# antoyang/FrozenBiLM

Hardware: AMD Instinct MI355X
Metric: video-text samples/sec (MLM fwd+bwd) DeBERTa-XL+adapters (higher is better)
Workload: dtype bf16; 1 GPU; DeBERTa-v2-XLarge(24L)+adapters ds8/8, B=32/GPU, T=10x1024, L=256 (S=266), MLM fwd+bwd+allreduce+clip+Adam, dropout 0.1 live, seeded random weights; global_batch=32, seq_len=266, parallelism=dp1, dead_layer23_encoder_pass=skipped (output unused, SURVEY fact 6); FLOPs still counted

## Files before the change

frozenbilm_amd/attn_bwd.py:

```python
from __future__ import annotations

import math
from dataclasses import dataclass, field
from typing import Optional

import torch

from . import lib as L

BF16, F32 = torch.bfloat16, torch.float32
ATTN_SCALE = 1.0 / math.sqrt(64 * 3)


_RANGE = {}


def _relidx_range(S, cfg):
    key = (S, cfg.position_buckets, cfg.max_rel, cfg.att_span)
    if key not in _RANGE:
        from .model.relpos import rel_index_vector

        rv = rel_index_vector(S, cfg.position_buckets, cfg.max_rel, cfg.att_span)
        _RANGE[key] = (int(rv[0]), int(rv[-1]) - int(rv[0]) + 1)
    return _RANGE[key]


_DRANGE = {}
POS_GRAD_MAX_DELTAS = 8


def _delta_ranges(S, cfg, dev, limit=POS_GRAD_MAX_DELTAS):
    key = (S, cfg.position_buckets, cfg.max_rel, cfg.att_span, str(dev))
    if key not in _DRANGE:
        import numpy as np

        from .model.relpos import rel_index_vector

        rv = np.asarray(rel_index_vector(S, cfg.position_buckets, cfg.max_rel, cfg.att_span), dtype=np.int64)
        rmin, rcnt = int(rv[0]), int(rv[-1]) - int(rv[0]) + 1
        first = np.searchsorted(rv, np.arange(rmin, rmin + rcnt), side="left")
        last = np.searchsorted(rv, np.arange(rmin, rmin + rcnt), side="right")
        dlo = (first - (S - 1)).astype(np.int16)
        dcnt = (last - first).astype(np.int16)
        _DRANGE[key] = (torch.from_numpy(dlo).to(dev), torch.from_numpy(dcnt).to(dev), int(dcnt.max()))
    cmax = _DRANGE[key][2]
    if limit is not None and cmax > limit:
        raise NotImplementedError(
            f"position-table gradients (fbl_attn_pos_grad) take at most {limit} relative positions per table "
            f"row; position_buckets={cfg.position_buckets}, max_relative_positions={cfg.max_rel} at sequence length {S} "
            f"puts {cmax} on one row")
    return _DRANGE[key]


def disent_attn_bwd(eng, run, sv, dctx, dqkv, dpqk, defer_pos=False):
    B, S, H, nh, span2 = run.B, run.S, eng.H, eng.nh, eng.span2
    Sp = (S + 63) // 64 * 64
    dev = eng.dev
    qkv = sv.qkv
    q, k, v = qkv[:, :H], qkv[:, H:2 * H], qkv[:, 2 * H:]
    pq, pk = sv.pqk[:, :H], sv.pqk[:, H:]
    relidx = eng.relidx(S)
    klen, border = run.klen, getattr(run, "border", None)
    scale = ATTN_SCALE
    pk_ = getattr(run, "pk", None)
    row0 = pk_.row0 if pk_ is not None else None
    saved_p = getattr(sv, "psave", None) is not None

    Dv = torch.empty(B, nh, S, dtype=F32, device=dev)
    PKX = torch.empty(nh, 2 * Sp, 64, dtype=BF16, device=dev)
    if saved_p:
        QT = PQT = None
        PQX = torch.empty(nh, 2 * Sp, 64, dtype=BF16, device=dev)
    else:
        QT = torch.empty(nh, 64, B, Sp, dtype=BF16, device=dev)
        PQT = torch.empty(nh, 64, span2, dtype=BF16, device=dev)
        PQX = None
    L.attn_bwd_prep(q, pq, pk, dctx, sv.ctx, QT, PQT, Dv, B, S, Sp, nh, span2, row0=row0, relidx=relidx, PQX=PQX, PKX=PKX)
    dS = torch.empty(B, nh, Sp, Sp, dtype=BF16, device=dev)
    dST = torch.empty(B, nh, Sp, Sp, dtype=BF16, device=dev)
    lin = eng.cfg.position_buckets // 2 if eng.cfg.position_buckets > 0 else eng.cfg.att_span - 1
    if saved_p:
        L.disent_attn_bwd_dspk(sv.psave, sv.msave, q, v, dctx, PQX, sv.lse, Dv, scale, dqkv[:, H:2 * H], dqkv[:, 2 * H:], dS, dST,
                               B, S, Sp, nh, p_drop=run.p_att, seed=sv.seed_att, klen=klen, border=border, row0=row0)
        sv.psave = sv.msave = None
    else:
        lin_a = min(lin, span2 // 2) if eng.cfg.position_buckets > 0 else 0
        L.disent_attn_bwd_ds(q, k, v, dctx, pk, pq, relidx, run.mask_i32, sv.lse, Dv, scale, dqkv[:, 2 * H:], dS, dST,
                             B, S, Sp, nh, span2, p_drop=run.p_att, seed=sv.seed_att, klen=klen, border=border, lin=lin_a, row0=row0)
    L.disent_attn_bwd_dq(dS, k, PKX, dqkv[:, :H], B, S, Sp, nh, klen=klen, border=border, row0=row0)
    if not saved_p:
        L.disent_attn_bwd_shear(dST, QT, PQT, relidx, dqkv[:, H:2 * H], B, S, Sp, nh, span2, klen=klen, lin=lin, border=border,
                                row0=row0)
    rmin, rcnt = _relidx_range(S, eng.cfg)
    state = dict(dS=dS, dST=dST, q=q, k=k, rmin=rmin, rcnt=rcnt, B=B, S=S, Sp=Sp, klen=klen, row0=row0)
    if defer_pos:
        return state
    dpqk.copy_(pos_table_grads(eng, state))
    return None


def pos_table_grads(eng, st):
    H, nh, span2 = eng.H, eng.nh, eng.span2
    rmin, rcnt, B, Sp = st["rmin"], st["rcnt"], st["B"], st["Sp"]
    dpos = torch.zeros(span2, 2 * H, dtype=F32, device=eng.dev)
    dlo, dcnt, cmax = _delta_ranges(st["S"], eng.cfg, eng.dev, limit=None)
    for neg, X, Y, col0 in ((0, st["dS"], st["q"], H), (1, st["dST"], st["k"], 0)):
        d = torch.empty(1, nh, rcnt, 64, dtype=F32, device=eng.dev)
        L.attn_pos_grad(neg, [X], [Y], dlo, dcnt, cmax, d, B, st["S"], Sp, nh, rcnt, klen=st["klen"], row0=st["row0"])
        dpos[rmin:rmin + rcnt, col0:col0 + H].view(rcnt, nh, 64).copy_(d[0].permute(1, 0, 2))
    return dpos


@dataclass
class PosChain:
    rmin: int
    rcnt: int
    B: int
    S: int
    Sp: int
    dS: list = field(default_factory=list)
    dST: list = field(default_factory=list)
    q: list = field(default_factory=list)
    k: list = field(default_factory=list)
    seeds: list = field(default_factory=list)
    klen: Optional[torch.Tensor] = None
    row0: Optional[torch.Tensor] = None
    n_formed: int = 0
    n_exec: int = 0
    nh: int = 0
    dev: Optional[torch.device] = None
    dbuf: Optional[tuple] = None

    def add(self, st, seed_pos):
        self.dS.append(st["dS"]); self.dST.append(st["dST"]); self.q.append(st["q"]); self.k.append(st["k"])
        self.seeds.append(seed_pos)
        self.klen, self.row0 = st["klen"], st["row0"]

    def formed_slot(self):
        assert not self.dS and self.n_exec > self.n_formed, "executions with formed table gradients come first"
        if self.dbuf is None:
            self.dbuf = tuple(torch.empty(self.n_exec, self.nh, self.rcnt, 64, dtype=F32, device=self.dev) for _ in range(2))
        return self.dbuf[0][self.n_formed], self.dbuf[1][self.n_formed]

    def add_formed(self, seed_pos):
        self.n_formed += 1
        self.seeds.append(seed_pos)


def pos_chain_buffers(eng, run):
    rmin, rcnt = _relidx_range(run.S, eng.cfg)
    return PosChain(rmin=rmin, rcnt=rcnt, B=run.B, S=run.S, Sp=(run.S + 63) // 64 * 64, nh=eng.nh, dev=eng.dev)


def pos_table_grads_batched(eng, run, pc: PosChain):
    H, nh, span2 = eng.H, eng.nh, eng.span2
    E, rmin, rcnt, B, Sp = len(pc.seeds), pc.rmin, pc.rcnt, pc.B, pc.Sp
    dev = eng.dev
    dpb = torch.empty(E, rcnt, 2 * H, dtype=BF16, device=dev)
    dlo, dcnt, cmax = _delta_ranges(pc.S, eng.cfg, dev, limit=None)
    for neg, X, Y, col0 in ((0, pc.dS, pc.q, H), (1, pc.dST, pc.k, 0)):
        nf = pc.n_formed
        if pc.dbuf is not None:
            assert pc.n_exec == E, (pc.n_exec, E)
            d = pc.dbuf[neg]
        else:
            d = torch.empty(E, nh, rcnt, 64, dtype=F32, device=dev)
        if X:
            L.attn_pos_grad(neg, X, Y, dlo, dcnt, cmax, d[nf:], B, pc.S, Sp, nh, rcnt, klen=pc.klen, row0=pc.row0)
        L.heads_to_rows_bf16(d, dpb[:, :, col0:col0 + H])
    if getattr(run, "lora_pos_wait", False):
        eng._lora_pos_bwd(run, pc, dpb)
    tmp = torch.empty(E, rcnt, H, dtype=F32, device=dev)
    L.gemm(dpb, eng.WposT_exec[:E], out_f32=tmp)
    dR = L.zeros(span2, H, dtype=F32, device=dev)
    L.dropout_sum_f32(tmp, pc.seeds if run.p_hid > 0 else [0] * E, run.p_hid, dR[rmin:rmin + rcnt], key0=rmin * H)
    return dR
```

frozenbilm_amd/build.py:

```python
from __future__ import annotations

import concurrent.futures as cf
import os
import shutil
import subprocess
import sys

HERE = os.path.dirname(os.path.abspath(__file__))
CSRC = os.path.join(HERE, "csrc")
DEBUG = os.environ.get("FBL_DEBUG_BUILD", "0") == "1"
OBJ = os.path.join(HERE, "csrc", "build_dbg" if DEBUG else "build")
LIB = os.path.join(HERE, "libfbl_dbg.so" if DEBUG else "libfbl.so")
ARCH = "gfx950"
FLAGS = ["--offload-arch=" + ARCH, "-O3", "-std=c++17", "-fPIC", "-fno-gpu-rdc", "-Wno-unused-result"]
if DEBUG:
    FLAGS.append("-DFBL_DEBUG_SWITCHES")
    FLAGS += os.environ.get("FBL_DEBUG_EXTRA_FLAGS", "").split()
    if os.environ.get("FBL_DEBUG_LIB_NAME"):
        LIB = os.path.join(HERE, os.environ["FBL_DEBUG_LIB_NAME"])
        OBJ = os.path.join(HERE, "csrc", "build_dbg_" + os.path.splitext(os.environ["FBL_DEBUG_LIB_NAME"])[0])


def _hipcc() -> str:
    for cand in (os.environ.get("HIPCC"), shutil.which("hipcc"), "/opt/rocm/bin/hipcc"):
        if cand and os.path.exists(cand):
            return cand
    raise RuntimeError("hipcc not found (need ROCm >= 7.0 with gfx950 support)")


def sources():
    return sorted(os.path.join(CSRC, f) for f in os.listdir(CSRC) if f.endswith(".hip"))


def _deps_mtime() -> float:
    hdrs = [os.path.join(CSRC, f) for f in os.listdir(CSRC) if f.endswith(".h")]
    hdrs += [os.path.join(os.path.dirname(HERE), "include", h) for h in ("fbl.h", "fbl_mha.h", "fbl_qrows.h", "fbl_live.h", "fbl_predict.h", "fbl_groups.h", "fbl_lora.h", "fbl_ema.h", "fbl_prompt.h")]
    return max(os.path.getmtime(h) for h in hdrs)


def _compile(src: str, force: bool) -> str:
    obj = os.path.join(OBJ, os.path.basename(src)[:-4] + ".o")
    if not force and os.path.exists(obj) and os.path.getmtime(obj) > max(os.path.getmtime(src), _deps_mtime()):
        return obj
    cmd = [_hipcc(), *FLAGS, "-Rpass-analysis=kernel-resource-usage", "-c", src, "-o", obj]
    r = subprocess.run(cmd, capture_output=True, text=True)
    if r.returncode != 0:
        raise RuntimeError(f"hipcc failed for {src}:\n{r.stdout}\n{r.stderr}")
    bad, name = [], "?"
    for line in r.stderr.splitlines():
        if "Function Name:" in line:
            name = line.split("Function Name:")[1].split("[")[0].strip()
        elif "ScratchSize [bytes/lane]:" in line:
            n = int(line.split("ScratchSize [bytes/lane]:")[1].split("[")[0])
            if n > 64:
                bad.append(f"{name}: {n} bytes/lane")
            elif n > 0:
                print(f"[frozenbilm_amd.build] note: {name} spills {n} bytes/lane")
    if bad and os.environ.get("FBL_ALLOW_SCRATCH", "0") != "1":
        os.remove(obj)
        raise RuntimeError(f"{os.path.basename(src)}: kernels using scratch memory (set FBL_ALLOW_SCRATCH=1 to build anyway):\n  "
                           + "\n  ".join(bad))
    return obj


def build_lib(force: bool = False, verbose: bool = True) -> str:
    os.makedirs(OBJ, exist_ok=True)
    srcs = sources()
    with cf.ThreadPoolExecutor(max_workers=min(8, len(srcs))) as ex:
        objs = list(ex.map(lambda s: _compile(s, force), srcs))
    if force or not os.path.exists(LIB) or any(os.path.getmtime(o) > os.path.getmtime(LIB) for o in objs):
        cmd = [_hipcc(), "--offload-arch=" + ARCH, "-shared", "-fPIC", "-o", LIB, *objs]
        r = subprocess.run(cmd, capture_output=True, text=True)
        if r.returncode != 0:
            raise RuntimeError(f"link failed:\n{r.stdout}\n{r.stderr}")
        if verbose:
            print(f"[frozenbilm_amd.build] linked {LIB} from {len(objs)} objects")
    elif verbose:
        print(f"[frozenbilm_amd.build] {LIB} up to date")
    return LIB


if __name__ == "__main__":
    build_lib(force="--force" in sys.argv)
```

frozenbilm_amd/csrc/rowops.hip:

```cpp
#include "fbl_common.h"
#include "../../include/fbl.h"
#include "../../include/fbl_live.h"
#include "../../include/fbl_groups.h"
#include "../../include/fbl_ema.h"

namespace {

template <int VEC>
struct VecF {};
template <>
struct VecF<4> {
  typedef f32x4 T;
};
template <>
struct VecF<2> {
  typedef f32x2 T;
};

template <int VEC>
__device__ __forceinline__ void ldf(const float* p, float* v) {
  if (VEC == 4) {
    f32x4 x = *(const f32x4*)p;
    v[0] = x[0]; v[1] = x[1]; v[2] = x[2]; v[3] = x[3];
  } else if (VEC == 2) {
    f32x2 x = *(const f32x2*)p;
    v[0] = x[0]; v[1] = x[1];
  } else {
    v[0] = p[0];
  }
}
template <int VEC>
__device__ __forceinline__ void stf(float* p, const float* v) {
  if (VEC == 4) *(f32x4*)p = (f32x4){v[0], v[1], v[2], v[3]};
  else if (VEC == 2) *(f32x2*)p = (f32x2){v[0], v[1]};
  else p[0] = v[0];
}
template <int VEC>
__device__ __forceinline__ void stb(bf16* p, const float* v) {
  if (VEC == 4) *(bf16x4*)p = (bf16x4){f2bf(v[0]), f2bf(v[1]), f2bf(v[2]), f2bf(v[3])};
  else if (VEC == 2) *(bf16x2*)p = (bf16x2){f2bf(v[0]), f2bf(v[1])};
  else p[0] = f2bf(v[0]);
}

struct LnFwdArgs {
  const float* y; long ldy; float p_drop; uint64_t seed; const uint64_t* seed_dev;
  const float* r_plain; const float* r_t; const float* r_stats; const float* r_gamma; const float* r_beta;
  const int32_t* r_rowmask;
  const float* gamma; const float* beta; float eps; const int32_t* rowmask;
  float* out_t; float* out_stats; bf16* out_bf16; float* out_f32;
  int N, H;
};

template <int EPL>
__global__ __launch_bounds__(256) void ln_fwd_kernel(LnFwdArgs a) {
  constexpr int VEC = (EPL % 4 == 0) ? 4 : ((EPL % 2 == 0) ? 2 : 1);
  constexpr int NIT = EPL / VEC;
  const int lane = threadIdx.x & 63;
  const int row = blockIdx.x * 4 + (threadIdx.x >> 6);
  if (row >= a.N) return;
  const int H = a.H;
  float v[EPL];
  const uint32_t thr = fbl_drop_thresh(a.p_drop);
  const float inv_keep = a.p_drop > 0.f ? 1.0f / (1.0f - a.p_drop) : 1.0f;
  const uint64_t seed = a.p_drop > 0.f ? fbl_seed(a.seed, a.seed_dev) : 0;
  float rmean = 0.f, rrstd = 0.f, rmask = 1.f;
  if (a.r_t) {
    rmean = a.r_stats[2 * (long)row];
    rrstd = a.r_stats[2 * (long)row + 1];
    if (a.r_rowmask) rmask = (float)a.r_rowmask[row];
  }
#pragma unroll
  for (int it = 0; it < NIT; ++it) {
    const int col = (it * 64 + lane) * VEC;
    float* vv = v + it * VEC;
    if (a.y) {
      ldf<VEC>(a.y + (long)row * a.ldy + col, vv);
      if (a.p_drop > 0.f) {
#pragma unroll
        for (int c = 0; c < VEC; ++c) vv[c] *= fbl_dropout_scale(seed, (uint64_t)row * H + col + c, thr, inv_keep);
      }
    } else {
#pragma unroll
      for (int c = 0; c < VEC; ++c) vv[c] = 0.f;
    }
    if (a.r_plain) {
      float r[VEC];
      ldf<VEC>(a.r_plain + (long)row * H + col, r);
#pragma unroll
      for (int c = 0; c < VEC; ++c) vv[c] += r[c];
    }
    if (a.r_t) {
      float r[VEC], gg[VEC], bb[VEC];
      ldf<VEC>(a.r_t + (long)row * H + col, r);
      ldf<VEC>(a.r_gamma + col, gg);
      ldf<VEC>(a.r_beta + col, bb);
#pragma unroll
      for (int c = 0; c < VEC; ++c) vv[c] += ((r[c] - rmean) * rrstd * gg[c] + bb[c]) * rmask;
    }
    if (a.out_t) stf<VEC>(a.out_t + (long)row * H + col, vv);
  }
  float s = 0.f;
#pragma unroll
  for (int e = 0; e < EPL; ++e) s += v[e];
  const float mean = wave_sum(s) / (float)H;
  float q = 0.f;
#pragma unroll
  for (int e = 0; e < EPL; ++e) {
    const float d = v[e] - mean;
    q += d * d;
  }
  const float var = wave_sum(q) / (float)H;
  const float rstd = rsqrtf(var + a.eps);
  if (lane == 0 && a.out_stats) {
    a.out_stats[2 * (long)row] = mean;
    a.out_stats[2 * (long)row + 1] = rstd;
  }
  const float om = a.rowmask ? (float)a.rowmask[row] : 1.0f;
#pragma unroll
  for (int it = 0; it < NIT; ++it) {
    const int col = (it * 64 + lane) * VEC;
    float gg[VEC], bb[VEC], o[VEC];
    ldf<VEC>(a.gamma + col, gg);
    ldf<VEC>(a.beta + col, bb);
#pragma unroll
    for (int c = 0; c < VEC; ++c) o[c] = ((v[it * VEC + c] - mean) * rstd * gg[c] + bb[c]) * om;
    if (a.out_bf16) stb<VEC>(a.out_bf16 + (long)row * H + col, o);
    if (a.out_f32) stf<VEC>(a.out_f32 + (long)row * H + col, o);
  }
}

struct LnMatArgs {
  const float* t; const float* stats; const float* gamma; const float* beta; const int32_t* rowmask;
  const float* add_bcast; int S; float* out_f32; bf16* out_bf16; int N, H;
};
template <int EPL>
__global__ __launch_bounds__(256) void ln_mat_kernel(LnMatArgs a) {
  constexpr int VEC = (EPL % 4 == 0) ? 4 : ((EPL % 2 == 0) ? 2 : 1);
  constexpr int NIT = EPL / VEC;
  const int lane = threadIdx.x & 63;
  const int row = blockIdx.x * 4 + (threadIdx.x >> 6);
  if (row >= a.N) return;
  const int H = a.H;
  const float mean = a.stats[2 * (long)row], rstd = a.stats[2 * (long)row + 1];
  const float om = a.rowmask ? (float)a.rowmask[row] : 1.0f;
#pragma unroll
  for (int it = 0; it < NIT; ++it) {
    const int col = (it * 64 + lane) * VEC;
    float x[VEC], gg[VEC], bb[VEC], o[VEC];
    ldf<VEC>(a.t + (long)row * H + col, x);
    ldf<VEC>(a.gamma + col, gg);
    ldf<VEC>(a.beta + col, bb);
#pragma unroll
    for (int c = 0; c < VEC; ++c) o[c] = ((x[c] - mean) * rstd * gg[c] + bb[c]) * om;
    if (a.add_bcast) {
      float p[VEC];
      ldf<VEC>(a.add_bcast + (long)(row % a.S) * H + col, p);
#pragma unroll
      for (int c = 0; c < VEC; ++c) o[c] += p[c];
    }
    if (a.out_f32) stf<VEC>(a.out_f32 + (long)row * H + col, o);
    if (a.out_bf16) stb<VEC>(a.out_bf16 + (long)row * H + col, o);
  }
}

constexpr int LNB_BLOCKS = 768;
struct LnBwdArgs {
  const float* dout; const int32_t* rowmask; const float* t; const float* stats; const float* gamma;
  float p_drop; uint64_t seed; const uint64_t* seed_dev; float* out_dt; bf16* out_dy_bf16; float* out_dy_f32; float* ws; int N, H;
  long ld_dyb;
};
template <int EPL>
__global__ __launch_bounds__(256) void ln_bwd_kernel(LnBwdArgs a) {
  constexpr int VEC = (EPL % 4 == 0) ? 4 : ((EPL % 2 == 0) ? 2 : 1);
  constexpr int NIT = EPL / VEC;
  __shared__ float red[4 * 64 * EPL];
  const int lane = threadIdx.x & 63, wave = threadIdx.x >> 6;
  const int H = a.H;
  float dg[EPL], db[EPL], dys[EPL], gam[EPL];
#pragma unroll
  for (int e = 0; e < EPL; ++e) dg[e] = db[e] = dys[e] = 0.f;
#pragma unroll
  for (int it = 0; it < NIT; ++it) ldf<VEC>(a.gamma + (it * 64 + lane) * VEC, gam + it * VEC);
  const uint32_t thr = fbl_drop_thresh(a.p_drop);
  const float inv_keep = a.p_drop > 0.f ? 1.0f / (1.0f - a.p_drop) : 1.0f;
  const uint64_t seed = a.p_drop > 0.f ? fbl_seed(a.seed, a.seed_dev) : 0;
  for (int row = blockIdx.x * 4 + wave; row < a.N; row += gridDim.x * 4) {
    const float mean = a.stats[2 * (long)row], rstd = a.stats[2 * (long)row + 1];
    const float om = a.rowmask ? (float)a.rowmask[row] : 1.0f;
    float g[EPL], xh[EPL];
    float s1 = 0.f, s2 = 0.f;
#pragma unroll
    for (int it = 0; it < NIT; ++it) {
      const int col = (it * 64 + lane) * VEC;
      float d[VEC], x[VEC];
      ldf<VEC>(a.dout + (long)row * H + col, d);
      ldf<VEC>(a.t + (long)row * H + col, x);
#pragma unroll
      for (int c = 0; c < VEC; ++c) {
        const int e = it * VEC + c;
        const float dd = d[c] * om;
        xh[e] = (x[c] - mean) * rstd;
        dg[e] += dd * xh[e];
        db[e] += dd;
        g[e] = dd * gam[e];
        s1 += g[e];
        s2 += g[e] * xh[e];
      }
    }
    s1 = wave_sum(s1) / (float)H;
    s2 = wave_sum(s2) / (float)H;
#pragma unroll
    for (int it = 0; it < NIT; ++it) {
      const int col = (it * 64 + lane) * VEC;
      float dt[VEC], dy[VEC];
#pragma unroll
      for (int c = 0; c < VEC; ++c) {
        const int e = it * VEC + c;
        dt[c] = rstd * (g[e] - s1 - xh[e] * s2);
        dy[c] = dt[c];
        if (a.p_drop > 0.f) dy[c] *= fbl_dropout_scale(seed, (uint64_t)row * H + col + c, thr, inv_keep);
        dys[e] += dy[c];
      }
      if (a.out_dt) stf<VEC>(a.out_dt + (long)row * H + col, dt);
      if (a.out_dy_bf16) stb<VEC>(a.out_dy_bf16 + (long)row * a.ld_dyb + col, dy);
      if (a.out_dy_f32) stf<VEC>(a.out_dy_f32 + (long)row * H + col, dy);
    }
  }
#pragma unroll
  for (int which = 0; which < 3; ++which) {
    const float* src = which == 0 ? dg : (which == 1 ? db : dys);
    if (which) __syncthreads();
#pragma unroll
    for (int it = 0; it < NIT; ++it) {
      const int col = (it * 64 + lane) * VEC;
#pragma unroll
      for (int c = 0; c < VEC; ++c) red[wave * H + col + c] = src[it * VEC + c];
    }
    __syncthreads();
    for (int i = threadIdx.x; i < H; i += 256) {
      float s_ = 0.f;
#pragma unroll
      for (int w = 0; w < 4; ++w) s_ += red[w * H + i];
      a.ws[(long)blockIdx.x * 3 * H + which * H + i] = s_;
    }
  }
}
template <int EPL>
__global__ __launch_bounds__(256, 3) void ln_bwd2_kernel(LnBwdArgs a) {
  static_assert(EPL % 2 == 0, "two waves share a row");
  constexpr int EW = EPL / 2;
  constexpr int VEC = (EW % 4 == 0) ? 4 : ((EW % 2 == 0) ? 2 : 1);
  constexpr int NIT = EW / VEC;
  __shared__ float red[2 * 64 * EPL];
  __shared__ float xch[2][2][2][2];
  const int lane = threadIdx.x & 63, wave = threadIdx.x >> 6;
  const int slot = wave >> 1, half = wave & 1;
  const int H = a.H;
  const int c0 = half * (H / 2);
  float dg[EW], db[EW], dys[EW], gam[EW];
#pragma unroll
  for (int e = 0; e < EW; ++e) dg[e] = db[e] = dys[e] = 0.f;
#pragma unroll
  for (int it = 0; it < NIT; ++it) ldf<VEC>(a.gamma + c0 + (it * 64 + lane) * VEC, gam + it * VEC);
  const uint32_t thr = fbl_drop_thresh(a.p_drop);
  const float inv_keep = a.p_drop > 0.f ? 1.0f / (1.0f - a.p_drop) : 1.0f;
  const uint64_t seed = a.p_drop > 0.f ? fbl_seed(a.seed, a.seed_dev) : 0;
  int par = 0;
  for (int base = blockIdx.x * 2; base < a.N; base += gridDim.x * 2, par ^= 1) {
    const int row = base + slot;
    const bool live = row < a.N;
    const int rr = live ? row : a.N - 1;
    const float mean = a.stats[2 * (long)rr], rstd = a.stats[2 * (long)rr + 1];
    const float om = live ? (a.rowmask ? (float)a.rowmask[rr] : 1.0f) : 0.f;
    float g[EW], xh[EW];
    float s1 = 0.f, s2 = 0.f;
#pragma unroll
    for (int it = 0; it < NIT; ++it) {
      const int col = c0 + (it * 64 + lane) * VEC;
      float d[VEC], x[VEC];
      ldf<VEC>(a.dout + (long)rr * H + col, d);
      ldf<VEC>(a.t + (long)rr * H + col, x);
#pragma unroll
      for (int c = 0; c < VEC; ++c) {
        const int e = it * VEC + c;
        const float dd = d[c] * om;
        xh[e] = (x[c] - mean) * rstd;
        dg[e] += dd * xh[e];
        db[e] += dd;
        g[e] = dd * gam[e];
        s1 += g[e];
        s2 += g[e] * xh[e];
      }
    }
    s1 = wave_sum(s1);
    s2 = wave_sum(s2);
    if (lane == 0) {
      xch[par][slot][half][0] = s1;
      xch[par][slot][half][1] = s2;
    }
    __syncthreads();
    s1 = (xch[par][slot][0][0] + xch[par][slot][1][0]) / (float)H;
    s2 = (xch[par][slot][0][1] + xch[par][slot][1][1]) / (float)H;
    if (live) {
#pragma unroll
      for (int it = 0; it < NIT; ++it) {
        const int col = c0 + (it * 64 + lane) * VEC;
        float dt[VEC], dy[VEC];
#pragma unroll
        for (int c = 0; c < VEC; ++c) {
          const int e = it * VEC + c;
          dt[c] = rstd * (g[e] - s1 - xh[e] * s2);
          dy[c] = dt[c];
          if (a.p_drop > 0.f) dy[c] *= fbl_dropout_scale(seed, (uint64_t)row * H + col + c, thr, inv_keep);
          dys[e] += dy[c];
        }
        if (a.out_dt) stf<VEC>(a.out_dt + (long)row * H + col, dt);
        if (a.out_dy_bf16) stb<VEC>(a.out_dy_bf16 + (long)row * a.ld_dyb + col, dy);
        if (a.out_dy_f32) stf<VEC>(a.out_dy_f32 + (long)row * H + col, dy);
      }
    }
  }
#pragma unroll
  for (int which = 0; which < 3; ++which) {
    const float* src = which == 0 ? dg : (which == 1 ? db : dys);
    __syncthreads();
#pragma unroll
    for (int it = 0; it < NIT; ++it) {
      const int col = c0 + (it * 64 + lane) * VEC;
#pragma unroll
      for (int c = 0; c < VEC; ++c) red[slot * H + col + c] = src[it * VEC + c];
    }
    __syncthreads();
    for (int i = threadIdx.x; i < H; i += 256) a.ws[(long)blockIdx.x * 3 * H + which * H + i] = red[i] + red[H + i];
  }
}

__device__ __forceinline__ float fold16(const float* ws, int nblk, int ncols, int col) {
  __shared__ float red[16][17];
  const int tx = threadIdx.x & 15, ty = threadIdx.x >> 4;
  float s = 0.f;
  if (col < ncols)
    for (int b = ty; b < nblk; b += 16) s += ws[(long)b * ncols + col];
  red[ty][tx] = s;
  __syncthreads();
  if (ty == 0) {
#pragma unroll
    for (int k = 1; k < 16; ++k) s += red[k][tx];
  }
  return s;
}
__global__ __launch_bounds__(256) void ln_bwd_fold_kernel(const float* ws, int nblk, int H, float* dgamma, float* dbeta,
                                                          float* dysum) {
  __shared__ f32x4 red[4][8];
  const int tx = threadIdx.x & 7, ty = threadIdx.x >> 3;
  const int lane = threadIdx.x & 63, wave = threadIdx.x >> 6;
  const int col = blockIdx.x * 32 + tx * 4;
  const int ncols = 3 * H;
  f32x4 s = {0.f, 0.f, 0.f, 0.f};
  if (col < ncols) {
    const float* p = ws + col;
    int b = ty;
    for (; b + 224 < nblk; b += 256) {
      f32x4 v[8];
#pragma unroll
      for (int u = 0; u < 8; ++u) v[u] = *(const f32x4*)(p + (long)(b + 32 * u) * ncols);
      s += ((v[0] + v[1]) + (v[2] + v[3])) + ((v[4] + v[5]) + (v[6] + v[7]));
    }
    for (; b < nblk; b += 32) s += *(const f32x4*)(p + (long)b * ncols);
  }
#pragma unroll
  for (int o = 8; o < 64; o <<= 1) {
#pragma unroll
    for (int r = 0; r < 4; ++r) s[r] += __shfl_xor(s[r], o, 64);
  }
  if (lane < 8) red[wave][lane] = s;
  __syncthreads();
  if (threadIdx.x < 8 && col < ncols) {
    s = (red[0][tx] + red[1][tx]) + (red[2][tx] + red[3][tx]);
    float* dst = col < H ? dgamma : (col < 2 * H ? dbeta : dysum);
    if (dst) {
      float* q = dst + (col % H);
#pragma unroll
      for (int r = 0; r < 4; ++r) q[r] += s[r];
    }
  }
}

__global__ void embed_gather_kernel(const int64_t* ids, const float* E, const float* vproj, int B, int T, int L, int H,
                                    float* out) {
  const int S = T + L;
  const int row = blockIdx.x;
  const int b = row / S, s = row % S;
  const float* src = (s < T) ? vproj + ((long)b * T + s) * H : E + ids[(long)b * L + (s - T)] * (long)H;
  float* dst = out + (long)row * H;
  for (int c = threadIdx.x * 4; c < H; c += blockDim.x * 4) *(f32x4*)(dst + c) = *(const f32x4*)(src + c);
}

__global__ void video_stage_kernel(const _Float16* feats, const int64_t* row_off, const int32_t* n_rows, int T, int F,
                                   float* out, int64_t* video_len, int64_t* video_mask) {
  const int b = blockIdx.x / T, j = blockIdx.x % T;
  const int n = n_rows[b];
  const int len = n < T ? n : T;
  if (threadIdx.x == 0) {
    if (j == 0 && video_len) video_len[b] = len;
    if (video_mask) video_mask[(long)b * T + j] = j < len ? 1 : 0;
  }
  float* dst = out + ((long)b * T + j) * F;
  if (j >= len) {
    for (int c = threadIdx.x * 4; c < F; c += blockDim.x * 4) *(f32x4*)(dst + c) = (f32x4){0.f, 0.f, 0.f, 0.f};
    return;
  }
  const long r = n > T ? ((long)j * n) / T : j;
  const _Float16* src = feats + (row_off[b] + r) * (long)F;
  typedef __attribute__((ext_vector_type(8))) _Float16 f16x8;
  for (int c = threadIdx.x * 8; c < F; c += blockDim.x * 8) {
    const f16x8 h = *(const f16x8*)(src + c);
    *(f32x4*)(dst + c) = (f32x4){(float)h[0], (float)h[1], (float)h[2], (float)h[3]};
    *(f32x4*)(dst + c + 4) = (f32x4){(float)h[4], (float)h[5], (float)h[6], (float)h[7]};
  }
}

__global__ void mask_tokens_kernel(int64_t* ids, int64_t* labels, long n, const int64_t* special, int n_special, float p,
                                   int64_t mask_id, int64_t vocab, uint64_t seed) {
  const long i = (long)blockIdx.x * blockDim.x + threadIdx.x;
  if (i >= n) return;
  const int64_t id = ids[i];
  bool sp = false;
  for (int k = 0; k < n_special; ++k) sp |= (special[k] == id);
  const float inv = 1.0f / 4294967296.0f;
  const bool pick = !sp && (float)fbl_hash(seed, 4ull * i) * inv < p;
  labels[i] = pick ? id : -100;
  if (!pick) return;
  if ((float)fbl_hash(seed, 4ull * i + 1) * inv < 0.8f) ids[i] = mask_id;
  else if ((float)fbl_hash(seed, 4ull * i + 2) * inv < 0.5f) ids[i] = (int64_t)(fbl_hash(seed, 4ull * i + 3) % (uint64_t)vocab);
}

__global__ void im2col3_kernel(const bf16* x, bf16* out, int B, int S, int H) {
  const int row = blockIdx.x;
  const int s = row % S;
  const int chunks = 3 * H / 8;
  for (int i = threadIdx.x; i < chunks; i += blockDim.x) {
    const int k = (i * 8) / H, c = (i * 8) % H;
    const int ss = s + k - 1;
    bf16x8 v = {0, 0, 0, 0, 0, 0, 0, 0};
    if (ss >= 0 && ss < S) v = *(const bf16x8*)(x + ((long)row + k - 1) * H + c);
    *(bf16x8*)(out + (long)row * 3 * H + i * 8) = v;
  }
}
__global__ void col2im3_kernel(const float* dcol, float* dx, int B, int S, int H, int accumulate) {
  const int row = blockIdx.x;
  const int s = row % S;
  for (int c = threadIdx.x * 4; c < H; c += blockDim.x * 4) {
    f32x4 acc = accumulate ? *(const f32x4*)(dx + (long)row * H + c) : (f32x4){0.f, 0.f, 0.f, 0.f};
#pragma unroll
    for (int k = 0; k < 3; ++k) {
      const int ss = s - k + 1;
      if (ss >= 0 && ss < S) acc += *(const f32x4*)(dcol + ((long)row - k + 1) * 3 * H + k * H + c);
    }
    *(f32x4*)(dx + (long)row * H + c) = acc;
  }
}

__global__ void dropout_gelu_fwd_kernel(const float* c, float p, uint64_t seed0, const uint64_t* seed_dev, float* out, long n) {
  const uint64_t seed = p > 0.f ? fbl_seed(seed0, seed_dev) : 0;
  const uint32_t thr = fbl_drop_thresh(p);
  const float ik = p > 0.f ? 1.f / (1.f - p) : 1.f;
  for (long i = (long)blockIdx.x * blockDim.x + threadIdx.x; i < n; i += (long)gridDim.x * blockDim.x) {
    float v = c[i];
    if (p > 0.f) v *= fbl_dropout_scale(seed, (uint64_t)i, thr, ik);
    out[i] = gelu_erf(v);
  }
}
// ... 472 lines not shown
__global__ __launch_bounds__(256) void swap_f32_kernel(float* a, float* b, long n4) {
  u32x4* a4 = (u32x4*)a;
  u32x4* b4 = (u32x4*)b;
  for (long i = (long)blockIdx.x * blockDim.x + threadIdx.x; i < n4; i += (long)gridDim.x * blockDim.x) {
    const u32x4 x = a4[i], y = b4[i];
    a4[i] = y;
    b4[i] = x;
  }
}
__global__ void cast_bf16_kernel(const float* in, bf16* out, long n) {
  for (long i = (long)blockIdx.x * blockDim.x + threadIdx.x; i < n; i += (long)gridDim.x * blockDim.x) out[i] = f2bf(in[i]);
}
__global__ void dropout_f32_kernel(const float* in, float p, uint64_t seed0, const uint64_t* seed_dev, float* of, bf16* ob, long n) {
  const uint64_t seed = p > 0.f ? fbl_seed(seed0, seed_dev) : 0;
  const uint32_t thr = fbl_drop_thresh(p);
  const float ik = p > 0.f ? 1.f / (1.f - p) : 1.f;
  for (long i = (long)blockIdx.x * blockDim.x + threadIdx.x; i < n; i += (long)gridDim.x * blockDim.x) {
    float v = in[i];
    if (p > 0.f) v *= fbl_dropout_scale(seed, (uint64_t)i, thr, ik);
    if (of) of[i] = v;
    if (ob) ob[i] = f2bf(v);
  }
}
__global__ void dropout_bf16_kernel(bf16* x, float p, uint64_t seed0, const uint64_t* seed_dev, long n) {
  const uint64_t seed = fbl_seed(seed0, seed_dev);
  const uint32_t thr = fbl_drop_thresh(p);
  const float ik = 1.f / (1.f - p);
  for (long i = (long)blockIdx.x * blockDim.x + threadIdx.x; i < n; i += (long)gridDim.x * blockDim.x)
    x[i] = f2bf(bf2f(x[i]) * fbl_dropout_scale(seed, (uint64_t)i, thr, ik));
}

struct DropSumArgs {
  uint64_t seeds[FBL_DROPSUM_MAX_SLICES];
  const float* x;
  const uint64_t* seed_dev;
  float* out;
  long n, key0;
  int ns;
  float p;
};
__global__ void dropout_sum_kernel(DropSumArgs a) {
  const uint32_t thr = fbl_drop_thresh(a.p);
  const float ik = a.p > 0.f ? 1.f / (1.f - a.p) : 1.f;
  const uint64_t word = (a.p > 0.f && a.seed_dev) ? *a.seed_dev : 0;
  for (long i = (long)blockIdx.x * blockDim.x + threadIdx.x; i < a.n; i += (long)gridDim.x * blockDim.x) {
    float acc = 0.f;
    for (int s = 0; s < a.ns; ++s) {
      float v = a.x[(long)s * a.n + i];
      if (a.p > 0.f) v *= fbl_dropout_scale(a.seeds[s] + word, (uint64_t)(a.key0 + i), thr, ik);
      acc += v;
    }
    a.out[i] = acc;
  }
}

__global__ void heads_to_rows_bf16_kernel(const float* src, bf16* dst, int E, int nh, int rows, long ld_dst) {
  const long total = (long)E * nh * rows * 8;
  for (long t = (long)blockIdx.x * blockDim.x + threadIdx.x; t < total; t += (long)gridDim.x * blockDim.x) {
    const int c8 = (int)(t & 7);
    const long q = t >> 3;
    const int r = (int)(q % rows);
    const long eh = q / rows;
    const int h = (int)(eh % nh);
    const long e = eh / nh;
    const f32x4 a = *(const f32x4*)(src + q * 64 + c8 * 8), b = *(const f32x4*)(src + q * 64 + c8 * 8 + 4);
    *(bf16x8*)(dst + (e * rows + r) * ld_dst + h * 64 + c8 * 8) =
        (bf16x8){f2bf(a[0]), f2bf(a[1]), f2bf(a[2]), f2bf(a[3]), f2bf(b[0]), f2bf(b[1]), f2bf(b[2]), f2bf(b[3])};
  }
}

inline int grid1d(long n, int block = 256, int cap = 256 * 16) {
  long b = (n + block - 1) / block;
  return (int)(b < 1 ? 1 : (b > cap ? cap : b));
}

}

#define FBL_EPL_DISPATCH(H, KERNEL, GRID, ARGS, STREAM)                                              \
  switch ((H) / 64) {                                                                                \
    case 1: hipLaunchKernelGGL(KERNEL<1>, GRID, dim3(256), 0, STREAM, ARGS); break;                  \
    case 2: hipLaunchKernelGGL(KERNEL<2>, GRID, dim3(256), 0, STREAM, ARGS); break;                  \
    case 4: hipLaunchKernelGGL(KERNEL<4>, GRID, dim3(256), 0, STREAM, ARGS); break;                  \
    case 8: hipLaunchKernelGGL(KERNEL<8>, GRID, dim3(256), 0, STREAM, ARGS); break;                  \
    case 12: hipLaunchKernelGGL(KERNEL<12>, GRID, dim3(256), 0, STREAM, ARGS); break;                \
    case 16: hipLaunchKernelGGL(KERNEL<16>, GRID, dim3(256), 0, STREAM, ARGS); break;                \
    case 24: hipLaunchKernelGGL(KERNEL<24>, GRID, dim3(256), 0, STREAM, ARGS); break;                \
    case 32: hipLaunchKernelGGL(KERNEL<32>, GRID, dim3(256), 0, STREAM, ARGS); break;                \
    default: return FBL_ERR_SHAPE;                                                                   \
  }

extern "C" int fbl_abi_version(void) { return 9; }

extern "C" int fbl_embed_gather(const int64_t* ids, const float* E, const float* vproj, int B, int T, int L, int H,
                                float* out_t, void* stream) {
  if (H % 4) return FBL_ERR_SHAPE;
  if (T > 0 && !vproj) return FBL_ERR_ARG;
  if (B * (T + L) <= 0) return 0;
  hipLaunchKernelGGL(embed_gather_kernel, dim3(B * (T + L)), dim3(128), 0, (hipStream_t)stream, ids, E, vproj, B, T, L,
                     H, out_t);
  FBL_CHECK_LAUNCH();
  return 0;
}

extern "C" int fbl_video_stage_f16(const void* feats_f16, const int64_t* row_off, const int32_t* n_rows, int B, int T, int F,
                                   float* out_f32, int64_t* video_len, int64_t* video_mask, void* stream) {
  if (F % 8 || ((uintptr_t)feats_f16 & 15) || ((uintptr_t)out_f32 & 15)) return FBL_ERR_ALIGN;
  if (B <= 0 || T <= 0) return 0;
  hipLaunchKernelGGL(video_stage_kernel, dim3(B * T), dim3(128), 0, (hipStream_t)stream, (const _Float16*)feats_f16, row_off,
                     n_rows, T, F, out_f32, video_len, video_mask);
  FBL_CHECK_LAUNCH();
  return 0;
}

extern "C" int fbl_mask_tokens(int64_t* ids, int64_t* labels, int64_t n, const int64_t* special_ids, int n_special,
                               float mlm_probability, int64_t mask_token_id, int64_t vocab_size, uint64_t seed,
                               void* stream) {
  if (n <= 0) return 0;
  if (vocab_size <= 0 || mlm_probability < 0.f || mlm_probability > 1.f || n_special < 0) return FBL_ERR_ARG;
  hipLaunchKernelGGL(mask_tokens_kernel, dim3((unsigned)((n + 255) / 256)), dim3(256), 0, (hipStream_t)stream, ids, labels,
                     (long)n, special_ids, n_special, mlm_probability, mask_token_id, vocab_size, seed);
  FBL_CHECK_LAUNCH();
  return 0;
}

extern "C" int fbl_ln_fwd(const float* y, int64_t ldy, float p_drop, uint64_t seed, const uint64_t* seed_dev, const float* r_plain,
                          const float* r_t, const float* r_stats, const float* r_gamma, const float* r_beta,
                          const int32_t* r_rowmask, const float* gamma, const float* beta, float eps,
                          const int32_t* rowmask, float* out_t, float* out_stats, void* out_bf16, float* out_f32, int N,
                          int H, void* stream) {
  if (H % 64 || H > 2048) return FBL_ERR_SHAPE;
  if (r_t && (!r_stats || !r_gamma || !r_beta)) return FBL_ERR_ARG;
  if (N <= 0) return 0;
  LnFwdArgs a{y, ldy, p_drop, seed, seed_dev, r_plain, r_t, r_stats, r_gamma, r_beta, r_rowmask, gamma, beta, eps, rowmask,
              out_t, out_stats, (bf16*)out_bf16, out_f32, N, H};
  dim3 grid((N + 3) / 4);
  FBL_EPL_DISPATCH(H, ln_fwd_kernel, grid, a, (hipStream_t)stream);
  FBL_CHECK_LAUNCH();
  return 0;
}

extern "C" int fbl_ln_materialize(const float* t, const float* stats, const float* gamma, const float* beta,
                                  const int32_t* rowmask, const float* add_bcast, int S, float* out_f32, void* out_bf16,
                                  int N, int H, void* stream) {
  if (H % 64 || H > 2048) return FBL_ERR_SHAPE;
  if (N <= 0) return 0;
  LnMatArgs a{t, stats, gamma, beta, rowmask, add_bcast, S > 0 ? S : 1, out_f32, (bf16*)out_bf16, N, H};
  dim3 grid((N + 3) / 4);
  FBL_EPL_DISPATCH(H, ln_mat_kernel, grid, a, (hipStream_t)stream);
  FBL_CHECK_LAUNCH();
  return 0;
}

extern "C" int64_t fbl_ln_bwd_ws_floats(int H) { return (int64_t)LNB_BLOCKS * 3 * H; }
extern "C" int fbl_ln_bwd(const float* dout, const int32_t* rowmask, const float* t, const float* stats,
                          const float* gamma, float p_drop, uint64_t seed, const uint64_t* seed_dev, float* out_dt, void* out_dy_bf16,
                          float* out_dy_f32, float* dgamma, float* dbeta, float* dysum, float* ws, int N, int H,
                          int64_t ld_dy_bf16, void* stream) {
  if (H % 64 || H > 2048) return FBL_ERR_SHAPE;
  if (N <= 0) return 0;
  if (ld_dy_bf16 == 0) ld_dy_bf16 = H;
  if (ld_dy_bf16 < H || (ld_dy_bf16 % 8)) return FBL_ERR_ALIGN;
  LnBwdArgs a{dout, rowmask, t, stats, gamma, p_drop, seed, seed_dev, out_dt, (bf16*)out_dy_bf16, out_dy_f32, ws, N, H, ld_dy_bf16};
  int nblk;
  if ((H / 64) % 2 == 0) {
    nblk = (N + 1) / 2;
    if (nblk > LNB_BLOCKS) nblk = LNB_BLOCKS;
    dim3 grid(nblk);
    switch (H / 64) {
      case 2: hipLaunchKernelGGL(ln_bwd2_kernel<2>, grid, dim3(256), 0, (hipStream_t)stream, a); break;
      case 4: hipLaunchKernelGGL(ln_bwd2_kernel<4>, grid, dim3(256), 0, (hipStream_t)stream, a); break;
      case 8: hipLaunchKernelGGL(ln_bwd2_kernel<8>, grid, dim3(256), 0, (hipStream_t)stream, a); break;
      case 12: hipLaunchKernelGGL(ln_bwd2_kernel<12>, grid, dim3(256), 0, (hipStream_t)stream, a); break;
      case 16: hipLaunchKernelGGL(ln_bwd2_kernel<16>, grid, dim3(256), 0, (hipStream_t)stream, a); break;
      case 24: hipLaunchKernelGGL(ln_bwd2_kernel<24>, grid, dim3(256), 0, (hipStream_t)stream, a); break;
      case 32: hipLaunchKernelGGL(ln_bwd2_kernel<32>, grid, dim3(256), 0, (hipStream_t)stream, a); break;
      default: return FBL_ERR_SHAPE;
    }
  } else {
    nblk = (N + 3) / 4;
    if (nblk > LNB_BLOCKS) nblk = LNB_BLOCKS;
    dim3 grid(nblk);
    FBL_EPL_DISPATCH(H, ln_bwd_kernel, grid, a, (hipStream_t)stream);
  }
  FBL_CHECK_LAUNCH();
  if (dgamma || dbeta || dysum) {
    hipLaunchKernelGGL(ln_bwd_fold_kernel, dim3((3 * H + 31) / 32), dim3(256), 0, (hipStream_t)stream, ws, nblk, H,
                       dgamma, dbeta, dysum);
    FBL_CHECK_LAUNCH();
  }
  return 0;
}

extern "C" int fbl_im2col3(const void* x_bf16, void* out_bf16, int B, int S, int H, void* stream) {
  if (H % 8) return FBL_ERR_SHAPE;
  if (B * S <= 0) return 0;
  hipLaunchKernelGGL(im2col3_kernel, dim3(B * S), dim3(256), 0, (hipStream_t)stream, (const bf16*)x_bf16,
                     (bf16*)out_bf16, B, S, H);
  FBL_CHECK_LAUNCH();
  return 0;
}
extern "C" int fbl_col2im3(const float* dcol, float* dx, int B, int S, int H, int accumulate, void* stream) {
  if (H % 4) return FBL_ERR_SHAPE;
  if (B * S <= 0) return 0;
  hipLaunchKernelGGL(col2im3_kernel, dim3(B * S), dim3(256), 0, (hipStream_t)stream, dcol, dx, B, S, H, accumulate);
  FBL_CHECK_LAUNCH();
  return 0;
}

extern "C" int fbl_dropout_gelu_fwd(const float* c, float p_drop, uint64_t seed, const uint64_t* seed_dev, float* out_f32,
                                    int64_t n, void* stream) {
  if (n <= 0) return 0;
  hipLaunchKernelGGL(dropout_gelu_fwd_kernel, dim3(grid1d(n)), dim3(256), 0, (hipStream_t)stream, c, p_drop, seed, seed_dev,
                     out_f32, (long)n);
  FBL_CHECK_LAUNCH();
  return 0;
}
extern "C" int fbl_dropout_gelu_bwd(const float* dy, const float* c, float p_drop, uint64_t seed, const uint64_t* seed_dev,
                                    void* out_bf16, float* out_f32, int64_t n, void* stream) {
  if (n <= 0) return 0;
  hipLaunchKernelGGL(dropout_gelu_bwd_kernel, dim3(grid1d(n)), dim3(256), 0, (hipStream_t)stream, dy, c, p_drop, seed, seed_dev,
                     (bf16*)out_bf16, out_f32, (long)n);
  FBL_CHECK_LAUNCH();
  return 0;
}

extern "C" int fbl_transpose_to_bf16(const void* in, int in_is_bf16, int64_t ld_in, int rows, int cols, void* out_bf16,
                                     int64_t rows_pad, void* stream) {
  if (rows_pad < rows) return FBL_ERR_ARG;
  if (rows_pad <= 0 || cols <= 0) return 0;
  dim3 grid((unsigned)((rows_pad + 63) / 64), (cols + 63) / 64);
  if (in_is_bf16)
    hipLaunchKernelGGL(transpose_kernel<true>, grid, dim3(256), 0, (hipStream_t)stream, in, (long)ld_in, rows, cols,
                       (bf16*)out_bf16, (long)rows_pad);
  else
    hipLaunchKernelGGL(transpose_kernel<false>, grid, dim3(256), 0, (hipStream_t)stream, in, (long)ld_in, rows, cols,
                       (bf16*)out_bf16, (long)rows_pad);
  FBL_CHECK_LAUNCH();
  return 0;
}

extern "C" int fbl_transpose_batched_bf16(const void* src_bf16, const int64_t* src_off, void* dst_bf16,
                                          const int64_t* dst_off, int count, int rows, int cols, void* stream) {
  if (count <= 0 || rows <= 0 || cols <= 0) return 0;
  hipLaunchKernelGGL(transpose_batched_kernel, dim3((rows + 63) / 64, (cols + 63) / 64, count), dim3(256), 0,
                     (hipStream_t)stream, (const bf16*)src_bf16, src_off, (bf16*)dst_bf16, dst_off, rows, cols);
  FBL_CHECK_LAUNCH();
  return 0;
}

extern "C" int64_t fbl_colsum_ws_floats(int cols) { return (int64_t)CS_BLOCKS * cols; }
extern "C" int fbl_colsum(const void* in, int in_is_bf16, int64_t ld_in, int rows, int cols, float* out, float* ws,
                          void* stream) {
  if (rows <= 0 || cols <= 0) return 0;
  int nblk = rows < CS_BLOCKS ? rows : CS_BLOCKS;
  dim3 grid(nblk, (cols + 255) / 256);
  if (in_is_bf16)
    hipLaunchKernelGGL(colsum_kernel<true>, grid, dim3(256), 0, (hipStream_t)stream, in, (long)ld_in, rows, cols, ws);
  else
    hipLaunchKernelGGL(colsum_kernel<false>, grid, dim3(256), 0, (hipStream_t)stream, in, (long)ld_in, rows, cols, ws);
  FBL_CHECK_LAUNCH();
  hipLaunchKernelGGL(colsum_fold_kernel, dim3((cols + 15) / 16), dim3(256), 0, (hipStream_t)stream, ws, nblk, cols,
                     out);
  FBL_CHECK_LAUNCH();
  return 0;
}

extern "C" int fbl_head_transpose(const void* v_bf16, int64_t ldv, void* vt_bf16, int B, int S, int Sp, int nh,
                                  int64_t out_sh, int64_t out_sb, int64_t out_sd, void* stream) {
  if (Sp < S || Sp % 64) return FBL_ERR_SHAPE;
  if (ldv % 8 || out_sh % 8 || out_sb % 8 || out_sd % 8 || ((uintptr_t)v_bf16 & 15) || ((uintptr_t)vt_bf16 & 15)) return FBL_ERR_ALIGN;
  if (B * S <= 0) return 0;
  hipLaunchKernelGGL(head_transpose_kernel, dim3(Sp / 64, nh, B), dim3(256), 0, (hipStream_t)stream,
                     (const bf16*)v_bf16, (long)ldv, (bf16*)vt_bf16, B, S, Sp, nh, (long)out_sh, (long)out_sb,
                     (long)out_sd);
  FBL_CHECK_LAUNCH();
  return 0;
}

extern "C" int fbl_ce_fwd(const float* logits, int64_t ldv, const int64_t* labels, int N, int V, float* row_lse,
                          float* loss_sum_cnt, void* stream) {
  if (N <= 0) return 0;
  hipLaunchKernelGGL(ce_fwd_kernel, dim3(N), dim3(256), 0, (hipStream_t)stream, logits, (long)ldv, labels, N, V,
                     row_lse, loss_sum_cnt);
  FBL_CHECK_LAUNCH();
  hipLaunchKernelGGL(ce_fold_kernel, dim3(1), dim3(256), 0, (hipStream_t)stream, logits, (long)ldv, labels, N, row_lse,
                     loss_sum_cnt);
  FBL_CHECK_LAUNCH();
  return 0;
}
extern "C" int fbl_ce_bwd_rows(const float* logits, int64_t ldv, const int64_t* labels, const int32_t* rows, int R,
                               int V, int Vp, const float* row_lse, const float* loss_sum_cnt, float gscale,
                               const float* gscale_dev, void* dlogits_bf16, void* stream) {
  if (R <= 0) return 0;
  if (Vp < V) return FBL_ERR_ARG;
  hipLaunchKernelGGL(ce_bwd_rows_kernel, dim3(R), dim3(256), 0, (hipStream_t)stream, logits, (long)ldv, labels, rows, V,
                     Vp, row_lse, loss_sum_cnt, gscale, gscale_dev, (bf16*)dlogits_bf16);
  FBL_CHECK_LAUNCH();
  return 0;
}

extern "C" int fbl_gather_rows_bf16(const void* in, int64_t ld, const int32_t* rows, int R, int cols, void* out,
                                    void* stream) {
  if (R <= 0) return 0;
  if (cols % 8 || ld % 8) return FBL_ERR_ALIGN;
  hipLaunchKernelGGL(gather_rows_bf16_kernel, dim3(R), dim3(128), 0, (hipStream_t)stream, (const bf16*)in, (long)ld,
                     rows, cols, (bf16*)out);
  FBL_CHECK_LAUNCH();
  return 0;
}
extern "C" int fbl_scatter_rows_f32(const float* in, const int32_t* rows, int R, int cols, float* out, int64_t ld,
                                    void* stream) {
  if (R <= 0) return 0;
  hipLaunchKernelGGL(scatter_rows_f32_kernel, dim3(R), dim3(256), 0, (hipStream_t)stream, in, rows, cols, out,
                     (long)ld);
  FBL_CHECK_LAUNCH();
  return 0;
}

extern "C" int64_t fbl_sumsq_ws_floats(void) { return SUMSQ_BLOCKS; }
extern "C" int fbl_sumsq(const float* x, int64_t n, float* out_sumsq, float* ws, void* stream) {
  if (n <= 0) return 0;
  if (!ws || !out_sumsq) return FBL_ERR_ARG;
  const int nblk = grid1d(n, 256, SUMSQ_BLOCKS);
  hipLaunchKernelGGL(sumsq_kernel, dim3(nblk), dim3(256), 0, (hipStream_t)stream, x, (long)n, ws);
  FBL_CHECK_LAUNCH();
  hipLaunchKernelGGL(sumsq_fold_kernel, dim3(1), dim3(256), 0, (hipStream_t)stream, (const float*)ws, nblk, out_sumsq);
  FBL_CHECK_LAUNCH();
  return 0;
}
extern "C" int fbl_adam_flat(float* p, const float* g, float* m, float* v, int64_t n, float lr, float beta1,
                             float beta2, float eps, float weight_decay, int step, const float* sumsq, float max_norm,
                             float grad_scale, void* stream) {
  if (n <= 0) return 0;
  const float bc1 = 1.0f - powf(beta1, (float)step);
  const float bc2 = 1.0f - powf(beta2, (float)step);
  hipLaunchKernelGGL(adam_flat_kernel, dim3(grid1d(n)), dim3(256), 0, (hipStream_t)stream, p, g, m, v, (long)n, lr,
                     beta1, beta2, eps, weight_decay, bc1, bc2, sumsq, max_norm, grad_scale);
  FBL_CHECK_LAUNCH();
  return 0;
}

static inline bool live_aligned(const void* a) { return ((uintptr_t)a & 15) == 0; }
extern "C" int fbl_sumsq_live(const float* x, int64_t n, const int64_t* ranges, float* out_sumsq, float* ws, void* stream) {
// ... 140 lines not shown
```

frozenbilm_amd/engine.py:

```python
from __future__ import annotations

from dataclasses import dataclass, field
from typing import Dict, List, Optional

import numpy as np
import torch

from . import lib as L
from .predict import check_topk, of_call as predictions_of_call
from .live_set import REL_LN, LiveSetMixin, flat_layout, stage_plan
from .attn_bwd import ATTN_SCALE, _relidx_range, disent_attn_bwd, pos_chain_buffers, pos_table_grads_batched
from .model.deberta import PROMPT_NAME
from .model.relpos import rel_index_vector

BF16, F32 = torch.bfloat16, torch.float32


def _ru(x: int, m: int) -> int:
    return (x + m - 1) // m * m


def check_logit_rows(logit_rows: torch.Tensor, n_grid: int) -> None:
    r = logit_rows.reshape(-1)
    if r.numel() == 0:
        return
    s = torch.sort(r.long()).values
    dup = (s[1:] == s[:-1]).any() if s.numel() > 1 else torch.zeros((), dtype=torch.bool, device=s.device)
    lo, hi, dup = torch.stack([s[0], s[-1], dup.long()]).tolist()
    if lo < 0 or hi >= n_grid:
        raise ValueError(f"logit_rows must index the [B, S] token grid: 0 <= row < {n_grid} (got {lo} .. {hi})")
    if dup:
        raise ValueError("logit_rows holds an index more than once: with gradients every requested row must be distinct")


@dataclass
class NormRef:
    t: torch.Tensor
    stats: torch.Tensor
    gamma: torch.Tensor
    beta: torch.Tensor
    rowmask: Optional[torch.Tensor] = None

    def as_args(self):
        return (self.t, self.stats, self.gamma, self.beta, self.rowmask)


@dataclass
class Stream:
    bf16: torch.Tensor
    norm: Optional[NormRef] = None
    plain: Optional[torch.Tensor] = None
    full: Optional[torch.Tensor] = None


@dataclass
class Packing:
    row0: torch.Tensor
    sel: torch.Tensor
    inv: torch.Tensor
    pos: torch.Tensor
    n: int


@dataclass
class MergedPack:
    A: int
    WT: torch.Tensor
    WM: torch.Tensor
    bM: torch.Tensor
    b16: torch.Tensor
    WF: Optional[torch.Tensor]
    groups: list


@dataclass
class AdapterSite:
    name: str
    A: int
    Ap: int
    down: torch.Tensor
    up: torch.Tensor
    bd: torch.Tensor
    bu: torch.Tensor
    merged: bool
    grouped: bool
    WM: Optional[torch.Tensor] = None
    bM: Optional[torch.Tensor] = None
    WF: Optional[torch.Tensor] = None
    upT: Optional[torch.Tensor] = None
    downT: Optional[torch.Tensor] = None


@dataclass
class LoraSite:
    name: str
    li: int
    t: int
    idx: int


class Engine(LiveSetMixin):
    def __init__(self, model):
        self.m = model
        cfg = model.config
        self.cfg = cfg
        self.H, self.I, self.V = cfg.hidden_size, cfg.intermediate_size, cfg.vocab_size
        self.nh = cfg.num_attention_heads
        self.nL = cfg.num_hidden_layers
        self.span2 = 2 * cfg.att_span
        self.lin_span = min(cfg.position_buckets // 2, cfg.att_span) if cfg.position_buckets > 0 else 0
        self.F = model.features_dim
        self.Fp = _ru(self.F, 64) if self.F else 0
        self.A1 = self.H // model.ds_factor_attn if model.ds_factor_attn else 0
        self.A2 = self.H // model.ds_factor_ff if model.ds_factor_ff else 0
        self.Vp = _ru(self.V, 64)
        dev = model.device
        if dev.type != "cuda":
            raise RuntimeError("frozenbilm_amd runs on MI355X only: move the model to a cuda (HIP) device; "
                               "there is no CPU fallback")
        L.load()
        self.dev = dev
        o = dict(getattr(model, "engine_options", None) or {})
        unknown = set(o) - {"eager_logits", "dw_group", "attn_save_p"}
        if unknown:
            raise ValueError(f"unknown engine_options: {sorted(unknown)}")
        self.eager_logits = bool(o.get("eager_logits", False))
        self.attn_save_p = bool(o.get("attn_save_p", True))
        self.dw_group = max(1, min(L.ADW_MAX_ADAPTERS, int(o.get("dw_group", 16))))
        self.n_prompt = int(getattr(model, "n_prompt", 0))
        self._build_flat()
        self._pack_frozen()
        self._build_trainable_operands()
        self._build_lora()
        self._compose_ev = None
        self._relidx: Dict[int, torch.Tensor] = {}
        self._pos_cache: Dict[int, torch.Tensor] = {}
        self._no_pos_cache = False
        self.reducer = None
        self._dyz_pool: Dict[tuple, list] = {}
        self._dyz_shape = None
        self.params_version = 0
        self._ops_version = None
        self.skip_dead_layer = True
        self._ln_ws = L.ln_bwd_ws(self.H, dev)
        self._cs_ws = L.colsum_ws(max(self.H, self.I), dev)
        self.sk_ws = torch.empty(48 << 20, dtype=F32, device=dev)
        self.side = torch.cuda.Stream(device=dev)
        self.side_ws = torch.empty(8 << 20, dtype=F32, device=dev)
        self.side_cs_ws = L.colsum_ws(max(self.H, self.I), dev)
        if L._AUX.get(dev.index if dev.index is not None else torch.cuda.current_device()) is None:
            L.set_aux_stream(torch.cuda.Stream(device=dev), dev)
        L.exclude_from_aux(self.side)

    def _build_flat(self):
        from .model.deberta import flat_order

        m = self.m
        named = dict(m.named_parameters())
        train_names = m.trainable_names()
        order = flat_order(self.cfg, train_names)
        offs, total = flat_layout(order, {n: named[n].numel() for n in order})
        self.flat = torch.zeros(total, dtype=F32, device=self.dev)
        from .parallel import SCALAR_SLOT

        self.flat_grad_full = torch.zeros(SCALAR_SLOT + total, dtype=F32, device=self.dev)
        self.flat_grad = self.flat_grad_full[SCALAR_SLOT:]
        self.flat_bf16 = torch.zeros(total, dtype=BF16, device=self.dev)
        self.offsets, self.order = offs, order
        self._adT_offs = {}
        self.G: Dict[str, torch.Tensor] = {}
        self.Pb: Dict[str, torch.Tensor] = {}
        for n in order:
            p = named[n]
            o, k = offs[n], p.numel()
            view = self.flat[o:o + k].view(p.shape)
            view.copy_(p.data)
            p.data = view
            self.G[n] = self.flat_grad[o:o + k].view(p.shape)
            self.Pb[n] = self.flat_bf16[o:o + k].view(p.shape)
        self.P = {n: p.data for n, p in named.items()}
        self.named = named
        self.bucket_ends: Dict[str, int] = {}
        for n in order:
            key = self._bucket_key(n)
            self.bucket_ends[key] = offs[n] + _ru(named[n].numel(), 8)
        self._plans: Dict[tuple, object] = {}
        self._init_live()

    def plan(self, grad_in=()):
        key = (self.live_version, bool(grad_in))
        pl = self._plans.get(key)
        if pl is None:
            pl = self._plans[key] = stage_plan(self.nL, bool(self.cfg.conv_kernel_size), self.live_order, grad_in)
        return pl

    def _bucket_key(self, name: str) -> str:
        if name.startswith("lm_predictions."):
            return "head"
        if name.startswith("deberta.encoder.layer."):
            return "layer" + name.split(".")[3]
        if name.startswith("deberta.encoder.conv."):
            return "conv"
        if name.startswith("deberta.encoder.LayerNorm"):
            return "relln"
        return "emb"

    def attach_grads(self):
        fresh = all(self.named[n].grad is None for n in self.live_order)
        if fresh:
            L.zero_(self.flat_grad)
        for n in self.live_order:
            p = self.named[n]
            if p.grad is None:
                if not fresh:
                    self.G[n].zero_()
                p.grad = self.G[n]
            elif p.grad.data_ptr() != self.G[n].data_ptr():
                self.G[n].copy_(p.grad)
                p.grad = self.G[n]

    def _pack_frozen(self):
        P, H, I = self.P, self.H, self.I
        nL, dev = self.nL, self.dev
        bf = lambda t: t.to(BF16).contiguous()
        self.WoT_rev = torch.empty(nL, H, H, dtype=BF16, device=dev)
        self.WdT_rev = torch.empty(nL, I, H, dtype=BF16, device=dev)
        self.Lw = []
        for i in range(self.nL):
            p = f"deberta.encoder.layer.{i}"
            s = p + ".attention.self."
            j = nL - 1 - i
            Wqkv = torch.cat([P[s + "query_proj.weight"], P[s + "key_proj.weight"], P[s + "value_proj.weight"]], 0)
            self.WoT_rev[j].copy_(P[p + ".attention.output.dense.weight"].t())
            self.WdT_rev[j].copy_(P[p + ".output.dense.weight"].t())
            d = dict(
                Wqkv=bf(Wqkv), WqkvT=bf(Wqkv.t()),
                bqkv=torch.cat([P[s + "query_proj.bias"], P[s + "key_proj.bias"], P[s + "value_proj.bias"]]).float().contiguous(),
                Wo=bf(P[p + ".attention.output.dense.weight"]), WoT=self.WoT_rev[j],
                bo=P[p + ".attention.output.dense.bias"].float().contiguous(),
                Wi=bf(P[p + ".intermediate.dense.weight"]), WiT=bf(P[p + ".intermediate.dense.weight"].t()),
                bi=P[p + ".intermediate.dense.bias"].float().contiguous(),
                Wd=bf(P[p + ".output.dense.weight"]), WdT=self.WdT_rev[j],
                bd=P[p + ".output.dense.bias"].float().contiguous(),
            )
            self.Lw.append(d)
        order = [nL - 1, nL - 1] + list(range(nL - 2, -1, -1)) + [nL - 1]
        self.WposT_exec = torch.empty(len(order), H, 2 * H, dtype=BF16, device=dev)
        for e, li in enumerate(order):
            self.WposT_exec[e].copy_(self.Lw[li]["WqkvT"][:, : 2 * H])
        if self.cfg.conv_kernel_size:
            w = P["deberta.encoder.conv.conv.weight"]
            W2 = w.permute(0, 2, 1).reshape(H, 3 * H)
            self.Wc, self.WcT = bf(W2), bf(W2.t())
            self.bc = P["deberta.encoder.conv.conv.bias"].float().contiguous()
        hd = "lm_predictions.lm_head."
        self.Wh, self.WhT = bf(P[hd + "dense.weight"]), bf(P[hd + "dense.weight"].t())
        self.bh = P[hd + "dense.bias"].float().contiguous()
        E = P["deberta.embeddings.word_embeddings.weight"]
        self.E32 = E.float().contiguous()
        self.Eb = bf(E)
        self.ETb = torch.zeros(H, self.Vp, dtype=BF16, device=self.dev)
        self.ETb[:, : self.V] = E.t().to(BF16)
        self.head_bias = P[hd + "bias"].float().contiguous()
        self.rel_emb = P["deberta.encoder.rel_embeddings.weight"].float().contiguous()
        self.pos_emb = P["deberta.embeddings.position_embeddings.weight"].float().contiguous()
        if self.m.n_ans:
            T = P["answer_embeddings.weight"]
            self.n_ans = T.shape[0]
            self.Ansb = bf(T)
            self.ans_bias = P["answer_bias"].float().contiguous()

    def _build_trainable_operands(self):
        H, nL, dev = self.H, self.nL, self.dev
        self.sites = [[None, None] for _ in range(nL)]
        self.packs: List[MergedPack] = []
        for k, (blk, A, K, WT, wkey, bkey) in enumerate(((".attention.output.adapter", self.A1, H, self.WoT_rev, "Wo", "bo"),
                                                         (".output.adapter", self.A2, self.I, self.WdT_rev, "Wd", "bd"))):
            if not A:
                continue
            Ap = _ru(A, 64)
            merged = A % 64 == 0 and H % 64 == 0
            names = [f"deberta.encoder.layer.{i}{blk}" for i in range(nL)]
            pack = None
            if merged:
                WF = torch.zeros(nL, H, _ru(H + A, 128), dtype=BF16, device=dev) if k == 0 else None
                ow = [self.offsets[n + ".down.weight"] for n in names]
                ob = [self.offsets[n + ".down.bias"] for n in names]
                if nL >= 3 and len({ow[i - 1] - ow[i] for i in range(2, nL)}) == 1 and \
                        len({ob[i - 1] - ob[i] for i in range(2, nL)}) == 1 and ow[nL - 2] - ow[nL - 1] == ob[nL - 2] - ob[nL - 1] > 0:
                    groups = [(nL - 1, 1, ow[0], ob[0], A * H), (0, nL - 1, ow[nL - 1], ob[nL - 1], ow[nL - 2] - ow[nL - 1])]
                else:
                    groups = [(nL - 1 - i, 1, ow[i], ob[i], A * H) for i in range(nL)]
                pack = MergedPack(A=A, WT=WT, WM=torch.zeros(nL, H + A, K, dtype=BF16, device=dev),
# ... 121 lines not shown
            for t, site in enumerate(sites):
                if self._lora_live(site):
                    segs.setdefault(site.name, []).append(self._lora_products(site, dpb[e][:, t * H:(t + 1) * H], x))
        groups, nseg = [], 0
        for nm, sg in list(segs.items()) + [(None, None)]:
            if groups and (nm is None or len(groups) == L.ADW_MAX_ADAPTERS or nseg + len(sg) > L.ADW_MAX_SEGMENTS):
                L.adapter_bwd_dw(groups, A=self.lora_r)
                groups, nseg = [], 0
            if nm is not None:
                groups.append((sg, *self._dw_outputs(nm, self.Gl)))
                nseg += len(sg)

    def relidx(self, S: int) -> torch.Tensor:
        if S not in self._relidx:
            v = rel_index_vector(S, self.cfg.position_buckets, self.cfg.max_rel, self.cfg.att_span)
            self._relidx[S] = torch.from_numpy(np.ascontiguousarray(v)).to(self.dev)
        return self._relidx[S]

    def _refresh_if_stale(self, need_grad: bool):
        frozen = getattr(self.m, "_weights_frozen", 0) > 0
        ver = (self.params_version, tuple(self.named[n]._version for n in self.order)) if (frozen and not need_grad) else None
        if ver is None or ver != self._ops_version:
            self.refresh_trainable_operands()
            self._ops_version = ver

    def seed_word_value(self) -> int:
        return (self.m.dropout_seed_base() * 0x9E3779B1) & 0x7FFFFFFFFFFFFFFF

    def prepare_inference(self):
        self._refresh_if_stale(False)
        if self._compose_ev is not None:
            torch.cuda.current_stream().wait_event(self._compose_ev[1])
            self._compose_ev = None

    def invalidate_operands(self):
        self._ops_version = None
        self.params_version += 1

    def refresh_trainable_operands(self):
        self._pos_cache.clear()
        L.cast_bf16(self.flat, self.flat_bf16)
        for a in self.all_sites:
            if a.Ap != a.A:
                a.up[:, :a.A] = self.Pb[a.name + ".up.weight"]
            a.upT = a.downT = None
        if self.packs:
            self.side.wait_stream(torch.cuda.current_stream())
            with torch.cuda.stream(self.side):
                self._compose_ev = self._compose_adapter_down()
        if self.F and self.Fp != self.F:
            self.Wv[:, : self.F] = self.Pb["deberta.embeddings.linear_video.weight"]
        if self.lora_r:
            self._lora_ops = None
            self._compose_lora()

    def _compose_adapter_down(self):
        H = self.H

        def run_group(pk: MergedPack, grp):
            A, (j0, nb, o_w, o_b, st) = pk.A, grp
            wd3 = torch.as_strided(self.flat_bf16, (nb, A, H), (st, H, 1), o_w)
            L.gemm(wd3, pk.WT[j0:j0 + nb], out_bf16=pk.WM[j0:j0 + nb, H:H + A, :])
            if pk.WF is not None:
                L.gemm(pk.WT[j0:j0 + nb], wd3, out_bf16=pk.WF[j0:j0 + nb, :, H:H + A])
            bd3 = torch.as_strided(self.flat, (nb, A, 1), (st, 1, 1), o_b)
            bo3 = torch.as_strided(pk.bM, (nb, A, 1), (pk.bM.stride(0), 1, 1), pk.bM[j0, H:].storage_offset())
            L.gemm(wd3, pk.b16[j0:j0 + nb], aux=bd3, aux_kind=L.AUX_ADD_F32, out_f32=bo3)

        for pk in self.packs:
            run_group(pk, pk.groups[0])
        ev0 = torch.cuda.Event()
        ev0.record()
        for pk in self.packs:
            for grp in pk.groups[1:]:
                run_group(pk, grp)
        ev1 = torch.cuda.Event()
        ev1.record()
        return ev0, ev1

    def _adapter_bwd_operands(self, site: AdapterSite):
        if site.upT is None:
            H = self.H
            groups = {}
            for a in self.all_sites:
                groups.setdefault((a.A, a.Ap), []).append(a)
            for (A, Ap), sites in groups.items():
                upT_all = torch.empty(len(sites), A, H, dtype=BF16, device=self.dev)
                for i, a in enumerate(sites):
                    a.upT = upT_all[i]
                cache = self._adT_offs.get((A, Ap))
                if cache is None:
                    i64 = lambda v: torch.tensor(v, dtype=torch.int64, device=self.dev)
                    cache = dict(up_src=i64([self.offsets[a.name + ".up.weight"] for a in sites]),
                                 dn_src=i64([self.offsets[a.name + ".down.weight"] for a in sites]),
                                 dst=i64([i * A * H for i in range(len(sites))]))
                    self._adT_offs[(A, Ap)] = cache
                L.transpose_batched_bf16(self.flat_bf16, cache["up_src"], upT_all, cache["dst"], H, A)
                if Ap == A:
                    dnT_all = torch.empty(len(sites), H, A, dtype=BF16, device=self.dev)
                    L.transpose_batched_bf16(self.flat_bf16, cache["dn_src"], dnT_all, cache["dst"], A, H)
                    for i, a in enumerate(sites):
                        a.downT = dnT_all[i]
                else:
                    for a in sites:
                        a.downT = torch.zeros(H, Ap, dtype=BF16, device=self.dev)
                        a.downT[:, :A].copy_(a.down.t())
        return site.upT, site.downT

    def run(self, input_ids, attention_mask, video, video_mask, labels, mlm, want_hidden, logit_rows=None, want_attn=False,
            inputs_embeds=None):
        m = self.m
        train = m.training
        k_pred = check_topk(getattr(m, "predict_topk", 0))
        text = input_ids if inputs_embeds is None else inputs_embeds
        if text.device != self.dev:
            raise RuntimeError(f"inputs must be on {self.dev}")
        B, Lt = text.shape[:2]
        if attention_mask is None:
            attention_mask = (torch.ones_like(input_ids) if inputs_embeds is None
                              else torch.ones(B, Lt, dtype=torch.long, device=self.dev))
        use_video = bool(self.F) and video is not None
        grad_on = torch.is_grad_enabled()
        grad_in = []
        if grad_on and use_video and video.requires_grad:
            grad_in.append(("video", video))
        if grad_on and inputs_embeds is not None and inputs_embeds.requires_grad:
            grad_in.append(("embeds", inputs_embeds))
        need_grad = grad_on and (self.update_live() or bool(grad_in))
        T = video.shape[1] if use_video else 0
        Pn = self.n_prompt
        S = T + Pn + Lt
        if S > self.cfg.max_position_embeddings:
            raise RuntimeError(
                f"sequence of {S} positions (video {T} + " + (f"prompt {Pn} + " if Pn else "") + f"text {Lt}) exceeds "
                f"max_position_embeddings={self.cfg.max_position_embeddings} (the reference fails the same way, "
                "model/deberta.py:1020-1021,1392)")
        front = []
        if use_video:
            if video_mask is None:
                video_mask = torch.ones(video.shape[:2], device=self.dev, dtype=attention_mask.dtype)
            front.append(video_mask.to(attention_mask.dtype))
        if Pn:
            front.append(torch.ones(B, Pn, device=self.dev, dtype=attention_mask.dtype))
        mask = torch.cat([*front, attention_mask], 1) if front else attention_mask
        mask = mask.to(torch.int32).contiguous()
        full_labels = None
        if labels is not None:
            if T + Pn:
                full_labels = torch.cat([torch.full((B, T + Pn), -100, dtype=torch.long, device=self.dev), labels], 1)
            else:
                full_labels = labels
            full_labels = full_labels.contiguous().view(-1)
            rows_labelled = torch.nonzero(full_labels != -100).view(-1)
        if logit_rows is not None:
            if full_labels is not None:
                raise RuntimeError("logit_rows cannot be combined with labels (the loss of a labelled call lives on its own rows)")
            if need_grad:
                check_logit_rows(logit_rows, B * S)
        pk = None
        if (getattr(m, "packed_rows", False) and not want_attn and (full_labels is not None or logit_rows is not None)
                and not torch.cuda.is_current_stream_capturing()):
            pk = self._make_packing(mask, full_labels, logit_rows, B, S, T)
        if train:
            m.step_seed += 1
        run = Run(B=B, S=S, T=T, P=Pn, Lt=Lt, train=train, save=need_grad, seed_base=self.seed_word_value() if train else 0,
                  p_hid=self.cfg.hidden_dropout_prob if train else 0.0,
                  p_att=self.cfg.attention_probs_dropout_prob if train else 0.0,
                  p_ad=m.adapter_dropout if train else 0.0, mask=mask.view(-1), pk=pk, N=pk.n if pk is not None else B * S,
                  want_attn=bool(want_attn), labels=full_labels, rows=rows_labelled if full_labels is not None else None)
        if want_attn and train and run.p_att > 0:
            raise NotImplementedError("output_attentions=True is served in eval mode (the probabilities of a training forward "
                                      "carry the attention dropout mask, which the fused kernel regenerates instead of storing)")
        if (getattr(m, "decoder_rows", False) and not self.lora_r and not want_attn and not want_hidden and not self.eager_logits
                and (full_labels is not None or logit_rows is not None) and not torch.cuda.is_current_stream_capturing()):
            run.dec_grid = (rows_labelled if full_labels is not None else logit_rows.to(self.dev).long().view(-1))
        if pk is not None and full_labels is not None:
            run.label_rows = rows_labelled
            run.rows = pk.inv[rows_labelled]
        self._refresh_if_stale(need_grad)
        use_ans = bool(m.n_ans) and not mlm
        if logit_rows is not None:
            run.logit_rows = logit_rows.to(self.dev).to(torch.int32).contiguous().view(-1)
            if pk is not None:
                run.logit_rows = pk.inv[run.logit_rows.long()].to(torch.int32)
        run.embeds = inputs_embeds
        run.video_dtype = video.dtype if use_video else None
        run.grad_in = tuple(k for k, _ in grad_in)
        if need_grad:
            run.plan, run.live_version = self.plan(run.grad_in), self.live_version
        run.hid_grad = bool(want_hidden) and need_grad
        with L.seed_word(run.seed_word):
            logits, loss_t = self._forward(run, input_ids.contiguous() if inputs_embeds is None else None, video, use_ans,
                                           want_hidden or want_attn)
        Vout = self.n_ans if use_ans else self.V
        if logit_rows is not None:
            res = {"logits": logits[:, :Vout], "loss": None, "run": run}
        else:
            res = {"logits": logits.view(B, S, -1)[:, :, :Vout] if logits is not None else None, "loss": None, "run": run}
        if k_pred:
            res["predictions"] = predictions_of_call(run, logits, k_pred, rows_labelled if full_labels is not None else None,
                                                     logit_rows)
        if want_hidden:
            res["hidden_states"] = run.hidden_out
        if want_attn:
            res["attentions"] = tuple(run.attn_out)
        if need_grad and res["logits"] is not None:
            lt = loss_t if loss_t is not None else torch.zeros((), dtype=F32, device=self.dev)
            hid = res["hidden_states"] if run.hid_grad else ()
            outs = _StepFn.apply(self, run, lt, res["logits"], len(hid), *hid, *[t for _, t in grad_in],
                                 *[self.named[n] for n in self.order])
            loss_o, res["logits"] = outs[:2]
            res["loss"] = loss_o if full_labels is not None else None
            if hid:
                res["hidden_states"] = tuple(outs[2:])
        elif full_labels is not None:
            res["loss"] = loss_t
        return res

    def _make_packing(self, mask, full_labels, logit_rows, B, S, T) -> Optional[Packing]:
        dev = self.dev
        keep = mask.view(B, S) != 0
        if full_labels is not None:
            keep = keep | (full_labels.view(B, S) != -100)
        if logit_rows is not None:
            want = torch.zeros(B * S, dtype=torch.bool, device=dev)
            want[logit_rows.to(dev).long().view(-1)] = True
            keep = keep | want.view(B, S)
        pos1 = torch.arange(1, S + 1, device=dev, dtype=torch.int32)
        plen_h = [max(int(v), T, 1) for v in (keep.to(torch.int32) * pos1).amax(1).tolist()]
        n = sum(plen_h)
        if n >= B * S:
            return None
        offs = [0]
        for v in plen_h:
            offs.append(offs[-1] + v)
        row0 = torch.tensor(offs, dtype=torch.int32, device=dev)
        b_of = torch.repeat_interleave(torch.arange(B, device=dev), torch.tensor(plen_h, device=dev), output_size=n)
        pos = torch.arange(n, device=dev) - row0[:-1].long()[b_of]
        sel = b_of * S + pos
        inv = torch.full((B * S,), -1, dtype=torch.int64, device=dev)
        inv[sel] = torch.arange(n, device=dev)
        return Packing(row0=row0, sel=sel, inv=inv, pos=pos, n=n)

    def _ln(self, run, name, *, y, resid: Optional[Stream], N, p_drop=0.0, rowmask=None, want_f32=False, tail=0):
        H = self.H
        g, b = self.P[name + ".weight"], self.P[name + ".bias"]
        t = torch.empty(N, H, dtype=F32, device=self.dev)
        stats = torch.empty(N, 2, dtype=F32, device=self.dev)
        full = torch.empty(N + tail, H, dtype=BF16, device=self.dev)
        ob = full[:N]
        of = torch.empty(N, H, dtype=F32, device=self.dev) if want_f32 else None
        seed = run.next_seed() if p_drop > 0 else 0
        r_norm = resid.norm.as_args() if resid is not None and resid.norm is not None else None
        r_plain = resid.plain if resid is not None and r_norm is None else None
        L.ln_fwd(y=y, p_drop=p_drop, seed=seed, r_plain=r_plain, r_norm=r_norm,
                 gamma=g, beta=b, eps=self.cfg.layer_norm_eps, rowmask=rowmask, out_t=t, out_stats=stats, out_bf16=ob,
                 out_f32=of, N=N, H=H)
        return Stream(bf16=ob, norm=NormRef(t, stats, g, b, rowmask), plain=of, full=full if tail else None), seed

    def _adapter_fwd(self, run, site: AdapterSite, x_f32, x_bf16, N):
        A, Ap = site.A, site.Ap
        z = torch.zeros(N, Ap, dtype=BF16, device=self.dev) if Ap != A else torch.empty(N, Ap, dtype=BF16, device=self.dev)
        seed = run.next_seed() if run.p_ad > 0 else 0
        L.adapter_down_fwd(x_bf16, site.down, site.bd, z, A=A, p_drop=run.p_ad, seed=seed)
        y = torch.empty(N, self.H, dtype=F32, device=self.dev)
        L.gemm(z, site.up, bias=site.bu, aux=x_f32, aux_kind=L.AUX_ADD_F32, out_f32=y)
        return y, z, seed

    def _dense_adapter_ln(self, run, li, x_bf16, W, bias, site: Optional[AdapterSite], N, ln_name, resid: Stream, tail=0):
        H, dev = self.H, self.dev
        ob = torch.empty(N, H, dtype=BF16, device=dev)
        if site is None or not site.merged:
            y = torch.empty(N, H, dtype=F32, device=dev)
            L.gemm(x_bf16, W, bias=bias, out_f32=y, out_bf16=ob)
            z, seed_ad = None, 0
            if site is not None:
                y, z, seed_ad = self._adapter_fwd(run, site, y, ob, N)
            out, seed_ln = self._ln(run, ln_name, y=y, resid=resid, N=N, p_drop=run.p_hid, tail=tail)
            return out, ob, z, seed_ad, seed_ln
        if self._compose_ev is not None:
            torch.cuda.current_stream().wait_event(self._compose_ev[0 if li == 0 else 1])
        A = site.A
        z = torch.empty(N, A, dtype=BF16, device=dev)
        seed_ad = run.next_seed() if run.p_ad > 0 else 0
        L.dense_adapter_down_fwd(x_bf16, site.WM, site.bM, H, z, y_bf16=ob, p_drop=run.p_ad, seed=seed_ad)
        g, b = self.P[ln_name + ".weight"], self.P[ln_name + ".bias"]
        t = torch.empty(N, H, dtype=F32, device=dev)
        stats = torch.empty(N, 2, dtype=F32, device=dev)
        full = torch.empty(N + tail, H, dtype=BF16, device=dev)
        seed_ln = run.next_seed() if run.p_hid > 0 else 0
        r_norm = resid.norm.as_args() if resid.norm is not None else None
        L.adapter_up_resid_fwd(z, site.up, site.bu, ob, t, A=A, p_drop=run.p_hid, seed=seed_ln,
                               r_plain=resid.plain if r_norm is None else None, r_norm=r_norm)
        L.ln_fwd(y=t, gamma=g, beta=b, eps=self.cfg.layer_norm_eps, out_stats=stats, out_bf16=full[:N], N=N, H=H)
        return (Stream(bf16=full[:N], norm=NormRef(t, stats, g, b, None), full=full if tail else None), ob, z, seed_ad,
                seed_ln)

    def _pos_proj_cached(self, li: int, W, Rb: torch.Tensor) -> torch.Tensor:
        c = self._pos_cache.get(li)
        if c is None:
            c = torch.empty(self.span2, 2 * self.H, dtype=BF16, device=self.dev)
            L.gemm(Rb, W["Wqkv"][: 2 * self.H], bias=W["bqkv"][: 2 * self.H], out_bf16=c)
            self._pos_cache[li] = c
        return c

    def _pos_cache_allowed(self, run) -> bool:
        return not run.save and run.p_hid == 0 and getattr(self.m, "_weights_frozen", 0) > 0 and not self._no_pos_cache

    def _layer_fwd(self, run, li: int, kv: Stream, q: Optional[Stream], Rb: torch.Tensor):
        W = self.Lw[li]
        B, S, H, nh = run.B, run.S, self.H, self.nh
        N = run.N
        Sp = _ru(S, 64)
        dev = self.dev
        sv = LayerSave(li=li, emd=q is not None)
        P_ = self.span2
        if run.p_hid > 0:
            sv.seed_pos = run.next_seed()

        def put_r(full):
            if run.p_hid > 0:
                L.dropout_f32(run.R32, run.p_hid, sv.seed_pos, out_bf16=full[N:])
            else:
                full[N:].copy_(Rb)

        infer = not run.save and run.p_hid == 0
        pqk_c = self._pos_proj_cached(li, W, Rb) if self._pos_cache_allowed(run) else None
        reuse = infer and q is not None and run.emd_qkv is not None
        if reuse:
            qkv = run.emd_qkv
            if pqk_c is None:
                put_r(q.full)
            L.gemm(q.full if pqk_c is None else q.bf16, W["Wqkv"][:H], bias=W["bqkv"][:H], out_bf16=qkv[:, :H])
        else:
            rows_in = N if pqk_c is not None else N + P_
            qkv = torch.empty(rows_in, 3 * H, dtype=BF16, device=dev)
            kin = kv.full[:rows_in]
            if pqk_c is None:
                put_r(kv.full)
            if q is None:
                L.gemm(kin, W["Wqkv"], bias=W["bqkv"], out_bf16=qkv)
            else:
                if pqk_c is None:
                    put_r(q.full)
                L.gemm(q.full[:rows_in], W["Wqkv"][:H], bias=W["bqkv"][:H], out_bf16=qkv[:, :H])
                L.gemm(kin, W["Wqkv"][H:], bias=W["bqkv"][H:], out_bf16=qkv[:, H:])
                if infer:
                    run.emd_qkv = qkv
        if pqk_c is not None:
            pq, pk = pqk_c[:, :H], pqk_c[:, H:]
        else:
            pq, pk = qkv[N:, :H], qkv[N:, H:2 * H]
        ctx = torch.empty(N, H, dtype=BF16, device=dev)
        lse = torch.empty(B, nh, S, dtype=F32, device=dev)
        sv.seed_att = run.next_seed() if run.p_att > 0 else 0
        psave = msave = None
        if run.save and self.attn_save_p:
            psave = torch.empty(B, nh, Sp, Sp, dtype=BF16, device=dev)
            msave = torch.empty(B, nh, Sp // 64, S, dtype=F32, device=dev)
        L.disent_attn_fwd(qkv[:N, :H], qkv[:N, H:2 * H], qkv[:N, 2 * H:], pk, pq, self.relidx(S), run.mask_i32,
                          ATTN_SCALE, ctx, lse, B, S, Sp, nh, self.span2, p_drop=run.p_att, seed=sv.seed_att, klen=run.klen,
                          border=run.border, lin=self.lin_span, row0=run.row0, psave=psave, msave=msave)
        sv.psave, sv.msave = psave, msave
        if run.want_attn and q is None:
            probs = torch.empty(B, nh, S, S, dtype=F32, device=dev)
            L.disent_attn_probs(qkv[:N, :H], qkv[:N, H:2 * H], pk, pq, self.relidx(S), run.mask_i32, lse,
                                ATTN_SCALE, probs, B, S, nh)
            run.attn_out.append(probs)
        if run.save:
            sv.qkv, sv.pqk, sv.ctx, sv.lse = qkv[:N], qkv[N:, : 2 * H], ctx, lse
# ... 172 lines not shown
        return Vout, table, bias, ldv

    def _labelled_loss(self, run, lc, labels):
        run.loss_acc = L.zeros(2, dtype=F32, device=self.dev)
        if lc is not None:
            run.labels_c = labels.contiguous()
            run.row_lse = torch.empty(lc.shape[0], dtype=F32, device=self.dev)
            L.ce_fwd(lc, run.labels_c, run.Vout, run.row_lse, run.loss_acc)
            run.logits_c = lc
        run.logits = torch.empty(run.B * run.S, run.ldv, dtype=F32, device=self.dev)
        run.logits_pending = True
        return run.loss_acc[0] / run.loss_acc[1]

    def _decoder_rows_fwd(self, run, kv: Stream, Rb, use_ans):
        from .row_plan import plan_query_rows

        H, nh, dev = self.H, self.nh, self.dev
        B, S, N = run.B, run.S, run.N
        li = self.nL - 1
        W = self.Lw[li]
        pk = run.pk
        pl = plan_query_rows(run.dec_grid, B, S, inv=pk.inv if pk is not None else None)
        run.dec_plan = pl
        R = pl.R
        Sp = _ru(S, 64)
        q = None
        if R:
            n_ = kv.norm
            if n_ is not None:
                qc32 = torch.empty(R, H, dtype=F32, device=dev)
                rm = n_.rowmask.index_select(0, pl.krows) if n_.rowmask is not None else None
                L.ln_materialize(n_.t.index_select(0, pl.krows), n_.stats.index_select(0, pl.krows), n_.gamma, n_.beta, rowmask=rm,
                                 out_f32=qc32)
            else:
                qc32 = kv.plain.index_select(0, pl.krows)
            qc32.add_(self.pos_emb.index_select(0, pl.rpos.long()))
            q = Stream(bf16=qc32.to(BF16), plain=qc32)
            kvp = torch.empty(N, 2 * H, dtype=BF16, device=dev)
            L.gemm(kv.bf16, W["Wqkv"][H:], bias=W["bqkv"][H:], out_bf16=kvp)
        keep = run.save
        run.save = keep and self._stage_runs(run, "decoder")
        for _ in range(2):
            sv = LayerSave(li=li, emd=True)
            if run.p_hid > 0:
                sv.seed_pos = run.next_seed()
            sv.seed_att = run.next_seed() if run.p_att > 0 else 0
            if not R:
                self._skip_tail_seeds(run, li)
                continue
            if run.p_hid > 0:
                Rd = torch.empty(self.span2, H, dtype=BF16, device=dev)
                L.dropout_f32(run.R32, run.p_hid, sv.seed_pos, out_bf16=Rd)
            else:
                Rd = Rb
            if self._pos_cache_allowed(run):
                pqk = self._pos_proj_cached(li, W, Rb)
            else:
                pqk = torch.empty(self.span2, 2 * H, dtype=BF16, device=dev)
                L.gemm(Rd, W["Wqkv"][: 2 * H], bias=W["bqkv"][: 2 * H], out_bf16=pqk)
            qp = torch.empty(R, H, dtype=BF16, device=dev)
            L.gemm(q.bf16, W["Wqkv"][:H], bias=W["bqkv"][:H], out_bf16=qp)
            ctx = torch.empty(R, H, dtype=BF16, device=dev)
            lse = torch.empty(nh, R, dtype=F32, device=dev)
            L.disent_attn_fwd_qrows(qp, pl.rseg, pl.rpos, kvp[:, :H], kvp[:, H:], pqk[:, H:], pqk[:, :H], self.relidx(S), run.mask_i32,
                                    run.klen, ATTN_SCALE, ctx, lse, B, S, Sp, nh, self.span2, p_drop=run.p_att, seed=sv.seed_att,
                                    row0=run.row0)
            if run.save:
                sv.qc, sv.kvp, sv.pqk, sv.ctx, sv.lse = qp, kvp, pqk, ctx, lse
            q = self._layer_tail(run, li, sv, ctx, q, R)
        run.save = keep
        Vout, table, bias, ldv = self._head_tables(run, use_ans)
        hin = q.bf16 if R else torch.empty(0, H, dtype=BF16, device=dev)
        hp, hl = self._head_stage(run, hin, R)
        run.head_pre, run.head_norm, run.head_ln_bf16 = hp, hl.norm, hl.bf16
        lc = torch.empty(R, ldv, dtype=F32, device=dev)
        if R:
            L.gemm(hl.bf16, table, bias=bias, out_f32=lc, N=Vout)
        if run.labels is None:
            run.logits = lc.index_select(0, pl.back)
            return run.logits, None
        run.rows_i32 = run.rows.to(torch.int32)
        loss_t = self._labelled_loss(run, lc, run.labels[pl.grid]) if R else self._labelled_loss(run, None, None)
        return run.logits, loss_t

    def fill_logits(self, run):
        if run.logits_pending:
            run.logits_pending = False
            if run.dec_plan is not None:
                run.logits.zero_()
                if run.dec_plan.R:
                    run.logits.index_copy_(0, run.dec_plan.grid, run.logits_c)
                return
            hin_all = run.head_in_all
            if hin_all is not None:
                _, hl = self._head_stage(run, hin_all, hin_all.shape[0])
                run.head_ln_bf16, run.head_in_all = hl.bf16, None
            pk = run.pk
            if pk is None:
                L.gemm(run.head_ln_bf16, run.head_table, bias=run.head_bias, out_f32=run.logits, N=run.Vout)
            else:
                run.logits.zero_()
                for r0 in range(0, pk.n, 1024):
                    r1 = min(pk.n, r0 + 1024)
                    slab = torch.empty(r1 - r0, run.logits.shape[1], dtype=F32, device=self.dev)
                    L.gemm(run.head_ln_bf16[r0:r1], run.head_table, bias=run.head_bias, out_f32=slab, N=run.Vout)
                    run.logits.index_copy_(0, pk.sel[r0:r1], slab)

    def _head_stage(self, run, hin, N):
        hp = torch.empty(N, self.H, dtype=F32, device=self.dev)
        L.gemm(hin, self.Wh, bias=self.bh, out_f32=hp)
        hg = torch.empty(N, self.H, dtype=F32, device=self.dev)
        L.dropout_gelu_fwd(hp, 0.0, 0, hg)
        hl, _ = self._ln(run, "lm_predictions.lm_head.LayerNorm", y=hg, resid=None, N=N)
        return hp, hl

    def _materialize(self, s: Stream, add=None, S=1, out_f32=None, out_bf16=None):
        N, H = s.bf16.shape
        if s.plain is not None and add is None and out_bf16 is None:
            return s.plain
        if out_f32 is None:
            out_f32 = torch.empty(N, H, dtype=F32, device=self.dev)
        if s.norm is not None:
            n = s.norm
            L.ln_materialize(n.t, n.stats, n.gamma, n.beta, rowmask=n.rowmask, add_bcast=add, S=S, out_f32=out_f32,
                             out_bf16=out_bf16)
        else:
            v = s.plain if add is None else (s.plain.view(-1, S, H) + add[:S]).view(N, H)
            out_f32.copy_(v)
            if out_bf16 is not None:
                out_bf16.copy_(v)
        return out_f32

    def _conv_fwd(self, run, emb: Stream, l0: Stream) -> Stream:
        B, S, H, dev = run.B, run.S, self.H, self.dev
        N = run.N
        pk = run.pk
        if pk is None:
            col = torch.empty(N, 3 * H, dtype=BF16, device=dev)
            L.im2col3(emb.bf16, col, B, S, H)
        else:
            grid = torch.zeros(B * S, H, dtype=BF16, device=dev).index_copy_(0, pk.sel, emb.bf16)
            colg = torch.empty(B * S, 3 * H, dtype=BF16, device=dev)
            L.im2col3(grid, colg, B, S, H)
            col = colg.index_select(0, pk.sel)
        c = torch.empty(N, H, dtype=F32, device=dev)
        L.gemm(col, self.Wc, bias=self.bc, rowscale=run.mask_f, out_f32=c)
        y = torch.empty(N, H, dtype=F32, device=dev)
        run.seed_conv = run.next_seed() if run.p_hid > 0 else 0
        L.dropout_gelu_fwd(c, run.p_hid, run.seed_conv, y)
        out, _ = self._ln(run, "deberta.encoder.conv.LayerNorm", y=y, resid=l0, N=N, rowmask=run.rowmask, tail=self.span2)
        run.conv_c, run.conv_norm = c, out.norm
        return out

    def _ln_bwd(self, name, dout, norm: NormRef, p_drop, seed, want_dy_bf16=True, dysum=None, tail=0, dy_out=None):
        N, H = dout.shape
        dt_full = torch.empty(N + tail, H, dtype=F32, device=self.dev)
        dt = dt_full[:N]
        if tail:
            dt_full[N:].zero_()
        dyb = dy_out if dy_out is not None else (torch.empty(N, H, dtype=BF16, device=self.dev) if want_dy_bf16 else None)
        L.ln_bwd(dout, norm.t, norm.stats, norm.gamma, rowmask=norm.rowmask, p_drop=p_drop, seed=seed, out_dt=dt,
                 out_dy_bf16=dyb, dgamma=self.Gl.get(name + ".weight"), dbeta=self.Gl.get(name + ".bias"), dysum=dysum,
                 ws=self._ln_ws)
        if tail:
            return dt, dyb, dt_full
        return dt, dyb

    def _adapter_bwd(self, run, site: AdapterSite, dyb, z, xin_b, seed, dz_out=None, pooled=None):
        N, H = dyb.shape
        A, Ap = site.A, site.Ap
        dev = self.dev
        upT, downT = self._adapter_bwd_operands(site)
        if dz_out is not None:
            dz = dz_out
        else:
            dz = torch.zeros(N, Ap, dtype=BF16, device=dev) if Ap != A else torch.empty(N, Ap, dtype=BF16, device=dev)
        inv_keep = 1.0 / (1.0 - run.p_ad) if run.p_ad > 0 else 1.0
        L.gemm(dyb, upT, alpha=inv_keep, aux=z, aux_kind=L.AUX_MUL_POS_BF16, out_bf16=dz, N=A)
        dx = None
        if dz_out is None:
            dx = torch.empty(N, H, dtype=BF16, device=dev)
            L.gemm(dz, downT, aux=dyb, aux_kind=L.AUX_ADD_BF16, out_bf16=dx)
        sk = max(2, min(16, N // 512))
        nm = site.name
        gwu, gwd, gbd = (self.Gl.get(nm + k) for k in (".up.weight", ".down.weight", ".down.bias"))
        if gwu is None and gwd is None and gbd is None:
            return dx

        if site.grouped:
            run.dw_pending.append((A, nm, (dyb, z, dz, xin_b), run.dw_count, pooled))
            run.dw_count += 1
            return dx

        self.side.wait_stream(torch.cuda.current_stream())
        with torch.cuda.stream(self.side):
            if gwu is not None:
                L.gemm_tn_acc(dyb, z, gwu, self.side_ws, N=A, splitk=sk)
            if gwd is not None:
                L.gemm_tn_acc(dz, xin_b, gwd, self.side_ws, M=A, splitk=sk)
            if gbd is not None:
                L.colsum(dz, gbd, self.side_cs_ws, cols=A)
        if not torch.cuda.is_current_stream_capturing():
            for t in (dyb, z, dz, xin_b):
                t.record_stream(self.side)
        else:
            run._pos_keep.extend((dyb, z, dz, xin_b))
        run.side_used = True
        if self.reducer is not None:
            run.dw_event = torch.cuda.Event()
            run.dw_event.record(self.side)
        return dx

    def _dw_flush(self, run, red=None, force=False):
        pend = run.dw_pending
        while pend and (force or len({rec[1] for rec in pend}) >= self.dw_group):
            take, names, rest = {}, set(), []
            for rec in pend:
                A, nm, seg = rec[:3]
                if nm in names or len(names) >= min(self.dw_group, L.ADW_MAX_ADAPTERS):
                    rest.append(rec)
                else:
                    names.add(nm)
                    take.setdefault((A, getattr(seg[0], "shape", (None,))[0]), []).append((nm, seg))
            for (A, _rows), recs in take.items():
                Gl = getattr(self, "Gl", None)
                Gl = self.G if Gl is None else Gl
                L.adapter_bwd_dw([([seg], *Engine._dw_outputs(self, nm, Gl)) for nm, seg in recs], A=A)
            kept = {id(r) for r in rest}
            for rec in pend:
                if id(rec) not in kept and rec[4] is not None and tuple(rec[4].shape) == self._dyz_shape:
                    self._dyz_pool.setdefault(self._dyz_shape, []).append(rec[4])
            pend[:] = rest
        if red is not None:
            parked = {self._bucket_key(rec[1] + ".up.weight") for rec in pend}
            still = []
            for key in run.dw_ready_keys:
                if key in parked:
                    still.append(key)
                elif not (getattr(run, "lora_pos_wait", False) and key.startswith("layer")):
                    red.ready(key)
            run.dw_ready_keys[:] = still

    def _layer_bwd(self, run, sv: "LayerSave", dout: torch.Tensor):
        li = sv.li
        W, (a1, a2) = self.Lw[li], self.sites[li]
        H, I, dev = self.H, self.I, self.dev
        N = dout.shape[0]
        p = f"deberta.encoder.layer.{li}"
        dt2, dy2 = self._ln_bwd(p + ".output.LayerNorm", dout, sv.ln2, run.p_hid, sv.seed_ln2,
                                dysum=self.Gl.get(a2.name + ".up.bias") if a2 is not None else None)
        df = dy2
        if a2 is not None:
            df = self._adapter_bwd(run, a2, dy2, sv.z2, sv.fb, sv.seed_ad2)
        dh = torch.empty(N, I, dtype=BF16, device=dev)
        L.gemm(df, W["WdT"], aux=sv.hpre, aux_kind=L.AUX_MUL_BF16, out_bf16=dh)
        da = torch.empty(N, H, dtype=F32, device=dev)
        L.gemm(dh, W["WiT"], aux=dt2, aux_kind=L.AUX_ADD_F32, out_f32=da)
        del dh
        dctx = torch.empty(N, H, dtype=BF16, device=dev)
        if a1 is not None and a1.merged:
            A1, Kf = a1.A, a1.WF.shape[1]
            pooled = None
            can_pool = not torch.cuda.is_current_stream_capturing() and a1.grouped and sv.kvp is None
            if can_pool and self._dyz_shape != (N, Kf):
                self._dyz_pool.clear()
                self._dyz_shape = (N, Kf)
            free = self._dyz_pool.get((N, Kf)) if can_pool else None
            if free:
                dyz = pooled = free.pop()
            elif can_pool:
                dyz = pooled = torch.zeros(N, Kf, dtype=BF16, device=dev)
            else:
                dyz = torch.empty(N, Kf, dtype=BF16, device=dev)
                if Kf > H + A1:
                    dyz[:, H + A1:].zero_()
            dt1, dy1 = self._ln_bwd(p + ".attention.output.LayerNorm", da, sv.ln1, run.p_hid, sv.seed_ln1,
                                    dysum=self.Gl.get(a1.name + ".up.bias"), dy_out=dyz[:, :H])
            self._adapter_bwd(run, a1, dy1, sv.z1, sv.ob, sv.seed_ad1, dz_out=dyz[:, H:H + A1], pooled=pooled)
            L.gemm(dyz, a1.WF, out_bf16=dctx)
            if pooled is not None and not any((a1.name + k) in self.Gl for k in (".up.weight", ".down.weight", ".down.bias")):
                self._dyz_pool.setdefault(self._dyz_shape, []).append(pooled)
        else:
            dt1, dy1 = self._ln_bwd(p + ".attention.output.LayerNorm", da, sv.ln1, run.p_hid, sv.seed_ln1,
                                    dysum=self.Gl.get(a1.name + ".up.bias") if a1 is not None else None)
            do = dy1
            if a1 is not None:
                do = self._adapter_bwd(run, a1, dy1, sv.z1, sv.ob, sv.seed_ad1)
            L.gemm(do, W["WoT"], out_bf16=dctx)
        if self.reducer is not None:
            self.reducer.window()
        if not sv.emd:
            dqkv = self._attn_bwd(run, sv, dctx)
            for t in range(3 if self.lora_r else 0):
                self._lora_bwd(run, li, t, dqkv[:, t * H:(t + 1) * H], sv.xkv)
            dx = torch.empty(N, H, dtype=F32, device=dev)
            L.gemm(dqkv, W["WqkvT"], aux=dt1, aux_kind=L.AUX_ADD_F32, out_f32=dx)
            return dx, None
        if sv.kvp is not None:
            dq_op, dkv_op = self._attn_bwd_qrows(run, sv, dctx)
        else:
            dqkv = self._attn_bwd(run, sv, dctx)
            dq_op, dkv_op = dqkv[:, :H], dqkv[:, H:]
            for t in range(3 if self.lora_r else 0):
                self._lora_bwd(run, li, t, dqkv[:, t * H:(t + 1) * H], sv.xq if t == 0 else sv.xkv)
        dq = torch.empty(N, H, dtype=F32, device=dev)
        L.gemm(dq_op, W["WqkvT"][:, :H], aux=dt1, aux_kind=L.AUX_ADD_F32, out_f32=dq)
        return dq, dkv_op

    def _attn_bwd(self, run, sv, dctx):
        dqkv = torch.empty(run.N, 3 * self.H, dtype=BF16, device=self.dev)
        st = disent_attn_bwd(self, run, sv, dctx, dqkv, None, defer_pos=True)
        if run.pos_chain is not None and sv.extra:
            run.pos_extra = (st, sv.seed_pos)
        elif run.pos_chain is not None:
            run.pos_chain.add(st, sv.seed_pos)
        return dqkv

    def _attn_bwd_qrows(self, run, sv, dctx):
        B, S, H, nh, dev = run.B, run.S, self.H, self.nh, self.dev
        pl = run.dec_plan
        R, Sp = pl.R, _ru(S, 64)
        rmin, rcnt = _relidx_range(S, self.cfg)
        dqc = torch.empty(R, H, dtype=BF16, device=dev)
        dkv = torch.empty(run.N, 2 * H, dtype=BF16, device=dev)
        dpk, dpq = run.pos_chain.formed_slot() if run.pos_chain is not None else (None, None)
        ws = torch.empty(L.disent_attn_bwd_qrows_ws_bytes(R, Sp, nh), dtype=torch.uint8, device=dev)
        kvp, pqk = sv.kvp, sv.pqk
        L.disent_attn_bwd_qrows(sv.qc, pl.rseg, pl.rpos, kvp[:, :H], kvp[:, H:], pqk[:, H:], pqk[:, :H], self.relidx(S), run.mask_i32,
                                run.klen, dctx, sv.ctx, sv.lse, ATTN_SCALE, dqc, dkv[:, :H], dkv[:, H:], dpk, dpq,
                                rmin, rcnt, ws, B, S, Sp, nh, self.span2, p_drop=run.p_att, seed=sv.seed_att, row0=run.row0)
        if run.pos_chain is not None:
            run.pos_chain.add_formed(sv.seed_pos)
        return dqc, dkv

    def _dlog_operand(self, g):
        rows, Vout = g.shape
        Vp = _ru(Vout, 64)
        dlog = torch.zeros(rows, Vp, dtype=BF16, device=self.dev) if Vp != Vout else torch.empty(rows, Vp, dtype=BF16, device=self.dev)
        dlog[:, :Vout].copy_(g)
        return dlog

    def _head_bwd(self, run, rows, dlog, dq, all_rows=False, compact=False):
        H, dev = self.H, self.dev
        R, Vp = dlog.shape
        Vout = run.Vout
        if Vout == self.V:
            tableT = self.ETb
        else:
            tableT = torch.zeros(H, Vp, dtype=BF16, device=dev)
            tableT[:, :Vout] = self.Ansb.t()
        dhl = L.zeros(R, H, dtype=F32, device=dev)
        if R >= 2048:
            L.gemm(dlog, tableT, out_f32=dhl)
        else:
            L.gemm(dlog, tableT, out_f32=dhl, splitk=max(2, min(16, Vp // 8192)), ws=self.sk_ws)
        hn = run.head_norm
        if compact:
            sub, pre = hn, run.head_pre
        else:
            rl = rows.long()
            sub, pre = NormRef(hn.t[rl].contiguous(), hn.stats[rl].contiguous(), hn.gamma, hn.beta), run.head_pre[rl].contiguous()
        dt, _ = self._ln_bwd("lm_predictions.lm_head.LayerNorm", dhl, sub, 0.0, 0, want_dy_bf16=False)
        dpre = torch.empty(R, H, dtype=BF16, device=dev)
        L.dropout_gelu_bwd(dt, pre, 0.0, 0, out_bf16=dpre)
        dqr = torch.empty(R, H, dtype=F32, device=dev)
        L.gemm(dpre, self.WhT, out_f32=dqr)
        if all_rows:
            dq.add_(dqr)
        else:
            L.scatter_rows_f32(dqr, rows, dq)

    def backward(self, run, gloss: Optional[torch.Tensor], glogits: Optional[torch.Tensor] = None, attach: bool = True,
                 ghid=None):
        if not run.save:
            raise RuntimeError("forward was run without gradient bookkeeping")
        with L.seed_word(run.seed_word):
            return self._backward(run, gloss, glogits, attach, ghid)

    def _hid_grad(self, run, ghid, i):
        g = ghid[i] if ghid is not None and i < len(ghid) else None
        if g is None:
            return None
        g = g.reshape(run.B * run.S, self.H).to(F32)
        return g.index_select(0, run.pk.sel) if run.pk is not None else g.contiguous()

    def _backward(self, run, gloss, glogits, attach, ghid=None):
        cfg, H, dev = self.cfg, self.H, self.dev
        B, S, T = run.B, run.S, run.T
        N = run.N
        pk = run.pk
        if run.plan is not None and run.live_version != self.live_version:
            raise RuntimeError("requires_grad of a trainable parameter changed between this step's forward and its backward: "
                               "the forward saved what the live set of ITS time needs; change the flags between steps")
        if attach:
            self.attach_grads()
        reducer = self.reducer
        runs = lambda stage: self._stage_runs(run, stage)
        if ghid is not None and all(g is None for g in ghid):
            ghid = None
        if run.logit_rows is not None and run.logit_rows.numel() == 0 and reducer is None and ghid is None:
            return

        red = _Ready(self, run, reducer) if reducer is not None else None
        run.dw_pending, run.dw_ready_keys, run.dw_count = [], [], 0
        dec = run.dec_plan
        dq = L.zeros(dec.R if dec is not None else N, H, dtype=F32, device=dev)
        Vout = run.Vout
        Vp = _ru(Vout, 64)
        if gloss is not None and run.labels is not None:
            rows = run.rows_i32
            R = rows.numel()
            if R > 0:
                dlog = torch.empty(R, Vp, dtype=BF16, device=dev)
                gs = gloss.detach().to(F32) if (isinstance(gloss, torch.Tensor) and gloss.is_cuda) else float(gloss)
                ar = torch.arange(R, dtype=torch.int32, device=dev)
                L.ce_bwd_rows(run.logits_c, run.labels_c, ar, Vout, Vp, run.row_lse, run.loss_acc, gs, dlog)
                if dec is not None:
                    self._head_bwd(run, None, dlog, dq, all_rows=True, compact=True)
                else:
                    self._head_bwd(run, rows, dlog, dq)
                del dlog
        if glogits is not None and run.logit_rows is not None:
            rows = run.logit_rows
            R = rows.numel()
            if R > 0:
                gl = glogits.reshape(R, Vout)
                if dec is not None:
                    self._head_bwd(run, None, self._dlog_operand(gl.index_select(0, dec.order)), dq, all_rows=True, compact=True)
                else:
                    self._head_bwd(run, rows, self._dlog_operand(gl), dq, compact=True)
        elif glogits is not None and dec is not None:
            if dec.R:
                gl = glogits.reshape(B * S, Vout).index_select(0, dec.grid)
                self._head_bwd(run, None, self._dlog_operand(gl), dq, all_rows=True, compact=True)
        elif glogits is not None:
            gl = glogits.reshape(B * S, Vout)
            if pk is not None:
                gl = gl.index_select(0, pk.sel)
            self._head_bwd(run, torch.arange(N, dtype=torch.int32, device=dev), self._dlog_operand(gl), dq, all_rows=True)

        def stage_done(key):
            run.dw_ready_keys.append(key)
            self._dw_flush(run, red)

        def end(dx_emb=None):
            self._dw_flush(run, red, force=True)
            if run.side_used:
                torch.cuda.current_stream().wait_stream(self.side)
            return self._backward_bottom(run, red, ghid, dx_emb)

        stage_done("head")
        run.pos_chain = None
        if not runs("decoder"):
            return end()
        run.lora_pos_wait = self._lora_pos and any(t < 2 and self._lora_live(s) for (_, t), s in self.lora_sites.items())
        if any(REL_LN + k in self.Gl for k in ("weight", "bias")) or run.lora_pos_wait:
            run.pos_chain = pos_chain_buffers(self, run)
            if dec is not None:
                run.pos_chain.n_exec = len(run.layers) + (0 if dec.R else 2)
                if not dec.R:
                    for _ in range(2):
                        dpk, dpq = run.pos_chain.formed_slot()
                        dpk.zero_(); dpq.zero_()
                        run.pos_chain.add_formed(0)
        layers = run.layers
        dkv_ops = []
        for _ in range(2 if dec is None or dec.R else 0):
            sv = layers.pop()
            dq, dkv_op = self._layer_bwd(run, sv, dq)
            dkv_ops.append(dkv_op)
        if dec is not None:
            dqc, dq = dq, L.zeros(N, H, dtype=F32, device=dev)
            if dec.R:
                L.scatter_rows_f32(dqc, dec.krows.to(torch.int32), dq)
        below = run.plan is None or run.plan.lowest < run.plan.stages.index("decoder")
        dx = None
        if below:
            WkvT = self.Lw[self.nL - 1]["WqkvT"][:, H:]
            dx = dq
            for op in dkv_ops:
                acc = torch.empty(N, H, dtype=F32, device=dev)
                L.gemm(op, WkvT, aux=dx, aux_kind=L.AUX_ADD_F32, out_f32=acc)
                dx = acc
        del dkv_ops
        if layers and layers[-1].extra:
            sv = layers.pop()
            g = self._hid_grad(run, ghid, self.nL)
            if g is not None:
                dxe, _ = self._layer_bwd(run, sv, g)
                if dx is not None:
                    dx.add_(dxe)
                del dxe
            del sv
        stage_done(f"layer{self.nL - 1}")
        if not below:
            return end()
        while layers:
            sv = layers.pop()
            g = self._hid_grad(run, ghid, sv.li + 1)
            if g is not None:
                dx.add_(g)
            if sv.li == 0 and cfg.conv_kernel_size:
                dx, dcol = self._conv_bwd(run, dx)
                dx, _ = self._layer_bwd(run, sv, dx)
                if pk is None:
                    L.col2im3(dcol, dx, B, S, H, 1)
                else:
                    dcg = torch.zeros(B * S, 3 * H, dtype=F32, device=dev).index_copy_(0, pk.sel, dcol)
                    dxg = torch.zeros(B * S, H, dtype=F32, device=dev)
                    L.col2im3(dcg, dxg, B, S, H, 1)
                    dx.add_(dxg.index_select(0, pk.sel))
                    del dcg, dxg
                stage_done("conv")
            else:
                dx, _ = self._layer_bwd(run, sv, dx)
            stage_done(f"layer{sv.li}")
        if cfg.conv_kernel_size and runs("conv") and not runs("layer0"):
            g = self._hid_grad(run, ghid, 1)
            if g is not None:
                dx.add_(g)
            cn = run.conv_norm
            L.ln_bwd(dx, cn.t, cn.stats, cn.gamma, rowmask=cn.rowmask, dgamma=self.Gl.get("deberta.encoder.conv.LayerNorm.weight"),
                     dbeta=self.Gl.get("deberta.encoder.conv.LayerNorm.bias"), ws=self._ln_ws)
            stage_done("conv")
        return end(dx if runs("emb") else None)

    def _backward_bottom(self, run, red, ghid, dx):
        H, dev = self.H, self.dev
        B, S, T, N, pk = run.B, run.S, run.T, run.N, run.pk
        rn = run.rel_norm
        if run.pos_chain is not None and run.pos_extra is not None:
            run.pos_chain.add(*run.pos_extra)
        run.pos_extra = None
        if run.pos_chain is not None:
            dR = pos_table_grads_batched(self, run, run.pos_chain)
            run.pos_chain = None
            if any(REL_LN + k in self.Gl for k in ("weight", "bias")):
                L.ln_bwd(dR, rn.t, rn.stats, rn.gamma, dgamma=self.Gl.get("deberta.encoder.LayerNorm.weight"),
                         dbeta=self.Gl.get("deberta.encoder.LayerNorm.bias"), ws=self._ln_ws)
        if red:
            red.ready("relln")
        if dx is None:
            if red:
                red.finish()
            return {}
        g = self._hid_grad(run, ghid, 0)
        if g is not None:
            dx.add_(g)
        if run.p_hid > 0:
            L.dropout_f32(dx, run.p_hid, run.seed_emb, out_f32=dx)
        en = run.emb_norm
        dt0 = torch.empty(N, H, dtype=F32, device=dev)
        L.ln_bwd(dx, en.t, en.stats, en.gamma, rowmask=en.rowmask, out_dt=dt0,
                 dgamma=self.Gl.get("deberta.embeddings.LayerNorm.weight"), dbeta=self.Gl.get("deberta.embeddings.LayerNorm.bias"),
                 ws=self._ln_ws)
        gvw, gvb = (self.Gl.get("deberta.embeddings.linear_video." + k) for k in ("weight", "bias"))
        if T and (gvw is not None or gvb is not None or "video" in run.grad_in):
            if pk is None:
                dv = dt0.view(B, S, H)[:, :T].reshape(B * T, H).contiguous()
            else:
                dv = dt0.index_select(0, (pk.row0[:-1].long()[:, None] + torch.arange(T, device=dev)[None]).reshape(-1))
            if gvw is not None:
                Kp = _ru(B * T, 64)
                dvT = torch.empty(H, Kp, dtype=BF16, device=dev)
                vT = torch.empty(self.Fp, Kp, dtype=BF16, device=dev)
                L.transpose_to_bf16(dv, dvT)
                L.transpose_to_bf16(run.video_bf16, vT)
                L.gemm(dvT, vT, aux=gvw, aux_kind=L.AUX_ADD_F32, out_f32=gvw, N=self.F)
            if gvb is not None:
                L.colsum(dv, gvb, self._cs_ws)
        gp = self.Gl.get(PROMPT_NAME)
        if gp is not None:
            L.prompt_grad(dt0, None if pk is None else pk.row0, B, S, T, gp)
        if red:
            red.ready("emb")
            red.finish()
        gin = {}
        if "video" in run.grad_in and T:
            wname = "deberta.embeddings.linear_video.weight"
            WvT = torch.empty(self.F, H, dtype=BF16, device=dev)
            L.transpose_to_bf16(self.Pb[wname], WvT)
            dvb = torch.empty(B * T, H, dtype=BF16, device=dev)
            L.cast_bf16(dv, dvb)
            dvid = torch.empty(B * T, self.Fp, dtype=F32, device=dev)
            L.gemm(dvb, WvT, out_f32=dvid, N=self.F)
            gin["video"] = dvid[:, : self.F].reshape(B, T, self.F).to(run.video_dtype)
        if "embeds" in run.grad_in:
            if pk is None:
                grid = dt0
            else:
                grid = L.zeros(B * S, H, dtype=F32, device=dev).index_copy_(0, pk.sel, dt0)
            gin["embeds"] = grid.view(B, S, H)[:, T + run.P:].to(run.embeds.dtype).contiguous()
        return gin

    def _conv_bwd(self, run, dout):
        B, S, H, dev = run.B, run.S, self.H, self.dev
        N = run.N
        cn = run.conv_norm
        dt = torch.empty(N, H, dtype=F32, device=dev)
        L.ln_bwd(dout, cn.t, cn.stats, cn.gamma, rowmask=cn.rowmask, out_dt=dt,
                 dgamma=self.Gl.get("deberta.encoder.conv.LayerNorm.weight"),
                 dbeta=self.Gl.get("deberta.encoder.conv.LayerNorm.bias"), ws=self._ln_ws)
        dc = torch.empty(N, H, dtype=BF16, device=dev)
        L.dropout_gelu_bwd(dt, run.conv_c, run.p_hid, run.seed_conv, out_bf16=dc)
        dcol = torch.empty(N, 3 * H, dtype=F32, device=dev)
        L.gemm(dc, self.WcT, rowscale=run.mask_f, out_f32=dcol)
        return dt, dcol


class _Ready:

    __slots__ = ("eng", "run", "reducer")

    def __init__(self, eng, run, reducer):
        self.eng, self.run, self.reducer = eng, run, reducer

    def ready(self, key):
        if self.run.dw_event is not None:
            torch.cuda.current_stream().wait_event(self.run.dw_event)
        self.reducer.ready(key)

    def finish(self):
        self.reducer.finish()


@dataclass
class LayerSave:
    li: int = 0
    emd: bool = False
    extra: bool = False
    qkv: torch.Tensor = None
    pqk: torch.Tensor = None
    ctx: torch.Tensor = None
    lse: torch.Tensor = None
    ob: torch.Tensor = None
    z1: torch.Tensor = None
    ln1: NormRef = None
    hpre: torch.Tensor = None
    fb: torch.Tensor = None
    z2: torch.Tensor = None
    ln2: NormRef = None
    seed_pos: int = 0
    seed_att: int = 0
    seed_ad1: int = 0
    seed_ad2: int = 0
    seed_ln1: int = 0
    seed_ln2: int = 0
    psave: torch.Tensor = None
    msave: torch.Tensor = None
    xkv: Optional[torch.Tensor] = None
    xq: Optional[torch.Tensor] = None
    qc: Optional[torch.Tensor] = None
    kvp: Optional[torch.Tensor] = None


@dataclass
class Run:
    B: int
    S: int
    T: int
    Lt: int
    train: bool
    save: bool
    seed_base: int
    p_hid: float
    p_att: float
    p_ad: float
    mask: torch.Tensor = None
    labels: torch.Tensor = None
    rows: torch.Tensor = None
    label_rows: Optional[torch.Tensor] = None
    logit_rows: Optional[torch.Tensor] = None
    want_attn: bool = False
    seed_word: Optional[torch.Tensor] = None
    pk: Optional["Packing"] = None
    N: int = 0
    embeds: Optional[torch.Tensor] = None
    P: int = 0
    grad_in: tuple = ()
    hid_grad: bool = False
    video_dtype: Optional[torch.dtype] = None
    _site: int = 0
    mask_i32: torch.Tensor = None
    rowmask: torch.Tensor = None
    mask_f: torch.Tensor = None
    klen: torch.Tensor = None
    border: torch.Tensor = None
    video_bf16: torch.Tensor = None
    emb_norm: NormRef = None
    seed_emb: int = 0
    rel_norm: NormRef = None
    R32: Optional[torch.Tensor] = None
    Rb: Optional[torch.Tensor] = None
    layers: list = field(default_factory=list)
    dec_grid: Optional[torch.Tensor] = None
    dec_plan: Optional[object] = None
    emd_qkv: Optional[torch.Tensor] = None
    attn_out: list = field(default_factory=list)
    hidden_out: tuple = None
    seed_conv: int = 0
    conv_c: torch.Tensor = None
    conv_norm: NormRef = None
    head_in_all: Optional[torch.Tensor] = None
    head_pre: torch.Tensor = None
    head_norm: NormRef = None
    head_ln_bf16: torch.Tensor = None
    head_table: torch.Tensor = None
    head_bias: torch.Tensor = None
    Vout: int = 0
    ldv: int = 0
    use_ans: bool = False
    rows_i32: torch.Tensor = None
    labels_c: torch.Tensor = None
    logits_c: torch.Tensor = None
    row_lse: torch.Tensor = None
    loss_acc: torch.Tensor = None
    logits: torch.Tensor = None
    logits_pending: bool = False
    dw_pending: list = field(default_factory=list)
    dw_ready_keys: list = field(default_factory=list)
    dw_count: int = 0
    side_used: bool = False
    dw_event: Optional[torch.cuda.Event] = None
    _pos_keep: list = field(default_factory=list)
    pos_chain: Optional["PosChain"] = None
    pos_extra: Optional[tuple] = None
    lora_pos_wait: bool = False
    plan: Optional[object] = None
    live_version: int = 0
    low_layer: int = -1

    def __post_init__(self):
        if not self.N:
            self.N = self.B * self.S

    @property
    def row0(self) -> Optional[torch.Tensor]:
        return self.pk.row0 if self.pk is not None else None

    def next_seed(self) -> int:
        self._site += 1
        return (self.seed_base + self._site * 0x85EBCA77) & 0xFFFFFFFFFFFFFFFF


class _StepFn(torch.autograd.Function):

    @staticmethod
    def forward(ctx, engine, run, loss_t, logits_t, n_hid, *rest):
        ctx.engine, ctx.run, ctx.n_hid = engine, run, n_hid
        ctx.set_materialize_grads(False)
        return (loss_t.detach().clone(), logits_t.detach()) + tuple(h.detach() for h in rest[:n_hid])

    @staticmethod
    def backward(ctx, gloss, glogits, *ghid):
        eng, run = ctx.engine, ctx.run
        gin = {}
        ghid = ghid if any(g is not None for g in ghid) else None
        if gloss is not None or glogits is not None or ghid is not None:
            gin = eng.backward(run, gloss, glogits, ghid=ghid) or {}
        return (None,) * (5 + ctx.n_hid) + tuple(gin.get(k) for k in run.grad_in) + tuple(None for _ in eng.order)
```

frozenbilm_amd/lib.py:

```python
from __future__ import annotations

import ctypes as C
import os
import re
from typing import Optional

import torch

HERE = os.path.dirname(os.path.abspath(__file__))
LIB_PATH = os.environ.get("FBL_LIB") or os.path.join(HERE, "libfbl.so")

ACT_NONE, ACT_GELU, ACT_RELU, ACT_GELU_GRAD = 0, 1, 2, 3
AUX_NONE, AUX_ADD_F32, AUX_ADD_BF16, AUX_MUL_DGELU_BF16, AUX_MUL_POS_BF16, AUX_MUL_BF16 = 0, 1, 2, 3, 4, 5
ABI_VERSION = 9

_CTYPES = {"int": C.c_int, "int64_t": C.c_int64, "float": C.c_float, "uint64_t": C.c_uint64}
_DECL = re.compile(r"(?:^|[;{}])\s*([\w\s*]+?)\s*\b(fbl_\w+)\s*\(([^;()]*)\)\s*(?=;)")


def _ctype(text: str, decl: str):
    if "*" in text:
        return C.c_void_p
    words = [w for w in text.split() if w != "const"]
    if not 1 <= len(words) <= 2 or words[0] not in _CTYPES or not words[-1].isidentifier():
        raise ValueError(f"{decl}: no ctypes mapping for '{text.strip()}'")
    return _CTYPES[words[0]]


def parse_signatures(src: str) -> dict:
    src = re.sub(r"/\*.*?\*/|//[^\n]*", "", src, flags=re.S)
    src = re.sub(r"^[ \t]*#.*$", "", src, flags=re.M)
    out = {}
    for ret, name, params in _DECL.findall(src):
        params = [] if params.strip() in ("", "void") else params.split(",")
        out[name] = (_ctype(ret, name), [_ctype(p, name) for p in params])
    unparsed = set(re.findall(r"\b(fbl_\w+)\s*\(", src)) - set(out)
    if unparsed:
        raise ValueError(f"{', '.join(sorted(unparsed))}: declaration not understood")
    return out


def _header_signatures(header: str) -> dict:
    p = os.path.join(os.path.dirname(HERE), "include", header)
    if not os.path.exists(p):
        raise RuntimeError(f"{p} not found: the binding of libfbl.so takes its argument types from the C headers")
    with open(p) as f:
        return parse_signatures(f.read())


SIGNATURES = _header_signatures("fbl.h")
MHA_SIGNATURES = _header_signatures("fbl_mha.h")
QROWS_SIGNATURES = _header_signatures("fbl_qrows.h")
LIVE_SIGNATURES = _header_signatures("fbl_live.h")
PREDICT_SIGNATURES = _header_signatures("fbl_predict.h")
GROUP_SIGNATURES = _header_signatures("fbl_groups.h")
LORA_SIGNATURES = _header_signatures("fbl_lora.h")
EMA_SIGNATURES = _header_signatures("fbl_ema.h")
PROMPT_SIGNATURES = _header_signatures("fbl_prompt.h")

_LIB = None


def load(path: Optional[str] = None):
    global _LIB
    if _LIB is not None and path is None:
        return _LIB
    p = path or LIB_PATH
    if not os.path.exists(p):
        raise RuntimeError(
            f"{p} not found: the FrozenBiLM MI355X path needs its HIP library (python -m frozenbilm_amd.build); "
            "there is no CPU/eager fallback")
    lib = C.CDLL(p)
    for name, (res, args) in (*SIGNATURES.items(), *MHA_SIGNATURES.items(), *QROWS_SIGNATURES.items(),
                              *LIVE_SIGNATURES.items(), *PREDICT_SIGNATURES.items(), *GROUP_SIGNATURES.items(),
                              *LORA_SIGNATURES.items(), *EMA_SIGNATURES.items(), *PROMPT_SIGNATURES.items()):
        fn = getattr(lib, name)
        fn.restype = res
        fn.argtypes = args
    ver = lib.fbl_abi_version()
    if ver != ABI_VERSION:
        raise RuntimeError(f"{p} has ABI version {ver}, this binding needs {ABI_VERSION}: rebuild it "
                           "(python -m frozenbilm_amd.build --force)")
    if path is None:
        _LIB = lib
    return lib


def _p(t: Optional[torch.Tensor]):
    return None if t is None else t.data_ptr()


def _stream():
    return torch.cuda.current_stream().cuda_stream


_AUX = {}
_NO_AUX = set()


def exclude_from_aux(stream: "torch.cuda.Stream"):
    _NO_AUX.add(stream.cuda_stream)



def set_aux_stream(stream: Optional["torch.cuda.Stream"], device=None):
    dev = torch.device("cuda", torch.cuda.current_device()) if device is None else torch.device(device)
    idx = dev.index if dev.index is not None else torch.cuda.current_device()
    if stream is None:
        _AUX.pop(idx, None)
    else:
        _AUX[idx] = stream


def _aux_stream():
    st = _AUX.get(torch.cuda.current_device())
    if st is None:
        return None
    h = st.cuda_stream
    cur = torch.cuda.current_stream().cuda_stream
    return None if (h == cur or cur in _NO_AUX) else h


_SEED_WORD = None


class seed_word:

    def __init__(self, t: Optional[torch.Tensor]):
        self.t, self.prev = t, None

    def __enter__(self):
        global _SEED_WORD
        if self.t is not None:
            assert self.t.dtype == torch.int64 and self.t.is_cuda and self.t.numel() >= 1
        self.prev, _SEED_WORD = _SEED_WORD, self.t
        return self

    def __exit__(self, *exc):
        global _SEED_WORD
        _SEED_WORD = self.prev
        return False


def _seed_dev():
    return None if _SEED_WORD is None else _SEED_WORD.data_ptr()


def _chk(code: int, name: str):
    if code != 0:
        raise RuntimeError(f"{name} failed with code {code}")


def _req(t: torch.Tensor, dtype, name: str):
    if t.dtype != dtype:
        raise TypeError(f"{name}: expected {dtype}, got {t.dtype}")
    if not t.is_cuda:
        raise RuntimeError(f"{name}: tensor must live in HBM (cuda device), got {t.device}")


def _rows2d(t: torch.Tensor, name: str):
    if t.dim() != 2 or t.stride(1) != 1:
        raise ValueError(f"{name}: need a 2-D row-major view (stride(1)==1), got shape {tuple(t.shape)} strides {t.stride()}")
    return t.stride(0)


def gemm_plan(M, N, K, batch=1, splitk=1):
    return load().fbl_gemm_plan(int(M), int(N), int(K), int(batch), int(splitk))


GK_NAMES = ("G8_256", "G8_224", "G8_128", "G8_SPLITK", "T2_256", "T2_224", "T2_128", "T2_64_RING", "T2_128_SPLITK")
ENTRY_PLAIN, ENTRY_ADAPTER_DOWN, ENTRY_DENSE_ADAPTER_DOWN, ENTRY_ADAPTER_TAIL = 0, 1, 2, 3
GPQ = dict(out_f32=1, out_bf16=2, out_pre=4, bias=8, rowscale=16, aux=32, dropout=64, ws=128, aux_stream=256, r_norm=512)


def gemm_plan_launches(entry, M, N, K, *, lda=None, ldb=None, ldc=None, ld_aux=0, seg_n=0, act=ACT_NONE, aux_kind=AUX_NONE,
                       opts=(), batch=1, splitk=1, ws_floats=0, n_cu=256):
    flags = 0
    for o in opts:
        flags |= GPQ[o]
    out = (C.c_int32 * 13)()
    code = load().fbl_gemm_plan_launches(int(entry), int(M), int(N), int(K), int(K if lda is None else lda),
                                         int(K if ldb is None else ldb), int(N if ldc is None else ldc), int(ld_aux),
                                         int(seg_n), int(act), int(aux_kind), flags, int(batch), int(splitk), int(ws_floats),
                                         int(n_cu), out)
    if code:
        return code, None
    launches = [(GK_NAMES[out[5 + 4 * i]], out[6 + 4 * i], out[7 + 4 * i], bool(out[8 + 4 * i])) for i in range(out[0])]
    return 0, dict(launches=launches, splitk=out[1], k8_per=out[2], fold=bool(out[3]), big8=bool(out[4]))


def gemm(A, B, *, bias=None, rowscale=None, alpha=1.0, act=ACT_NONE, aux=None, aux_kind=AUX_NONE, out_f32=None,
         out_bf16=None, out_pre=None, splitk=1, M=None, N=None, ws=None):
    _req(A, torch.bfloat16, "A")
    _req(B, torch.bfloat16, "B")
    batch = 1
    sA = sB = sC = sX = 0
    if A.dim() == 3:
        batch = A.shape[0]
        sA, sB = A.stride(0), (B.stride(0) if B.dim() == 3 else 0)
        A2, B2 = A[0], (B[0] if B.dim() == 3 else B)
    else:
        A2, B2 = A, B
    lda, ldb = _rows2d(A2, "A"), _rows2d(B2, "B")
    Mv, K = A2.shape
    Nv = B2.shape[0]
    assert B2.shape[1] == K, (A2.shape, B2.shape)
    M = Mv if M is None else M
    N = Nv if N is None else N
    ldc = None
    for o, dt in ((out_f32, torch.float32), (out_bf16, torch.bfloat16), (out_pre, torch.bfloat16)):
        if o is None:
            continue
        _req(o, dt, "out")
        o2 = o[0] if o.dim() == 3 else o
        l = _rows2d(o2, "out")
        assert o2.shape[0] >= M and o2.shape[1] >= N, (o2.shape, M, N)
        if ldc is None:
            ldc = l
            sC = o.stride(0) if o.dim() == 3 else 0
        assert ldc == l, "all outputs of one GEMM must share the row stride"
    ld_aux = 0
    if aux is not None:
        a2 = aux[0] if aux.dim() == 3 else aux
        ld_aux = _rows2d(a2, "aux")
        sX = aux.stride(0) if aux.dim() == 3 else 0
        _req(aux, torch.float32 if aux_kind == AUX_ADD_F32 else torch.bfloat16, "aux")
    sBias = 0
    if bias is not None:
# ... 351 lines not shown
                                          float(scale), float(p_drop), int(seed), _seed_dev(), _p(dQ), _rows2d(dQ, "dQ"),
                                          _p(dK), _rows2d(dK, "dK"), _p(dV), _rows2d(dV, "dV"), _p(dPK), _p(dPQ), int(rmin),
                                          int(rcnt), _p(ws), ws.numel() * ws.element_size(), B, S, Sp, nh, span2, _stream()),
         "fbl_disent_attn_bwd_qrows")


def disent_attn_probs(q, k, pk, pq, relidx, mask, lse, scale, probs, B, S, nh):
    for t, n in ((q, "q"), (k, "k"), (pk, "pk"), (pq, "pq")):
        _req(t, torch.bfloat16, n)
    _req(relidx, torch.int16, "relidx"); _req(mask, torch.int32, "mask"); _req(lse, torch.float32, "lse"); _req(probs, torch.float32, "probs")
    ldq, ldp = _rows2d(q, "q"), _rows2d(pk, "pk")
    assert _rows2d(k, "k") == ldq and _rows2d(pq, "pq") == ldp and probs.is_contiguous() and probs.numel() == B * nh * S * S
    _chk(load().fbl_disent_attn_probs(_p(q), _p(k), ldq, _p(pk), _p(pq), ldp, _p(relidx), _p(mask), _p(lse), float(scale),
                                      _p(probs), B, S, nh, _stream()), "fbl_disent_attn_probs")


def attn_bwd_prep(q, pq, pk, dO, O, QT, PQT, Dv, B, S, Sp, nh, span2, row0=None, relidx=None, PQX=None, PKX=None):
    ldq, ldp, ldo = _rows2d(q, "q"), _rows2d(pq, "pq"), _rows2d(dO, "dO")
    assert _rows2d(pk, "pk") == ldp and _rows2d(O, "O") == ldo
    for t in (QT, PQT, PQX, PKX):
        if t is not None:
            _req(t, torch.bfloat16, "transposed output")
            assert t.is_contiguous()
    for t in (PQX, PKX):
        if t is not None:
            _req(relidx, torch.int16, "relidx")
            assert t.numel() == nh * 64 * 2 * Sp and relidx.numel() == 2 * S - 1
    _chk(load().fbl_attn_bwd_prep(_p(q), ldq, _p(pq), _p(pk), ldp, _p(dO), _p(O), ldo, _p(QT), _p(PQT), _p(Dv), _p(relidx),
                                  _p(PQX), _p(PKX), B, S, Sp, nh, span2, _row0(row0, B, True), _stream()),
         "fbl_attn_bwd_prep")


def attn_rowdot(dO, O, out, B, S, nh):
    ld = _rows2d(dO, "dO")
    assert _rows2d(O, "O") == ld
    _chk(load().fbl_attn_rowdot(_p(dO), _p(O), ld, _p(out), B, S, nh, _stream()), "fbl_attn_rowdot")


def disent_attn_bwd_ds(q, k, v, dO, pk, pq, relidx, mask, lse, Dv, scale, dV, dS, dST, B, S, Sp, nh, span2,
                       p_drop=0.0, seed=0, klen=None, border=None, lin=0, row0=None):
    ldq = _rows2d(q, "q")
    assert _rows2d(k, "k") == ldq and _rows2d(v, "v") == ldq
    ldo, ldp, lddv = _rows2d(dO, "dO"), _rows2d(pk, "pk"), _rows2d(dV, "dV")
    assert _rows2d(pq, "pq") == ldp
    _chk(load().fbl_disent_attn_bwd_ds(_p(q), _p(k), _p(v), ldq, _p(dO), ldo, _p(pk), _p(pq), ldp,
                                       _p(relidx), _p(mask), _p(klen), _p(border), _p(lse), _p(Dv), float(scale), float(p_drop), int(seed), _seed_dev(),
                                       _p(dV), lddv, _p(dS), _p(dST), B, S, Sp, nh, span2, int(lin), _row0(row0, B, klen), _stream()),
         "fbl_disent_attn_bwd_ds")


def disent_attn_bwd_dspk(psave, msave, q, v, dO, pqx, lse, Dv, scale, dK, dV, dS, dST, B, S, Sp, nh, p_drop=0.0, seed=0, klen=None,
                         border=None, row0=None):
    _req(psave, torch.bfloat16, "psave"); _req(msave, torch.float32, "msave"); _req(pqx, torch.bfloat16, "pqx")
    assert psave.is_contiguous() and msave.is_contiguous() and pqx.is_contiguous()
    assert psave.numel() == B * nh * Sp * Sp and msave.numel() == B * nh * (Sp // 64) * S and pqx.numel() == nh * 64 * 2 * Sp
    ldq, ldv, ldo, lddk, lddv = _rows2d(q, "q"), _rows2d(v, "v"), _rows2d(dO, "dO"), _rows2d(dK, "dK"), _rows2d(dV, "dV")
    _chk(load().fbl_disent_attn_bwd_dspk(_p(psave), _p(msave), _p(q), ldq, _p(v), ldv, _p(dO), ldo, _p(pqx), _p(klen), _p(border),
                                         _p(lse), _p(Dv), float(scale), float(p_drop), int(seed), _seed_dev(), _p(dK), lddk,
                                         _p(dV), lddv, _p(dS), _p(dST), B, S, Sp, nh, _row0(row0, B, klen), _stream()),
         "fbl_disent_attn_bwd_dspk")


def disent_attn_bwd_dq(dS, k, pkx, dQ, B, S, Sp, nh, klen=None, border=None, row0=None):
    _req(dS, torch.bfloat16, "dS"); _req(pkx, torch.bfloat16, "pkx")
    assert dS.is_contiguous() and pkx.is_contiguous() and dS.numel() == B * nh * Sp * Sp and pkx.numel() == nh * 2 * Sp * 64
    ldk, lddq = _rows2d(k, "k"), _rows2d(dQ, "dQ")
    _chk(load().fbl_disent_attn_bwd_dq(_p(dS), _p(k), ldk, _p(pkx), _p(klen), _p(border), _p(dQ), lddq, B, S, Sp, nh,
                                       _row0(row0, B, klen), _stream()), "fbl_disent_attn_bwd_dq")


def attn_pos_grad(neg, Xs, Ys, dlo, dcnt, dcnt_max, out, B, S, Sp, nh, rcnt, klen=None, row0=None):
    E = len(Xs)
    assert E == len(Ys) and E > 0
    ldy = _rows2d(Ys[0], "Y")
    for x, y in zip(Xs, Ys):
        _req(x, torch.bfloat16, "X"); _req(y, torch.bfloat16, "Y")
        assert x.is_contiguous() and x.numel() == B * nh * Sp * Sp and _rows2d(y, "Y") == ldy
    _req(dlo, torch.int16, "dlo"); _req(dcnt, torch.int16, "dcnt"); _req(out, torch.float32, "out")
    assert dlo.numel() == rcnt and dcnt.numel() == rcnt and out.is_contiguous() and out.numel() == E * nh * rcnt * 64
    xp = (C.c_void_p * E)(*[x.data_ptr() for x in Xs])
    yp = (C.c_void_p * E)(*[y.data_ptr() for y in Ys])
    _chk(load().fbl_attn_pos_grad(int(neg), xp, yp, ldy, _p(dlo), _p(dcnt), int(dcnt_max), _p(klen), _row0(row0, B, klen), _p(out),
                                  E, B, S, Sp, nh, int(rcnt), _stream()), "fbl_attn_pos_grad")


def disent_attn_bwd_shear(dST, QT, PQT, relidx, dK, B, S, Sp, nh, span2, klen=None, lin=0, border=None, row0=None):
    lddk = _rows2d(dK, "dK")
    sh, sb, sd = head_strides(B, Sp, nh, True)
    _chk(load().fbl_disent_attn_bwd_shear(_p(dST), _p(QT), sh, sb, sd, _p(PQT), _p(relidx), _p(klen), _p(border), _p(dK), lddk,
                                          int(lin), B, S, Sp, nh, span2, _row0(row0, B, klen), _stream()),
         "fbl_disent_attn_bwd_shear")


def ce_fwd(logits, labels, V, row_lse, loss_sum_cnt):
    ldv = _rows2d(logits, "logits")
    _req(logits, torch.float32, "logits"); _req(labels, torch.int64, "labels")
    _chk(load().fbl_ce_fwd(_p(logits), ldv, _p(labels), logits.shape[0], V, _p(row_lse), _p(loss_sum_cnt), _stream()),
         "fbl_ce_fwd")


def ce_bwd_rows(logits, labels, rows, V, Vp, row_lse, loss_sum_cnt, gscale, dlogits):
    ldv = _rows2d(logits, "logits")
    _req(rows, torch.int32, "rows")
    gdev = None
    if isinstance(gscale, torch.Tensor):
        gdev = gscale.reshape(1)
        _req(gdev, torch.float32, "gscale")
        gscale = 1.0
    _chk(load().fbl_ce_bwd_rows(_p(logits), ldv, _p(labels), _p(rows), rows.numel(), V, Vp, _p(row_lse),
                                _p(loss_sum_cnt), float(gscale), _p(gdev), _p(dlogits), _stream()), "fbl_ce_bwd_rows")


PREDICT_MAX_K = 16


def row_predict(logits, V, k, labels=None, row_lse=None):
    ldv = _rows2d(logits, "logits")
    _req(logits, torch.float32, "logits")
    R, dev = logits.shape[0], logits.device
    if not 1 <= int(k) <= PREDICT_MAX_K:
        raise ValueError(f"k = {k}: fbl_row_predict takes 1..{PREDICT_MAX_K}")
    if labels is not None:
        _req(labels, torch.int64, "labels")
        assert labels.is_contiguous() and labels.numel() == R
    if row_lse is not None:
        _req(row_lse, torch.float32, "row_lse")
        assert row_lse.is_contiguous() and row_lse.numel() == R
    ids = torch.empty(R, k, dtype=torch.int32, device=dev)
    lp = torch.empty(R, k, dtype=torch.float32, device=dev)
    rank = torch.empty(R, dtype=torch.int32, device=dev) if labels is not None else None
    nll = torch.empty(R, dtype=torch.float32, device=dev) if labels is not None else None
    h = load()
    nbytes = h.fbl_row_predict_ws_bytes(R, int(V), int(k))
    if nbytes < 0:
        _chk(nbytes, "fbl_row_predict_ws_bytes")
    ws = torch.empty(max(nbytes, 8) // 8, dtype=torch.int64, device=dev)
    _chk(h.fbl_row_predict(_p(logits), ldv, R, int(V), int(k), _p(labels), _p(row_lse), _p(ids), _p(lp), _p(rank), _p(nll),
                           _p(ws), nbytes, _stream()), "fbl_row_predict")
    return ids, lp, rank, nll


def gather_rows_bf16(x, rows, out):
    ld = _rows2d(x, "x")
    _chk(load().fbl_gather_rows_bf16(_p(x), ld, _p(rows), rows.numel(), x.shape[1], _p(out), _stream()),
         "fbl_gather_rows_bf16")


def scatter_rows_f32(x, rows, out):
    ld = _rows2d(out, "out")
    _chk(load().fbl_scatter_rows_f32(_p(x), _p(rows), rows.numel(), x.shape[1], _p(out), ld, _stream()),
         "fbl_scatter_rows_f32")


_SUMSQ_WS = {}


def sumsq(x, out, ws=None):
    if ws is None:
        ws = _SUMSQ_WS.get(x.device)
        if ws is None:
            ws = _SUMSQ_WS[x.device] = torch.empty(load().fbl_sumsq_ws_floats(), dtype=torch.float32, device=x.device)
    _chk(load().fbl_sumsq(_p(x), x.numel(), _p(out), _p(ws), _stream()), "fbl_sumsq")


def adam_flat(p, g, m, v, lr, beta1, beta2, eps, weight_decay, step, sumsq_t=None, max_norm=0.0, grad_scale=1.0):
    _chk(load().fbl_adam_flat(_p(p), _p(g), _p(m), _p(v), p.numel(), float(lr), float(beta1), float(beta2), float(eps),
                              float(weight_decay), int(step), _p(sumsq_t), float(max_norm), float(grad_scale),
                              _stream()), "fbl_adam_flat")


LIVE_MAX_RANGES = 1024


def live_table(ranges, n: int, device) -> torch.Tensor:
    if len(ranges) > LIVE_MAX_RANGES:
        raise ValueError(f"{len(ranges)} live ranges: the kernels take {LIVE_MAX_RANGES}")
    tab, cum, last = [len(ranges), 0], 0, 0
    for b, e in ranges:
        if b < last or e <= b or e > n or b % 8 or e % 8:
            raise ValueError(f"live range [{b}, {e}) of {n}: ranges must be sorted, disjoint, non-empty and 8-aligned")
        tab += [b, cum]
        cum += e - b
        last = e
    tab[1] = cum
    return torch.tensor(tab, dtype=torch.int64, device=device)


def sumsq_live(x, table, out, ws):
    _req(x, torch.float32, "x"); _req(table, torch.int64, "table")
    _chk(load().fbl_sumsq_live(_p(x), x.numel(), _p(table), _p(out), _p(ws), _stream()), "fbl_sumsq_live")


def adam_flat_live(p, g, m, v, table, lr, beta1, beta2, eps, weight_decay, step, sumsq_t=None, max_norm=0.0, grad_scale=1.0):
    _req(table, torch.int64, "table")
    _chk(load().fbl_adam_flat_live(_p(p), _p(g), _p(m), _p(v), p.numel(), _p(table), float(lr), float(beta1), float(beta2),
                                   float(eps), float(weight_decay), int(step), _p(sumsq_t), float(max_norm), float(grad_scale),
                                   _stream()), "fbl_adam_flat_live")


ADAM_MAX_GROUPS = 64
ADAM_GROUP_FLOATS = 6


def group_table(segments, n: int, device, n_groups: int = ADAM_MAX_GROUPS) -> torch.Tensor:
    if len(segments) > LIVE_MAX_RANGES:
        raise ValueError(f"{len(segments)} segments: the kernel takes {LIVE_MAX_RANGES}")
    if not 1 <= n_groups <= ADAM_MAX_GROUPS:
        raise ValueError(f"{n_groups} parameter groups: the kernel takes 1 .. {ADAM_MAX_GROUPS}")
    tab, cum, last = [len(segments), 0], 0, 0
    for b, e, k in segments:
        if b < last or e <= b or e > n or b % 8 or e % 8:
            raise ValueError(f"segment [{b}, {e}) of {n}: segments must be sorted, disjoint, non-empty and 8-aligned")
        if not 0 <= k < n_groups:
            raise ValueError(f"segment [{b}, {e}): group {k} outside [0, {n_groups})")
        tab += [b, cum, k]
        cum += e - b
        last = e
    tab[1] = cum
    return torch.tensor(tab, dtype=torch.int64, device=device)


def adam_hyper(groups):
    if not 1 <= len(groups) <= ADAM_MAX_GROUPS:
        raise ValueError(f"{len(groups)} parameter groups: the kernel takes 1 .. {ADAM_MAX_GROUPS}")
    flat = []
    for lr, b1, b2, eps, wd, dec in groups:
        flat += [float(lr), float(b1), float(b2), float(eps), float(wd), 1.0 if dec else 0.0]
    return (C.c_float * len(flat))(*flat)


def adam_flat_groups(p, g, m, v, table, groups, step, sumsq_t=None, max_norm=0.0, grad_scale=1.0):
    _req(table, torch.int64, "table")
    hyper = groups if isinstance(groups, C.Array) else adam_hyper(groups)
    _chk(load().fbl_adam_flat_groups(_p(p), _p(g), _p(m), _p(v), p.numel(), _p(table), len(hyper) // ADAM_GROUP_FLOATS, hyper,
                                     int(step), _p(sumsq_t), float(max_norm), float(grad_scale), _stream()),
         "fbl_adam_flat_groups")


def _flat32(t, n, name):
    _req(t, torch.float32, name)
    if t.numel() != n or not t.is_contiguous():
        raise ValueError(f"{name}: a contiguous buffer of {n} elements is needed, got {tuple(t.shape)}")
    if n % 8 or t.data_ptr() % 16:
        raise ValueError(f"{name}: {n} elements at {t.data_ptr():#x}: a multiple of 8 elements on a 16-byte boundary is needed")


def adam_flat_groups_ema(p, g, m, v, ema, table, groups, step, ema_w, sumsq_t=None, max_norm=0.0, grad_scale=1.0):
    _req(table, torch.int64, "table")
    for t, name in ((p, "p"), (g, "g"), (m, "m"), (v, "v"), (ema, "ema")):
        _flat32(t, p.numel(), name)
    if ema.device != p.device:
        raise ValueError(f"ema lives on {ema.device}, the parameters on {p.device}")
    if not 0.0 < float(ema_w) <= 1.0:
        raise ValueError(f"ema_w = {ema_w}: the weight of the new parameter lies in (0, 1]")
    hyper = groups if isinstance(groups, C.Array) else adam_hyper(groups)
    _chk(load().fbl_adam_flat_groups_ema(_p(p), _p(g), _p(m), _p(v), _p(ema), p.numel(), _p(table),
                                         len(hyper) // ADAM_GROUP_FLOATS, hyper, int(step), _p(sumsq_t), float(max_norm),
                                         float(grad_scale), float(ema_w), _stream()), "fbl_adam_flat_groups_ema")


def swap_(a, b):
    _flat32(a, a.numel(), "a"); _flat32(b, a.numel(), "b")
    if a.device != b.device:
        raise ValueError(f"a lives on {a.device}, b on {b.device}")
    lo, hi = sorted((a.data_ptr(), b.data_ptr()))
    if a.numel() and lo + 4 * a.numel() > hi:
        raise ValueError("swap_: the two buffers overlap")
    _chk(load().fbl_swap_f32(_p(a), _p(b), a.numel(), _stream()), "fbl_swap_f32")


LORA_MAX_RANK, LORA_SITE_WORDS = 64, 16


class LoraTable:

    def __init__(self, sites, device):
        import struct

        words, self.keep = [], []
        for s in sites:
            W, A, B, dst, dstT, d32 = s["W"], s["A"], s["B"], s["dst"], s["dstT"], s.get("dst32")
            _req(W, torch.float32, "W"); _req(A, torch.float32, "A"); _req(B, torch.float32, "B")
            _req(dst, torch.bfloat16, "dst"); _req(dstT, torch.bfloat16, "dstT")
            O, I = W.shape
            r = A.shape[0]
            assert A.shape == (r, I) and B.shape == (O, r) and A.is_contiguous() and B.is_contiguous(), (W.shape, A.shape, B.shape)
            assert tuple(dst.shape) == (O, I) and tuple(dstT.shape) == (I, O)
            ld32 = 0
            if d32 is not None:
                _req(d32, torch.float32, "dst32")
                assert tuple(d32.shape) == (O, I)
                ld32 = _rows2d(d32, "dst32")
            bits = struct.unpack("<I", struct.pack("<f", float(s["scale"])))[0]
            words += [W.data_ptr(), _rows2d(W, "W"), A.data_ptr(), B.data_ptr(), dst.data_ptr(), _rows2d(dst, "dst"),
                      dstT.data_ptr(), _rows2d(dstT, "dstT"), _p(d32) or 0, ld32, O, I, r, bits, 0, 0]
            self.keep.append((W, A, B, dst, dstT, d32))
        self.n = len(sites)
        self.host = (C.c_int64 * max(len(words), 1))(*words)
        self.dev = torch.tensor(words or [0], dtype=torch.int64, device=device)


def lora_compose(table: LoraTable):
    _chk(load().fbl_lora_compose(table.host, _p(table.dev), table.n, _stream()), "fbl_lora_compose")


def cast_bf16(x, out):
# ... 103 lines not shown
```

frozenbilm_amd/model/deberta.py:

```python
from __future__ import annotations

from collections import OrderedDict
from typing import Dict, List, Optional, Tuple

import torch
from torch import nn

from .. import lib as L
from .adapter import Adapter
from .config import DebertaV2Config


class MaskedLMOutput(dict):

    _fill = None

    def _sync_logits(self):
        fill = self.__dict__.get("_fill")
        if fill is not None:
            self.__dict__["_fill"] = None
            fill()

    def __getattr__(self, k):
        try:
# ... 92 lines not shown
    sh[c + ".LayerNorm.bias"] = (H,)
    if cfg.conv_kernel_size > 0:
        sh[c + ".conv.conv.weight"] = (H, H, cfg.conv_kernel_size)
        sh[c + ".conv.conv.bias"] = (H,)
        sh[c + ".conv.LayerNorm.weight"] = (H,)
        sh[c + ".conv.LayerNorm.bias"] = (H,)
    h = "lm_predictions.lm_head"
    sh[h + ".bias"] = (V,)
    sh[h + ".dense.weight"] = (H, H)
    sh[h + ".dense.bias"] = (H,)
    sh[h + ".LayerNorm.weight"] = (H,)
    sh[h + ".LayerNorm.bias"] = (H,)
    if n_ans:
        sh["answer_embeddings.weight"] = (n_ans, H)
        sh["answer_bias"] = (n_ans,)
    return sh


LORA_TARGETS = ("query_proj", "key_proj", "value_proj")
LORA_DEFAULT_TARGETS = ("query_proj", "value_proj")
LORA_MAX_RANK = 64


def check_lora(rank, alpha, targets):
    if isinstance(rank, bool) or not isinstance(rank, int) or not 0 <= rank <= LORA_MAX_RANK:
        raise ValueError(f"lora_rank must be an integer in 0..{LORA_MAX_RANK} (got {rank!r})")
    if isinstance(targets, str):
        targets = (targets,)
    targets = tuple(targets)
    unknown = [t for t in targets if t not in LORA_TARGETS]
    if unknown:
        raise ValueError(f"lora_targets must be a subset of {LORA_TARGETS} (got {unknown})")
    if rank > 0 and not targets:
        raise ValueError("lora_rank > 0 needs at least one of lora_targets " + str(LORA_TARGETS))
    if rank == 0:
        return 0, 0.0, ()
    alpha = rank if alpha is None else alpha
    return rank, float(alpha) / rank, tuple(t for t in LORA_TARGETS if t in targets)


def lora_shapes(cfg: DebertaV2Config, rank: int, targets) -> "OrderedDict[str, tuple]":
    sh: "OrderedDict[str, tuple]" = OrderedDict()
    for i in range(cfg.num_hidden_layers if rank else 0):
        for t in targets:
            p = f"deberta.encoder.layer.{i}.attention.self.{t}"
            sh[p + ".lora_A.weight"] = (rank, cfg.hidden_size)
            sh[p + ".lora_B.weight"] = (cfg.hidden_size, rank)
    return sh


PROMPT_MAX = 128
PROMPT_NAME = "deberta.embeddings.prompt_embeddings.weight"


def check_n_prompt(n_prompt) -> int:
    if isinstance(n_prompt, bool) or not isinstance(n_prompt, int) or not 0 <= n_prompt <= PROMPT_MAX:
        raise ValueError(f"n_prompt must be an integer in 0..{PROMPT_MAX} (got {n_prompt!r})")
    return n_prompt


def flat_order(cfg: DebertaV2Config, names: List[str]) -> List[str]:
    def take(prefix):
        return [n for n in names if n.startswith(prefix)]

    out: List[str] = []
    out += take("lm_predictions.")
    for i in reversed(range(cfg.num_hidden_layers)):
        if i == 0:
            out += take("deberta.encoder.conv.")
        out += take(f"deberta.encoder.layer.{i}.")
    out += take("deberta.encoder.LayerNorm.")
    out += take("deberta.embeddings.")
    rest = [n for n in names if n not in set(out)]
    return out + rest


class DebertaV2ForMaskedLM(nn.Module):
    def __init__(
        self,
        config,
        max_feats=10,
        features_dim=768,
        freeze_lm=True,
        freeze_mlm=True,
        ds_factor_attn=8,
        ds_factor_ff=8,
        ft_ln=True,
        dropout=0.1,
        n_ans=0,
        freeze_last=True,
        lora_rank=0,
        lora_alpha=None,
        lora_targets=LORA_DEFAULT_TARGETS,
        n_prompt=0,
    ):
        super().__init__()
        self.n_prompt = check_n_prompt(n_prompt)
        self.lora_rank, self.lora_scale, self.lora_targets = check_lora(lora_rank, lora_alpha, lora_targets)
        self.config = DebertaV2Config.from_any(config)
        self.config.validate_supported()
        cfg = self.config
        for ds in (ds_factor_attn, ds_factor_ff):
            if ds:
                assert not cfg.hidden_size % ds
        self.max_feats = max_feats
        self.features_dim = features_dim
        self.ds_factor_attn = ds_factor_attn
        self.ds_factor_ff = ds_factor_ff
        self.adapter_dropout = float(dropout) if dropout else 0.0
        self.n_ans = n_ans
        self.freeze_lm, self.freeze_mlm, self.ft_ln, self.freeze_last = freeze_lm, freeze_mlm, ft_ln, freeze_last
        if not (freeze_lm and freeze_mlm):
            raise NotImplementedError(
                "the MI355X path implements FrozenBiLM's frozen-LM regime (freeze_lm=freeze_mlm=True): "
                "only linear_video, adapters and LayerNorms receive gradients")
        if n_ans and not freeze_last:
            raise NotImplementedError("--ft_last (trainable answer-embedding module) is not implemented: the answer "
                                      "head is used frozen, the reference's default (args.py:358-363)")

        shapes = param_shapes(cfg, features_dim, ds_factor_attn, ds_factor_ff, n_ans)
        g = torch.Generator().manual_seed(0)
        for name, shape in shapes.items():
            if "LayerNorm" in name:
                t = torch.ones(shape) if name.endswith("weight") else torch.zeros(shape)
            elif name.endswith(".bias") or name == "answer_bias":
                t = torch.zeros(shape)
            else:
                t = torch.randn(shape, generator=g) * cfg.initializer_range
            if name.endswith("word_embeddings.weight"):
                t[cfg.pad_token_id].zero_()
            self._register(name, nn.Parameter(t, requires_grad=self._trainable(name)))
        g2 = torch.Generator().manual_seed(1)
        for name, shape in lora_shapes(cfg, self.lora_rank, self.lora_targets).items():
            if ".lora_A." in name:
                bound = 1.0 / shape[1] ** 0.5
                t = (torch.rand(shape, generator=g2) * 2 - 1) * bound
            else:
                t = torch.zeros(shape)
            self._register(name, nn.Parameter(t, requires_grad=True))
        if self.n_prompt:
            g3 = torch.Generator().manual_seed(2)
            t = torch.randn((self.n_prompt, cfg.hidden_size), generator=g3) * cfg.initializer_range
            self._register(PROMPT_NAME, nn.Parameter(t, requires_grad=True))
        emb = self._module("deberta.embeddings")
        emb.register_buffer("position_ids", torch.arange(cfg.max_position_embeddings).expand((1, -1)))
        self._engine = None
        self.engine_options = {}
        self.inference_graphs = self.training_graphs = self.finetune_graphs = False
        from ..train_graph import new_states

        self._graph_routes = new_states()
        self.packed_rows = False
        self.decoder_rows = False
        self.predict_topk = 0
        self._weights_frozen = 0
        self._reducer = None
        self.step_seed = 0
        self._seed_salt = None

    def _module(self, dotted: str) -> nn.Module:
        m: nn.Module = self
        for part in dotted.split("."):
            if part not in m._modules:
                m.add_module(part, _Node())
            m = m._modules[part]
        return m

    def _register(self, name: str, p: nn.Parameter):
        if "." in name:
            mod, leaf = name.rsplit(".", 1)
            self._module(mod).register_parameter(leaf, p)
        else:
            self.register_parameter(name, p)

    def _trainable(self, name: str) -> bool:
        if name.startswith("answer_"):
            return not self.freeze_last
        if "linear_video" in name or "adapter" in name or ".lora_" in name or name == PROMPT_NAME:
            return True
        return bool(self.ft_ln and "LayerNorm" in name)

    def trainable_names(self) -> List[str]:
        return [n for n, _ in self.named_parameters() if self._trainable(n)]

    @property
    def device(self):
        return next(self.parameters()).device

    def get_param(self, name: str) -> torch.Tensor:
        m: nn.Module = self
        parts = name.split(".")
        for part in parts[:-1]:
            m = m._modules[part]
        return m._parameters[parts[-1]]

    def set_answer_embeddings(self, a2tok, freeze_last=True):
        if not freeze_last:
            raise NotImplementedError("--ft_last (trainable answer-embedding module) is not implemented")
        E = self.get_param("deberta.embeddings.word_embeddings.weight")
        pad = self.config.pad_token_id
        a2tok = a2tok.to(E.device)
        keep = (a2tok != pad)
        table = (E.data[a2tok] * keep.float()[:, :, None]).sum(1) / keep.sum(1, keepdim=True).clamp(min=1)
        if len(table) != self.n_ans or "answer_embeddings" not in self._modules:
            assert not self.training
            self.n_ans = len(table)
            self._register("answer_embeddings.weight", nn.Parameter(table.clone(), requires_grad=False))
            old = self._parameters.get("answer_bias")
            self.register_parameter("answer_bias", nn.Parameter(torch.zeros(self.n_ans, device=E.device), requires_grad=False))
            del old
        else:
            self.get_param("answer_embeddings.weight").data = table
        self.freeze_last = freeze_last
        self.get_param("answer_embeddings.weight").requires_grad_(False)
        self.get_param("answer_bias").requires_grad_(False)
        self.invalidate()

    def weights_frozen(self):
        import contextlib

        @contextlib.contextmanager
        def scope():
            self._weights_frozen += 1
            try:
                yield self
            finally:
                self._weights_frozen -= 1
                if self._weights_frozen == 0 and self._engine is not None:
                    self._engine._ops_version = None

        return scope()

    def ema_weights(self):
        from ..ema import weights

        return weights(self)

    def lora_names(self) -> List[str]:
        return [f"deberta.encoder.layer.{i}.attention.self.{t}" for i in range(self.config.num_hidden_layers if self.lora_rank else 0)
                for t in self.lora_targets]

    @torch.no_grad()
    def merge_lora(self):
        from ..ema import refuse_if_open

        refuse_if_open(self, "merge_lora()")
        if not self.lora_rank:
            return self
        self.engine().merge_lora()
        self.invalidate()
        return self

    @torch.no_grad()
    def init_prompt_from_ids(self, ids):
        if not self.n_prompt:
            raise RuntimeError("init_prompt_from_ids needs a model built with n_prompt > 0")
        E = self.get_param("deberta.embeddings.word_embeddings.weight")
        ids = torch.as_tensor(ids)
        if ids.dtype != torch.long or tuple(ids.shape) != (self.n_prompt,):
            raise ValueError(f"ids must be a LongTensor of shape [{self.n_prompt}] (got {ids.dtype} {tuple(ids.shape)})")
        if int(ids.min()) < 0 or int(ids.max()) >= E.shape[0]:
            raise ValueError(f"ids outside the vocabulary 0..{E.shape[0] - 1}")
        self.get_param(PROMPT_NAME).data.copy_(E.data[ids.to(E.device)])
        self.invalidate()
        return self

    def invalidate(self):
        self._engine = None
        from ..train_graph import ROUTES

        for route in ROUTES:
            self.__dict__.pop(route.cache, None)

    def _load_from_state_dict(self, *a, **k):
        self.invalidate()
        return super()._load_from_state_dict(*a, **k)

    def load_state_dict(self, state_dict, strict=True, **kw):
        from ..ema import refuse_if_open

        refuse_if_open(self, "load_state_dict()")
        self.invalidate()
        sd = {k: v for k, v in state_dict.items() if "lm_head.decoder" not in k}
        return super().load_state_dict(sd, strict=strict, **kw)

    def _apply(self, fn, *a, **k):
        self.invalidate()
        return super()._apply(fn, *a, **k)

    def engine(self):
        if self._engine is None:
            from ..engine import Engine

            self._engine = Engine(self)
            if self._reducer is not None:
                self._reducer.rebind(self._engine)
        return self._engine

    def dropout_seed_base(self) -> int:
        if self._seed_salt is None:
            rank = 0
            try:
                import torch.distributed as dist

                if dist.is_available() and dist.is_initialized():
                    rank = dist.get_rank()
# ... 59 lines not shown
```

Measured before the change: 796.4 samples/s.

## Run backward on compacted live rows, skipping padded tokens in dense ops

Adds a compact-backward mode. In this mode the backward pass keeps gradients only for live (non-padding) rows and gathers saved activations into compact buffers with a new multi-tensor row gather kernel. LayerNorm backward gets a row-indexed variant that reads compact gradients, writes zero-filled padded outputs for attention, and skips padded rows. The goal is to cut GEMM and elementwise work on padding tokens in the backward pass. The cost is extra gather/scatter traffic and added bookkeeping to convert back to the full grid at the conv layer and at the end.

```diff
diff --git a/frozenbilm_amd/attn_bwd.py b/frozenbilm_amd/attn_bwd.py
--- a/frozenbilm_amd/attn_bwd.py
+++ b/frozenbilm_amd/attn_bwd.py
@@ -62,7 +62,7 @@
     relidx = eng.relidx(S)
     klen, border = run.klen, getattr(run, "border", None)
     scale = ATTN_SCALE
-    pk_ = getattr(run, "pk", None)
+    pk_ = getattr(run, "cb", None) or getattr(run, "pk", None)
     row0 = pk_.row0 if pk_ is not None else None
     saved_p = getattr(sv, "psave", None) is not None
 
diff --git a/frozenbilm_amd/build.py b/frozenbilm_amd/build.py
--- a/frozenbilm_amd/build.py
+++ b/frozenbilm_amd/build.py
@@ -34,7 +34,7 @@
 
 def _deps_mtime() -> float:
     hdrs = [os.path.join(CSRC, f) for f in os.listdir(CSRC) if f.endswith(".h")]
-    hdrs += [os.path.join(os.path.dirname(HERE), "include", h) for h in ("fbl.h", "fbl_mha.h", "fbl_qrows.h", "fbl_live.h", "fbl_predict.h", "fbl_groups.h", "fbl_lora.h", "fbl_ema.h", "fbl_prompt.h")]
+    hdrs += [os.path.join(os.path.dirname(HERE), "include", h) for h in ("fbl.h", "fbl_mha.h", "fbl_qrows.h", "fbl_live.h", "fbl_predict.h", "fbl_groups.h", "fbl_lora.h", "fbl_ema.h", "fbl_prompt.h", "fbl_rows.h")]
     return max(os.path.getmtime(h) for h in hdrs)
 
 
diff --git a/frozenbilm_amd/csrc/rowops.hip b/frozenbilm_amd/csrc/rowops.hip
--- a/frozenbilm_amd/csrc/rowops.hip
+++ b/frozenbilm_amd/csrc/rowops.hip
@@ -3,6 +3,7 @@
 #include "../../include/fbl_live.h"
 #include "../../include/fbl_groups.h"
 #include "../../include/fbl_ema.h"
+#include "../../include/fbl_rows.h"
 
 namespace {
 
@@ -168,8 +169,9 @@
   const float* dout; const int32_t* rowmask; const float* t; const float* stats; const float* gamma;
   float p_drop; uint64_t seed; const uint64_t* seed_dev; float* out_dt; bf16* out_dy_bf16; float* out_dy_f32; float* ws; int N, H;
   long ld_dyb;
+  const int32_t* inv; bf16* out_dy_pad;
 };
-template <int EPL>
+template <int EPL, bool ROWS = false>
 __global__ __launch_bounds__(256) void ln_bwd_kernel(LnBwdArgs a) {
   constexpr int VEC = (EPL % 4 == 0) ? 4 : ((EPL % 2 == 0) ? 2 : 1);
   constexpr int NIT = EPL / VEC;
@@ -185,6 +187,17 @@
   const float inv_keep = a.p_drop > 0.f ? 1.0f / (1.0f - a.p_drop) : 1.0f;
   const uint64_t seed = a.p_drop > 0.f ? fbl_seed(a.seed, a.seed_dev) : 0;
   for (int row = blockIdx.x * 4 + wave; row < a.N; row += gridDim.x * 4) {
+    long crow = row;
+    if (ROWS) {
+      const int cr = a.inv[row];
+      if (cr < 0) {
+        const float z[VEC] = {};
+#pragma unroll
+        for (int it = 0; it < NIT; ++it) stb<VEC>(a.out_dy_pad + (long)row * H + (it * 64 + lane) * VEC, z);
+        continue;
+      }
+      crow = cr;
+    }
     const float mean = a.stats[2 * (long)row], rstd = a.stats[2 * (long)row + 1];
     const float om = a.rowmask ? (float)a.rowmask[row] : 1.0f;
     float g[EPL], xh[EPL];
@@ -193,7 +206,7 @@
     for (int it = 0; it < NIT; ++it) {
       const int col = (it * 64 + lane) * VEC;
       float d[VEC], x[VEC];
-      ldf<VEC>(a.dout + (long)row * H + col, d);
+      ldf<VEC>(a.dout + crow * H + col, d);
       ldf<VEC>(a.t + (long)row * H + col, x);
 #pragma unroll
       for (int c = 0; c < VEC; ++c) {
@@ -221,9 +234,10 @@
         if (a.p_drop > 0.f) dy[c] *= fbl_dropout_scale(seed, (uint64_t)row * H + col + c, thr, inv_keep);
         dys[e] += dy[c];
       }
-      if (a.out_dt) stf<VEC>(a.out_dt + (long)row * H + col, dt);
-      if (a.out_dy_bf16) stb<VEC>(a.out_dy_bf16 + (long)row * a.ld_dyb + col, dy);
-      if (a.out_dy_f32) stf<VEC>(a.out_dy_f32 + (long)row * H + col, dy);
+      if (a.out_dt) stf<VEC>(a.out_dt + crow * H + col, dt);
+      if (a.out_dy_bf16) stb<VEC>(a.out_dy_bf16 + crow * a.ld_dyb + col, dy);
+      if (a.out_dy_f32) stf<VEC>(a.out_dy_f32 + crow * H + col, dy);
+      if (ROWS) stb<VEC>(a.out_dy_pad + (long)row * H + col, dy);
     }
   }
 #pragma unroll
@@ -245,7 +259,7 @@
     }
   }
 }
-template <int EPL>
+template <int EPL, bool ROWS = false>
 __global__ __launch_bounds__(256, 3) void ln_bwd2_kernel(LnBwdArgs a) {
   static_assert(EPL % 2 == 0, "two waves share a row");
   constexpr int EW = EPL / 2;
@@ -268,32 +282,44 @@
   int par = 0;
   for (int base = blockIdx.x * 2; base < a.N; base += gridDim.x * 2, par ^= 1) {
     const int row = base + slot;
-    const bool live = row < a.N;
+    bool live = row < a.N;
     const int rr = live ? row : a.N - 1;
-    const float mean = a.stats[2 * (long)rr], rstd = a.stats[2 * (long)rr + 1];
-    const float om = live ? (a.rowmask ? (float)a.rowmask[rr] : 1.0f) : 0.f;
+    long crow = row;
+    bool pad_zero = false;
+    if (ROWS) {
+      const int cr = a.inv[rr];
+      pad_zero = live && cr < 0;
+      live = live && cr >= 0;
+      crow = cr;
+    }
     float g[EW], xh[EW];
-    float s1 = 0.f, s2 = 0.f;
-#pragma unroll
-    for (int it = 0; it < NIT; ++it) {
-      const int col = c0 + (it * 64 + lane) * VEC;
-      float d[VEC], x[VEC];
-      ldf<VEC>(a.dout + (long)rr * H + col, d);
-      ldf<VEC>(a.t + (long)rr * H + col, x);
-#pragma unroll
-      for (int c = 0; c < VEC; ++c) {
-        const int e = it * VEC + c;
-        const float dd = d[c] * om;
-        xh[e] = (x[c] - mean) * rstd;
-        dg[e] += dd * xh[e];
-        db[e] += dd;
-        g[e] = dd * gam[e];
-        s1 += g[e];
-        s2 += g[e] * xh[e];
+    float s1 = 0.f, s2 = 0.f, rstd = 0.f;
+    if (!ROWS || live) {
+      const long lr = ROWS ? crow : (long)rr;
+      const float mean = a.stats[2 * (long)rr];
+      rstd = a.stats[2 * (long)rr + 1];
+      const float om = live ? (a.rowmask ? (float)a.rowmask[rr] : 1.0f) : 0.f;
+#pragma unroll
+      for (int it = 0; it < NIT; ++it) {
+        const int col = c0 + (it * 64 + lane) * VEC;
+        float d[VEC], x[VEC];
+        ldf<VEC>(a.dout + lr * H + col, d);
+        ldf<VEC>(a.t + (long)rr * H + col, x);
+#pragma unroll
+        for (int c = 0; c < VEC; ++c) {
+          const int e = it * VEC + c;
+          const float dd = d[c] * om;
+          xh[e] = (x[c] - mean) * rstd;
+          dg[e] += dd * xh[e];
+          db[e] += dd;
+          g[e] = dd * gam[e];
+          s1 += g[e];
+          s2 += g[e] * xh[e];
+        }
       }
-    }
-    s1 = wave_sum(s1);
-    s2 = wave_sum(s2);
+      s1 = wave_sum(s1);
+      s2 = wave_sum(s2);
+    }
     if (lane == 0) {
       xch[par][slot][half][0] = s1;
       xch[par][slot][half][1] = s2;
@@ -314,10 +340,15 @@
           if (a.p_drop > 0.f) dy[c] *= fbl_dropout_scale(seed, (uint64_t)row * H + col + c, thr, inv_keep);
           dys[e] += dy[c];
         }
-        if (a.out_dt) stf<VEC>(a.out_dt + (long)row * H + col, dt);
-        if (a.out_dy_bf16) stb<VEC>(a.out_dy_bf16 + (long)row * a.ld_dyb + col, dy);
-        if (a.out_dy_f32) stf<VEC>(a.out_dy_f32 + (long)row * H + col, dy);
+        if (a.out_dt) stf<VEC>(a.out_dt + crow * H + col, dt);
+        if (a.out_dy_bf16) stb<VEC>(a.out_dy_bf16 + crow * a.ld_dyb + col, dy);
+        if (a.out_dy_f32) stf<VEC>(a.out_dy_f32 + crow * H + col, dy);
+        if (ROWS) stb<VEC>(a.out_dy_pad + (long)row * H + col, dy);
       }
+    } else if (ROWS && pad_zero) {
+      const float z[VEC] = {};
+#pragma unroll
+      for (int it = 0; it < NIT; ++it) stb<VEC>(a.out_dy_pad + (long)row * H + c0 + (it * 64 + lane) * VEC, z);
     }
   }
 #pragma unroll
@@ -1096,6 +1127,41 @@
 }
 
 extern "C" int64_t fbl_ln_bwd_ws_floats(int H) { return (int64_t)LNB_BLOCKS * 3 * H; }
+template <bool ROWS>
+static int ln_bwd_launch(const LnBwdArgs& a, float* dgamma, float* dbeta, float* dysum, hipStream_t stream) {
+  const int N = a.N, H = a.H;
+  int nblk;
+  if ((H / 64) % 2 == 0) {
+    nblk = (N + 1) / 2;
+    if (nblk > LNB_BLOCKS) nblk = LNB_BLOCKS;
+    dim3 grid(nblk);
+    switch (H / 64) {
+      case 2: hipLaunchKernelGGL((ln_bwd2_kernel<2, ROWS>), grid, dim3(256), 0, stream, a); break;
+      case 4: hipLaunchKernelGGL((ln_bwd2_kernel<4, ROWS>), grid, dim3(256), 0, stream, a); break;
+      case 8: hipLaunchKernelGGL((ln_bwd2_kernel<8, ROWS>), grid, dim3(256), 0, stream, a); break;
+      case 12: hipLaunchKernelGGL((ln_bwd2_kernel<12, ROWS>), grid, dim3(256), 0, stream, a); break;
+      case 16: hipLaunchKernelGGL((ln_bwd2_kernel<16, ROWS>), grid, dim3(256), 0, stream, a); break;
+      case 24: hipLaunchKernelGGL((ln_bwd2_kernel<24, ROWS>), grid, dim3(256), 0, stream, a); break;
+      case 32: hipLaunchKernelGGL((ln_bwd2_kernel<32, ROWS>), grid, dim3(256), 0, stream, a); break;
+      default: return FBL_ERR_SHAPE;
+    }
+  } else {
+    nblk = (N + 3) / 4;
+    if (nblk > LNB_BLOCKS) nblk = LNB_BLOCKS;
+    dim3 grid(nblk);
+    switch (H / 64) {
+      case 1: hipLaunchKernelGGL((ln_bwd_kernel<1, ROWS>), grid, dim3(256), 0, stream, a); break;
+      default: return FBL_ERR_SHAPE;
+    }
+  }
+  FBL_CHECK_LAUNCH();
+  if (dgamma || dbeta || dysum) {
+    hipLaunchKernelGGL(ln_bwd_fold_kernel, dim3((3 * H + 31) / 32), dim3(256), 0, stream, a.ws, nblk, H, dgamma, dbeta, dysum);
+    FBL_CHECK_LAUNCH();
+  }
+  return 0;
+}
+
 extern "C" int fbl_ln_bwd(const float* dout, const int32_t* rowmask, const float* t, const float* stats,
                           const float* gamma, float p_drop, uint64_t seed, const uint64_t* seed_dev, float* out_dt, void* out_dy_bf16,
                           float* out_dy_f32, float* dgamma, float* dbeta, float* dysum, float* ws, int N, int H,
@@ -1104,35 +1170,23 @@
   if (N <= 0) return 0;
   if (ld_dy_bf16 == 0) ld_dy_bf16 = H;
   if (ld_dy_bf16 < H || (ld_dy_bf16 % 8)) return FBL_ERR_ALIGN;
-  LnBwdArgs a{dout, rowmask, t, stats, gamma, p_drop, seed, seed_dev, out_dt, (bf16*)out_dy_bf16, out_dy_f32, ws, N, H, ld_dy_bf16};
-  int nblk;
-  if ((H / 64) % 2 == 0) {
-    nblk = (N + 1) / 2;
-    if (nblk > LNB_BLOCKS) nblk = LNB_BLOCKS;
-    dim3 grid(nblk);
-    switch (H / 64) {
-      case 2: hipLaunchKernelGGL(ln_bwd2_kernel<2>, grid, dim3(256), 0, (hipStream_t)stream, a); break;
-      case 4: hipLaunchKernelGGL(ln_bwd2_kernel<4>, grid, dim3(256), 0, (hipStream_t)stream, a); break;
-      case 8: hipLaunchKernelGGL(ln_bwd2_kernel<8>, grid, dim3(256), 0, (hipStream_t)stream, a); break;
-      case 12: hipLaunchKernelGGL(ln_bwd2_kernel<12>, grid, dim3(256), 0, (hipStream_t)stream, a); break;
-      case 16: hipLaunchKernelGGL(ln_bwd2_kernel<16>, grid, dim3(256), 0, (hipStream_t)stream, a); break;
-      case 24: hipLaunchKernelGGL(ln_bwd2_kernel<24>, grid, dim3(256), 0, (hipStream_t)stream, a); break;
-      case 32: hipLaunchKernelGGL(ln_bwd2_kernel<32>, grid, dim3(256), 0, (hipStream_t)stream, a); break;
-      default: return FBL_ERR_SHAPE;
-    }
-  } else {
-    nblk = (N + 3) / 4;
-    if (nblk > LNB_BLOCKS) nblk = LNB_BLOCKS;
-    dim3 grid(nblk);
-    FBL_EPL_DISPATCH(H, ln_bwd_kernel, grid, a, (hipStream_t)stream);
-  }
-  FBL_CHECK_LAUNCH();
-  if (dgamma || dbeta || dysum) {
-    hipLaunchKernelGGL(ln_bwd_fold_kernel, dim3((3 * H + 31) / 32), dim3(256), 0, (hipStream_t)stream, ws, nblk, H,
-                       dgamma, dbeta, dysum);
-    FBL_CHECK_LAUNCH();
-  }
-  return 0;
+  LnBwdArgs a{dout, rowmask, t, stats, gamma, p_drop, seed, seed_dev, out_dt, (bf16*)out_dy_bf16, out_dy_f32, ws, N, H, ld_dy_bf16,
+              nullptr, nullptr};
+  return ln_bwd_launch<false>(a, dgamma, dbeta, dysum, (hipStream_t)stream);
+}
+
+extern "C" int fbl_ln_bwd_rows(const float* dout, const int32_t* inv, const int32_t* rowmask, const float* t, const float* stats,
+                               const float* gamma, float p_drop, uint64_t seed, const uint64_t* seed_dev, float* out_dt,
+                               void* out_dy_bf16, int64_t ld_dy_bf16, void* out_dy_pad_bf16, float* dgamma, float* dbeta,
+                               float* dysum, float* ws, int N_pad, int H, void* stream) {
+  if (H % 64 || H > 2048) return FBL_ERR_SHAPE;
+  if (!dout || !inv || !t || !stats || !gamma || !ws || !out_dy_pad_bf16) return FBL_ERR_ARG;
+  if (N_pad <= 0) return 0;
+  if (ld_dy_bf16 == 0) ld_dy_bf16 = H;
+  if (ld_dy_bf16 < H || (ld_dy_bf16 % 8)) return FBL_ERR_ALIGN;
+  LnBwdArgs a{dout, rowmask, t, stats, gamma, p_drop, seed, seed_dev, out_dt, (bf16*)out_dy_bf16, nullptr, ws, N_pad, H, ld_dy_bf16,
+              inv, (bf16*)out_dy_pad_bf16};
+  return ln_bwd_launch<true>(a, dgamma, dbeta, dysum, (hipStream_t)stream);
 }
 
 extern "C" int fbl_im2col3(const void* x_bf16, void* out_bf16, int B, int S, int H, void* stream) {
diff --git a/frozenbilm_amd/csrc/rows.hip b/frozenbilm_amd/csrc/rows.hip
--- /dev/null
+++ b/frozenbilm_amd/csrc/rows.hip
@@ -0,0 +1,95 @@
+#include "fbl_common.h"
+#include "../../include/fbl_rows.h"
+
+namespace {
+
+typedef __attribute__((ext_vector_type(4))) unsigned int u32x4;
+
+struct GatherArgs {
+  const char* src[FBL_GATHER_MAX_TENSORS];
+  char* dst[FBL_GATHER_MAX_TENSORS];
+  long sld[FBL_GATHER_MAX_TENSORS], dld[FBL_GATHER_MAX_TENSORS];
+  int units[FBL_GATHER_MAX_TENSORS];
+  int v16[FBL_GATHER_MAX_TENSORS];
+  const int32_t* sel;
+  int n;
+};
+
+template <typename V>
+__device__ __forceinline__ void copy_row(const V* __restrict__ s, V* __restrict__ d, int n) {
+  for (int j = threadIdx.x; j < n; j += 4 * 256) {
+    V v[4];
+#pragma unroll
+    for (int u = 0; u < 4; ++u)
+      if (j + u * 256 < n) v[u] = s[j + u * 256];
+#pragma unroll
+    for (int u = 0; u < 4; ++u)
+      if (j + u * 256 < n) d[j + u * 256] = v[u];
+  }
+}
+
+__global__ __launch_bounds__(256) void gather_rows_multi_kernel(GatherArgs a) {
+  const long c = blockIdx.x;
+  const long r = a.sel[c];
+#pragma unroll
+  for (int i = 0; i < FBL_GATHER_MAX_TENSORS; ++i) {
+    if (i < a.n) {
+      const char* s = a.src[i] + r * a.sld[i];
+      char* d = a.dst[i] + c * a.dld[i];
+      if (a.v16[i]) copy_row<u32x4>((const u32x4*)s, (u32x4*)d, a.units[i]);
+      else copy_row<uint32_t>((const uint32_t*)s, (uint32_t*)d, a.units[i]);
+    }
+  }
+}
+
+__global__ __launch_bounds__(256) void scatter_rows_zero_bf16_kernel(const bf16* __restrict__ src, long ld_src,
+                                                                     const int32_t* __restrict__ inv, long n_units, int upr,
+                                                                     bf16* __restrict__ dst, long ld_dst) {
+  const long idx = (long)blockIdx.x * 256 + threadIdx.x;
+  if (idx >= n_units) return;
+  const long r = idx / upr;
+  const int u = (int)(idx - r * upr);
+  const int c = inv[r];
+  u32x4 v = {0u, 0u, 0u, 0u};
+  if (c >= 0) v = *(const u32x4*)(src + (long)c * ld_src + u * 8);
+  *(u32x4*)(dst + r * ld_dst + u * 8) = v;
+}
+
+}
+
+extern "C" int fbl_gather_rows_multi(int n, const void* const* src, void* const* dst, const int64_t* row_bytes,
+                                     const int64_t* src_ld, const int64_t* dst_ld, const int32_t* sel, int Np, void* stream) {
+  if (n < 1 || n > FBL_GATHER_MAX_TENSORS || !src || !dst || !row_bytes || !src_ld || !dst_ld || !sel) return FBL_ERR_ARG;
+  GatherArgs a{};
+  for (int i = 0; i < n; ++i) {
+    if (!src[i] || !dst[i] || row_bytes[i] <= 0 || src_ld[i] < row_bytes[i] || dst_ld[i] < row_bytes[i]) return FBL_ERR_ARG;
+    if (row_bytes[i] > ((int64_t)1 << 30)) return FBL_ERR_ARG;
+    const uintptr_t bits = (uintptr_t)src[i] | (uintptr_t)dst[i] | (uintptr_t)row_bytes[i] | (uintptr_t)src_ld[i] | (uintptr_t)dst_ld[i];
+    if (bits & 3) return FBL_ERR_ALIGN;
+    a.src[i] = (const char*)src[i];
+    a.dst[i] = (char*)dst[i];
+    a.sld[i] = (long)src_ld[i];
+    a.dld[i] = (long)dst_ld[i];
+    a.v16[i] = (bits & 15) == 0;
+    a.units[i] = (int)(row_bytes[i] / (a.v16[i] ? 16 : 4));
+  }
+  if (Np <= 0) return 0;
+  a.sel = sel;
+  a.n = n;
+  hipLaunchKernelGGL(gather_rows_multi_kernel, dim3(Np), dim3(256), 0, (hipStream_t)stream, a);
+  FBL_CHECK_LAUNCH();
+  return 0;
+}
+
+extern "C" int fbl_scatter_rows_zero_bf16(const void* src, int64_t ld_src, const int32_t* inv, int N_pad, int cols, void* dst,
+                                          int64_t ld_dst, void* stream) {
+  if (N_pad <= 0 || cols == 0) return 0;
+  if (!src || !inv || !dst || cols < 0 || ld_src < cols || ld_dst < cols) return FBL_ERR_ARG;
+  if ((cols % 8) || (ld_src % 8) || (ld_dst % 8) || ((uintptr_t)src & 15) || ((uintptr_t)dst & 15)) return FBL_ERR_ALIGN;
+  const int upr = cols / 8;
+  const long n_units = (long)N_pad * upr;
+  hipLaunchKernelGGL(scatter_rows_zero_bf16_kernel, dim3((unsigned)((n_units + 255) / 256)), dim3(256), 0, (hipStream_t)stream,
+                     (const bf16*)src, (long)ld_src, inv, n_units, upr, (bf16*)dst, (long)ld_dst);
+  FBL_CHECK_LAUNCH();
+  return 0;
+}
diff --git a/frozenbilm_amd/engine.py b/frozenbilm_amd/engine.py
--- a/frozenbilm_amd/engine.py
+++ b/frozenbilm_amd/engine.py
@@ -1,5 +1,6 @@
 from __future__ import annotations
 
+import dataclasses
 from dataclasses import dataclass, field
 from typing import Dict, List, Optional
 
@@ -60,6 +61,8 @@
     inv: torch.Tensor
     pos: torch.Tensor
     n: int
+    sel32: Optional[torch.Tensor] = None
+    inv32: Optional[torch.Tensor] = None
 
 
 @dataclass
@@ -139,6 +142,7 @@
         self.reducer = None
         self._dyz_pool: Dict[tuple, list] = {}
         self._dyz_shape = None
+        self._dyz_compact = None
         self.params_version = 0
         self._ops_version = None
         self.skip_dead_layer = True
@@ -566,6 +570,8 @@
                 full_labels = labels
             full_labels = full_labels.contiguous().view(-1)
             rows_labelled = torch.nonzero(full_labels != -100).view(-1)
+        bwd_rows = self._backward_rows(m, need_grad, tuple(k for k, _ in grad_in), mask, full_labels, logit_rows, want_hidden, want_attn,
+                                        B, S, T)
         if logit_rows is not None:
             if full_labels is not None:
                 raise RuntimeError("logit_rows cannot be combined with labels (the loss of a labelled call lives on its own rows)")
@@ -581,7 +587,8 @@
                   p_hid=self.cfg.hidden_dropout_prob if train else 0.0,
                   p_att=self.cfg.attention_probs_dropout_prob if train else 0.0,
                   p_ad=m.adapter_dropout if train else 0.0, mask=mask.view(-1), pk=pk, N=pk.n if pk is not None else B * S,
-                  want_attn=bool(want_attn), labels=full_labels, rows=rows_labelled if full_labels is not None else None)
+                  want_attn=bool(want_attn), labels=full_labels, rows=rows_labelled if full_labels is not None else None,
+                  bwd_rows=bwd_rows)
         if want_attn and train and run.p_att > 0:
             raise NotImplementedError("output_attentions=True is served in eval mode (the probabilities of a training forward "
                                       "carry the attention dropout mask, which the fused kernel regenerates instead of storing)")
@@ -630,6 +637,23 @@
         elif full_labels is not None:
             res["loss"] = loss_t
         return res
+
+    COMPACT_BWD_MIN_DROPPED = 0.37
+
+    def _backward_rows(self, m, need_grad, grad_in, mask, full_labels, logit_rows, want_hidden, want_attn, B, S, T) -> Optional[Packing]:
+        force = getattr(m, "compact_backward", None)
+        if (force is False or not need_grad or full_labels is None or logit_rows is not None or want_hidden or want_attn
+                or torch.cuda.is_current_stream_capturing() or getattr(m, "packed_rows", False) or getattr(m, "decoder_rows", False)
+                or self.lora_r or self.n_prompt or self.reducer is not None or not self.attn_save_p):
+            return None
+        plan = self.plan(grad_in)
+        if plan is not None and plan.lowest != 0:
+            return None
+        pk = self._make_packing(mask, full_labels, None, B, S, T)
+        if pk is None or (force is not True and 1.0 - pk.n / (B * S) < self.COMPACT_BWD_MIN_DROPPED):
+            return None
+        pk.sel32, pk.inv32 = pk.sel.to(torch.int32), pk.inv.to(torch.int32)
+        return pk
 
     def _make_packing(self, mask, full_labels, logit_rows, B, S, T) -> Optional[Packing]:
         dev = self.dev
@@ -1108,8 +1132,16 @@
         run.conv_c, run.conv_norm = c, out.norm
         return out
 
-    def _ln_bwd(self, name, dout, norm: NormRef, p_drop, seed, want_dy_bf16=True, dysum=None, tail=0, dy_out=None):
+    def _ln_bwd(self, name, dout, norm: NormRef, p_drop, seed, want_dy_bf16=True, dysum=None, tail=0, dy_out=None, cb=None):
         N, H = dout.shape
+        if cb is not None:
+            dt = torch.empty(N, H, dtype=F32, device=self.dev)
+            dyb = dy_out if dy_out is not None else torch.empty(N, H, dtype=BF16, device=self.dev)
+            dy_pad = torch.empty(norm.t.shape[0], H, dtype=BF16, device=self.dev)
+            L.ln_bwd_rows(dout, cb.inv32, norm.t, norm.stats, norm.gamma, rowmask=norm.rowmask, p_drop=p_drop, seed=seed, out_dt=dt,
+                          out_dy_bf16=dyb, out_dy_pad=dy_pad, dgamma=self.Gl.get(name + ".weight"), dbeta=self.Gl.get(name + ".bias"),
+                          dysum=dysum, ws=self._ln_ws)
+            return dt, dyb, dy_pad
         dt_full = torch.empty(N + tail, H, dtype=F32, device=self.dev)
         dt = dt_full[:N]
         if tail:
@@ -1122,7 +1154,7 @@
             return dt, dyb, dt_full
         return dt, dyb
 
-    def _adapter_bwd(self, run, site: AdapterSite, dyb, z, xin_b, seed, dz_out=None, pooled=None):
+    def _adapter_bwd(self, run, site: AdapterSite, dyb, z, xin_b, seed, dz_out=None, pooled=None, pad=None):
         N, H = dyb.shape
         A, Ap = site.A, site.Ap
         dev = self.dev
@@ -1137,11 +1169,15 @@
         if dz_out is None:
             dx = torch.empty(N, H, dtype=BF16, device=dev)
             L.gemm(dz, downT, aux=dyb, aux_kind=L.AUX_ADD_BF16, out_bf16=dx)
-        sk = max(2, min(16, N // 512))
         nm = site.name
         gwu, gwd, gbd = (self.Gl.get(nm + k) for k in (".up.weight", ".down.weight", ".down.bias"))
         if gwu is None and gwd is None and gbd is None:
             return dx
+        if pad is not None:
+            dz_c, (dyb, z) = dz, pad
+            dz = torch.empty(dyb.shape[0], dz_c.shape[1], dtype=BF16, device=dev)
+            L.scatter_rows_zero_bf16(dz_c, run.cb.inv32, dz)
+        sk = max(2, min(16, dyb.shape[0] // 512))
 
         if site.grouped:
             run.dw_pending.append((A, nm, (dyb, z, dz, xin_b), run.dw_count, pooled))
@@ -1203,6 +1239,9 @@
         H, I, dev = self.H, self.I, self.dev
         N = dout.shape[0]
         p = f"deberta.encoder.layer.{li}"
+        cb = run.cb
+        if cb is not None:
+            return self._layer_bwd_compact(run, sv, dout, cb)
         dt2, dy2 = self._ln_bwd(p + ".output.LayerNorm", dout, sv.ln2, run.p_hid, sv.seed_ln2,
                                 dysum=self.Gl.get(a2.name + ".up.bias") if a2 is not None else None)
         df = dy2
@@ -1263,8 +1302,59 @@
         L.gemm(dq_op, W["WqkvT"][:, :H], aux=dt1, aux_kind=L.AUX_ADD_F32, out_f32=dq)
         return dq, dkv_op
 
+    def _layer_bwd_compact(self, run, sv: "LayerSave", dout: torch.Tensor, cb: Packing):
+        li = sv.li
+        W, (a1, a2) = self.Lw[li], self.sites[li]
+        H, I, dev = self.H, self.I, self.dev
+        Np = dout.shape[0]
+        p = f"deberta.encoder.layer.{li}"
+        pairs = [(t, torch.empty(Np, t.shape[1], dtype=t.dtype, device=dev))
+                 for t in (sv.qkv, sv.ctx, sv.hpre, sv.z1 if a1 is not None else None, sv.z2 if a2 is not None else None) if t is not None]
+        L.gather_rows_multi(pairs, cb.sel32)
+        got = {id(src): dst for src, dst in pairs}
+        qkv, ctx, hpre = got[id(sv.qkv)], got[id(sv.ctx)], got[id(sv.hpre)]
+        dt2, dy2, dy2p = self._ln_bwd(p + ".output.LayerNorm", dout, sv.ln2, run.p_hid, sv.seed_ln2,
+                                      dysum=self.Gl.get(a2.name + ".up.bias") if a2 is not None else None, cb=cb)
+        df = dy2
+        if a2 is not None:
+            df = self._adapter_bwd(run, a2, dy2, got[id(sv.z2)], sv.fb, sv.seed_ad2, pad=(dy2p, sv.z2))
+        del dy2p
+        dh = torch.empty(Np, I, dtype=BF16, device=dev)
+        L.gemm(df, W["WdT"], aux=hpre, aux_kind=L.AUX_MUL_BF16, out_bf16=dh)
+        da = torch.empty(Np, H, dtype=F32, device=dev)
+        L.gemm(dh, W["WiT"], aux=dt2, aux_kind=L.AUX_ADD_F32, out_f32=da)
+        del dh, hpre
+        dctx = torch.empty(Np, H, dtype=BF16, device=dev)
+        if a1 is not None and a1.merged:
+            A1, Kf = a1.A, a1.WF.shape[1]
+            dyz = self._dyz_compact
+            if dyz is None or tuple(dyz.shape) != (Np, Kf):
+                dyz = self._dyz_compact = torch.zeros(Np, Kf, dtype=BF16, device=dev)
+            dt1, dy1, dy1p = self._ln_bwd(p + ".attention.output.LayerNorm", da, sv.ln1, run.p_hid, sv.seed_ln1,
+                                          dysum=self.Gl.get(a1.name + ".up.bias"), dy_out=dyz[:, :H], cb=cb)
+            self._adapter_bwd(run, a1, dy1, got[id(sv.z1)], sv.ob, sv.seed_ad1, dz_out=dyz[:, H:H + A1], pad=(dy1p, sv.z1))
+            L.gemm(dyz, a1.WF, out_bf16=dctx)
+        else:
+            dt1, dy1, dy1p = self._ln_bwd(p + ".attention.output.LayerNorm", da, sv.ln1, run.p_hid, sv.seed_ln1,
+                                          dysum=self.Gl.get(a1.name + ".up.bias") if a1 is not None else None, cb=cb)
+            do = dy1
+            if a1 is not None:
+                do = self._adapter_bwd(run, a1, dy1, got[id(sv.z1)], sv.ob, sv.seed_ad1, pad=(dy1p, sv.z1))
+            L.gemm(do, W["WoT"], out_bf16=dctx)
+        del dy1p
+        svc = dataclasses.replace(sv, qkv=qkv, ctx=ctx)
+        dqkv = self._attn_bwd(run, svc, dctx)
+        sv.psave = sv.msave = None
+        if not sv.emd:
+            dx = torch.empty(Np, H, dtype=F32, device=dev)
+            L.gemm(dqkv, W["WqkvT"], aux=dt1, aux_kind=L.AUX_ADD_F32, out_f32=dx)
+            return dx, None
+        dq = torch.empty(Np, H, dtype=F32, device=dev)
+        L.gemm(dqkv[:, :H], W["WqkvT"][:, :H], aux=dt1, aux_kind=L.AUX_ADD_F32, out_f32=dq)
+        return dq, dqkv[:, H:]
+
     def _attn_bwd(self, run, sv, dctx):
-        dqkv = torch.empty(run.N, 3 * self.H, dtype=BF16, device=self.dev)
+        dqkv = torch.empty(dctx.shape[0], 3 * self.H, dtype=BF16, device=self.dev)
         st = disent_attn_bwd(self, run, sv, dctx, dqkv, None, defer_pos=True)
         if run.pos_chain is not None and sv.extra:
             run.pos_extra = (st, sv.seed_pos)
@@ -1296,7 +1386,7 @@
         dlog[:, :Vout].copy_(g)
         return dlog
 
-    def _head_bwd(self, run, rows, dlog, dq, all_rows=False, compact=False):
+    def _head_bwd(self, run, rows, dlog, dq, all_rows=False, compact=False, to_rows=None):
         H, dev = self.H, self.dev
         R, Vp = dlog.shape
         Vout = run.Vout
@@ -1324,7 +1414,7 @@
         if all_rows:
             dq.add_(dqr)
         else:
-            L.scatter_rows_f32(dqr, rows, dq)
+            L.scatter_rows_f32(dqr, rows if to_rows is None else to_rows, dq)
 
     def backward(self, run, gloss: Optional[torch.Tensor], glogits: Optional[torch.Tensor] = None, attach: bool = True,
                  ghid=None):
@@ -1360,7 +1450,9 @@
         red = _Ready(self, run, reducer) if reducer is not None else None
         run.dw_pending, run.dw_ready_keys, run.dw_count = [], [], 0
         dec = run.dec_plan
-        dq = L.zeros(dec.R if dec is not None else N, H, dtype=F32, device=dev)
+        cb = run.cb = run.bwd_rows if (glogits is None and ghid is None and gloss is not None and dec is None and pk is None) else None
+        run.bwd_compact = cb is not None
+        dq = L.zeros(dec.R if dec is not None else (cb.n if cb is not None else N), H, dtype=F32, device=dev)
         Vout = run.Vout
         Vp = _ru(Vout, 64)
         if gloss is not None and run.labels is not None:
@@ -1374,7 +1466,7 @@
                 if dec is not None:
                     self._head_bwd(run, None, dlog, dq, all_rows=True, compact=True)
                 else:
-                    self._head_bwd(run, rows, dlog, dq)
+                    self._head_bwd(run, rows, dlog, dq, to_rows=cb.inv32[rows.long()] if cb is not None else None)
                 del dlog
         if glogits is not None and run.logit_rows is not None:
             rows = run.logit_rows
@@ -1399,7 +1491,12 @@
             run.dw_ready_keys.append(key)
             self._dw_flush(run, red)
 
+        def to_grid(x):
+            run.cb = None
+            return L.zeros(N, H, dtype=F32, device=dev).index_copy_(0, cb.sel, x)
+
         def end(dx_emb=None):
+            run.cb = None
             self._dw_flush(run, red, force=True)
             if run.side_used:
                 torch.cuda.current_stream().wait_stream(self.side)
@@ -1435,7 +1532,7 @@
             WkvT = self.Lw[self.nL - 1]["WqkvT"][:, H:]
             dx = dq
             for op in dkv_ops:
-                acc = torch.empty(N, H, dtype=F32, device=dev)
+                acc = torch.empty(dx.shape[0], H, dtype=F32, device=dev)
                 L.gemm(op, WkvT, aux=dx, aux_kind=L.AUX_ADD_F32, out_f32=acc)
                 dx = acc
         del dkv_ops
@@ -1456,7 +1553,14 @@
             g = self._hid_grad(run, ghid, sv.li + 1)
             if g is not None:
                 dx.add_(g)
-            if sv.li == 0 and cfg.conv_kernel_size:
+            if sv.li == 0 and cfg.conv_kernel_size and cb is not None:
+                dx, dcol = self._conv_bwd(run, to_grid(dx))
+                run.cb = cb
+                dx, _ = self._layer_bwd(run, sv, dx.index_select(0, cb.sel))
+                dx = to_grid(dx)
+                L.col2im3(dcol, dx, B, S, H, 1)
+                stage_done("conv")
+            elif sv.li == 0 and cfg.conv_kernel_size:
                 dx, dcol = self._conv_bwd(run, dx)
                 dx, _ = self._layer_bwd(run, sv, dx)
                 if pk is None:
@@ -1479,6 +1583,8 @@
             L.ln_bwd(dx, cn.t, cn.stats, cn.gamma, rowmask=cn.rowmask, dgamma=self.Gl.get("deberta.encoder.conv.LayerNorm.weight"),
                      dbeta=self.Gl.get("deberta.encoder.conv.LayerNorm.bias"), ws=self._ln_ws)
             stage_done("conv")
+        if run.cb is not None:
+            dx = to_grid(dx)
         return end(dx if runs("emb") else None)
 
     def _backward_bottom(self, run, red, ghid, dx):
@@ -1630,6 +1736,9 @@
     want_attn: bool = False
     seed_word: Optional[torch.Tensor] = None
     pk: Optional["Packing"] = None
+    bwd_rows: Optional["Packing"] = None
+    cb: Optional["Packing"] = None
+    bwd_compact: bool = False
     N: int = 0
     embeds: Optional[torch.Tensor] = None
     P: int = 0
diff --git a/frozenbilm_amd/lib.py b/frozenbilm_amd/lib.py
--- a/frozenbilm_amd/lib.py
+++ b/frozenbilm_amd/lib.py
@@ -57,6 +57,8 @@
 LORA_SIGNATURES = _header_signatures("fbl_lora.h")
 EMA_SIGNATURES = _header_signatures("fbl_ema.h")
 PROMPT_SIGNATURES = _header_signatures("fbl_prompt.h")
+
+ROWS_SIGNATURES = _header_signatures("fbl_rows.h")
 
 _LIB = None
 
@@ -73,7 +75,8 @@
     lib = C.CDLL(p)
     for name, (res, args) in (*SIGNATURES.items(), *MHA_SIGNATURES.items(), *QROWS_SIGNATURES.items(),
                               *LIVE_SIGNATURES.items(), *PREDICT_SIGNATURES.items(), *GROUP_SIGNATURES.items(),
-                              *LORA_SIGNATURES.items(), *EMA_SIGNATURES.items(), *PROMPT_SIGNATURES.items()):
+                              *LORA_SIGNATURES.items(), *EMA_SIGNATURES.items(), *PROMPT_SIGNATURES.items(),
+                              *ROWS_SIGNATURES.items()):
         fn = getattr(lib, name)
         fn.restype = res
         fn.argtypes = args
@@ -731,6 +734,44 @@
          "fbl_scatter_rows_f32")
 
 
+GATHER_MAX_TENSORS = 8
+
+
+def gather_rows_multi(pairs, sel):
+    _req(sel, torch.int32, "sel")
+    Np, n = sel.numel(), len(pairs)
+    assert sel.is_contiguous() and 1 <= n <= GATHER_MAX_TENSORS
+    rb, sl, dl = [], [], []
+    for src, dst in pairs:
+        assert src.dtype == dst.dtype and src.is_cuda and dst.is_cuda and src.shape[1] == dst.shape[1] and dst.shape[0] == Np
+        es = src.element_size()
+        rb.append(src.shape[1] * es); sl.append(_rows2d(src, "src") * es); dl.append(_rows2d(dst, "dst") * es)
+    tab = lambda ts: (C.c_void_p * n)(*[_p(t) for t in ts])
+    arr = lambda v: (C.c_int64 * n)(*v)
+    _chk(load().fbl_gather_rows_multi(n, tab([s for s, _ in pairs]), tab([d for _, d in pairs]), arr(rb), arr(sl), arr(dl), _p(sel),
+                                      Np, _stream()), "fbl_gather_rows_multi")
+
+
+def scatter_rows_zero_bf16(src, inv, out):
+    _req(src, torch.bfloat16, "src"); _req(out, torch.bfloat16, "out"); _req(inv, torch.int32, "inv")
+    assert inv.is_contiguous() and inv.numel() == out.shape[0] and src.shape[1] == out.shape[1]
+    _chk(load().fbl_scatter_rows_zero_bf16(_p(src), _rows2d(src, "src"), _p(inv), out.shape[0], out.shape[1], _p(out),
+                                           _rows2d(out, "out"), _stream()), "fbl_scatter_rows_zero_bf16")
+
+
+def ln_bwd_rows(dout, inv, t, stats, gamma, *, rowmask=None, p_drop=0.0, seed=0, out_dt=None, out_dy_bf16=None, out_dy_pad,
+                dgamma=None, dbeta=None, dysum=None, ws=None):
+    N, H = t.shape
+    _req(inv, torch.int32, "inv"); _req(out_dy_pad, torch.bfloat16, "out_dy_pad")
+    assert dout.is_contiguous() and t.is_contiguous() and inv.is_contiguous() and inv.numel() == N
+    assert out_dy_pad.is_contiguous() and tuple(out_dy_pad.shape) == (N, H) and dout.shape[1] == H
+    assert out_dt is None or (out_dt.is_contiguous() and out_dt.shape == dout.shape)
+    ld_dyb = _rows2d(out_dy_bf16, "out_dy_bf16") if out_dy_bf16 is not None else 0
+    _chk(load().fbl_ln_bwd_rows(_p(dout), _p(inv), _p(rowmask), _p(t), _p(stats), _p(gamma), float(p_drop), int(seed), _seed_dev(),
+                                _p(out_dt), _p(out_dy_bf16), ld_dyb, _p(out_dy_pad), _p(dgamma), _p(dbeta), _p(dysum), _p(ws), N, H,
+                                _stream()), "fbl_ln_bwd_rows")
+
+
 _SUMSQ_WS = {}
 
 
diff --git a/frozenbilm_amd/model/deberta.py b/frozenbilm_amd/model/deberta.py
--- a/frozenbilm_amd/model/deberta.py
+++ b/frozenbilm_amd/model/deberta.py
@@ -268,6 +268,7 @@
         self._graph_routes = new_states()
         self.packed_rows = False
         self.decoder_rows = False
+        self.compact_backward = None
         self.predict_topk = 0
         self._weights_frozen = 0
         self._reducer = None
diff --git a/include/fbl_rows.h b/include/fbl_rows.h
--- /dev/null
+++ b/include/fbl_rows.h
@@ -0,0 +1,24 @@
+#ifndef FBL_ROWS_H
+#define FBL_ROWS_H
+#include "fbl.h"
+#ifdef __cplusplus
+extern "C" {
+#endif
+
+#define FBL_GATHER_MAX_TENSORS 8
+
+int fbl_ln_bwd_rows(const float* dout, const int32_t* inv, const int32_t* rowmask, const float* t, const float* stats,
+                    const float* gamma, float p_drop, uint64_t seed, const uint64_t* seed_dev, float* out_dt, void* out_dy_bf16,
+                    int64_t ld_dy_bf16, void* out_dy_pad_bf16, float* dgamma, float* dbeta, float* dysum, float* ws, int N_pad,
+                    int H, void* stream);
+
+int fbl_gather_rows_multi(int n, const void* const* src, void* const* dst, const int64_t* row_bytes, const int64_t* src_ld,
+                          const int64_t* dst_ld, const int32_t* sel, int Np, void* stream);
+
+int fbl_scatter_rows_zero_bf16(const void* src, int64_t ld_src, const int32_t* inv, int N_pad, int cols, void* dst, int64_t ld_dst,
+                               void* stream);
+
+#ifdef __cplusplus
+}
+#endif
+#endif
```

Measured after the change: 831.1 samples/s, median of 6. 4.4% higher.
